# KwangsungKim138/Korean-F5-TTS

Hardware: AMD Instinct MI355X
Metric: RTF (audio_sec/wall_sec) F5-TTS Base NFE=16 batch=1 (higher is better)
Workload: dtype f16; 1 GPU; C2: F5-TTS Base, 1 utterance/rank/step, prompt 256 + generated 768 mel frames, NFE=16 EPSS, cfg 2.0, sway -1, Vocos decode, mel all_gather when n_gpus>1; global_batch=1, frames=1024, parallelism=dp1, weights=synthetic random-init seed 0

## Files before the change

### korean-f5-tts_amd/csrc/attn2.h

```cpp
#pragma once
#include "attn.h"
#include "gemm2.h"

namespace f5 {

__device__ __forceinline__ float group_max(float v) {
    const unsigned u = __builtin_bit_cast(unsigned, v);
    auto a = __builtin_amdgcn_permlane32_swap(u, u, false, false);
    float m = fmaxf(__builtin_bit_cast(float, (unsigned)a[0]), __builtin_bit_cast(float, (unsigned)a[1]));
    const unsigned w = __builtin_bit_cast(unsigned, m);
    auto b = __builtin_amdgcn_permlane16_swap(w, w, false, false);
    return fmaxf(__builtin_bit_cast(float, (unsigned)b[0]), __builtin_bit_cast(float, (unsigned)b[1]));
}

template <typename T, int STAGE_IDX, bool EDGE, int VAR>
__device__ __forceinline__ void attn2_tile(const char* smem_ptr, unsigned lds_base, int k_off, int kc0, int kc1, int v_off, int vc,
                                           const u32x4 (&qf)[2][2], f32x4 (&o)[4][2], float (&mrun)[2], float (&lrun)[2],
                                           int key_base, int kv_len, bool first) {
    constexpr bool LAZY = (VAR & 4) != 0;
    constexpr int TILE = 64 * 128;
    constexpr float L2E = 1.4426950408889634f;
    const unsigned sb = lds_base + STAGE_IDX * (2 * TILE);
    u32x4 kf[2][2], vf[4];
    const char* sbp = smem_ptr + STAGE_IDX * (2 * TILE);
// ... 78 lines not shown
#pragma unroll
            for (int ks = 0; ks < 2; ++ks)
#pragma unroll
                for (int r = 0; r < 4; ++r) {
                    float p = __builtin_amdgcn_exp2f(s[ks][qs][r]);
                    if (EDGE && key_base + ks * 4 + r >= kv_len) p = 0.f;
                    s[ks][qs][r] = p;
                    psum += p;
                }
            lrun[qs] += psum;
        }
    } else {
    float alpha[2];
    bool grew = false;
#pragma unroll
    for (int qs = 0; qs < 2; ++qs) {
        if (EDGE) {
#pragma unroll
            for (int ks = 0; ks < 2; ++ks)
#pragma unroll
                for (int r = 0; r < 4; ++r)
                    if (key_base + ks * 4 + r >= kv_len) s[ks][qs][r] = -1e30f;
        }
#pragma unroll
        for (int ks = 0; ks < 2; ++ks)
#pragma unroll
            for (int r = 0; r < 4; ++r) s[ks][qs][r] *= L2E;
        float mloc = fmaxf(fmaxf(fmaxf(s[0][qs][0], s[0][qs][1]), fmaxf(s[0][qs][2], s[0][qs][3])),
                           fmaxf(fmaxf(s[1][qs][0], s[1][qs][1]), fmaxf(s[1][qs][2], s[1][qs][3])));
        if (VAR & 2) {
            mloc = group_max(mloc);
        } else {
            mloc = fmaxf(mloc, __shfl_xor(mloc, 16, 64));
            mloc = fmaxf(mloc, __shfl_xor(mloc, 32, 64));
        }
        const float mnew = fmaxf(mrun[qs], mloc);
        grew = grew || (mnew > mrun[qs]);
        alpha[qs] = __builtin_amdgcn_exp2f(mrun[qs] - mnew);
        mrun[qs] = mnew;
        float psum = 0.f;
#pragma unroll
        for (int ks = 0; ks < 2; ++ks)
#pragma unroll
            for (int r = 0; r < 4; ++r) {
                float p = __builtin_amdgcn_exp2f(s[ks][qs][r] - mnew);
                if (EDGE && key_base + ks * 4 + r >= kv_len) p = 0.f;
                s[ks][qs][r] = p;
                psum += p;
            }
        lrun[qs] = lrun[qs] * alpha[qs] + psum;
    }
    if (__any(grew)) {
#pragma unroll
        for (int qs = 0; qs < 2; ++qs)
#pragma unroll
            for (int dt = 0; dt < 4; ++dt) {
                o[dt][qs][0] *= alpha[qs]; o[dt][qs][1] *= alpha[qs]; o[dt][qs][2] *= alpha[qs]; o[dt][qs][3] *= alpha[qs];
            }
    }
    }
    u32x4 pf2[2];
#pragma unroll
    for (int qs = 0; qs < 2; ++qs) {
        pf2[qs] = pack8<T>(s[0][qs][0], s[0][qs][1], s[0][qs][2], s[0][qs][3], s[1][qs][0], s[1][qs][1], s[1][qs][2], s[1][qs][3]);
    }
    if (VAR & 1) {
        __builtin_amdgcn_sched_barrier(0);
        wait_lgkm<0>(vf[0], vf[1], vf[2], vf[3]);
    }
#pragma unroll
    for (int dt = 0; dt < 4; ++dt) {
#pragma unroll
        for (int qs = 0; qs < 2; ++qs) o[dt][qs] = Mma<T>::run(vf[dt], pf2[qs], o[dt][qs]);
    }
}

__device__ __forceinline__ int kswz(int r) { return (((r >> 3) & 3) << 1) | ((r >> 1) & 1); }

template <typename T, int VAR>
__global__ __launch_bounds__(512) void attn2_fwd_kernel(const T* __restrict__ Q, const T* __restrict__ K,
                                                               const T* __restrict__ Vt, T* __restrict__ O, int H,
                                                               int N, int Npad, const int* __restrict__ kv_lens,
                                                               int nbatch_lens, const int* __restrict__ q_lens,
                                                               const int* __restrict__ o_row_start, float* __restrict__ Of = nullptr) {
    extern __shared__ __attribute__((aligned(16))) char smem[];
    int bhid, qblk;
    attn_block_map(bhid, qblk);
    if (q_lens && qblk * 128 >= q_lens[(bhid / H) % nbatch_lens]) return;
    constexpr int NS = 3;
    constexpr int TILE = 64 * 128;
    constexpr int STAGE = 2 * TILE;
    constexpr int L = 2;
    constexpr float L2E = 1.4426950408889634f;

    const int tid = threadIdx.x, lane = tid & 63;
    const int wave = __builtin_amdgcn_readfirstlane(tid >> 6);
    const int qg = wave >> 1, kh = wave & 1;
    const int l15 = lane & 15, g = lane >> 4;
    const int b = bhid / H, h = bhid - b * H;
    const size_t bh = (size_t)bhid;
    const int q0 = qblk * 128 + qg * 32;
    int kv_len = N;
    if (kv_lens) kv_len = min(N, kv_lens[b % nbatch_lens]);
    const int nkt = (kv_len + 63) / 64;

    u32x4 qf[2][2];
#pragma unroll
    for (int qs = 0; qs < 2; ++qs) {
        const int q = min(q0 + qs * 16 + l15, N - 1);
#pragma unroll
        for (int f = 0; f < 2; ++f)
            qf[qs][f] = *reinterpret_cast<const u32x4*>(reinterpret_cast<const char*>(Q + (bh * N + q) * 64) + f * 64 + g * 16);
    }

    const int lr = lane >> 3, ls = lane & 7;
    const int krow = wave * 8 + lr;
    const int kchunk = ls ^ kswz(krow);
    const int vrow = wave * 8 + lr;
    const int vchunk = ls ^ (vrow & 7);
    const T* ksrc = K + bh * (size_t)N * 64 + kchunk * 8;
    const T* vsrc = Vt + (bh * 64 + vrow) * (size_t)Npad + vchunk * 8;
    auto issue = [&](int kt, int stage) {
        if (kt >= nkt) return;
        const int t = kt;
        char* base = smem + stage * STAGE;
        const int key = min(t * 64 + krow, N - 1);
        glds16(ksrc + (size_t)key * 64, base + wave * 1024);
        glds16(vsrc + t * 64, base + TILE + wave * 1024);
    };

    f32x4 o[4][2];
#pragma unroll
    for (int dt = 0; dt < 4; ++dt)
#pragma unroll
        for (int qs = 0; qs < 2; ++qs) o[dt][qs] = f32x4{0.f, 0.f, 0.f, 0.f};
    float mrun[2] = {(VAR & 4) ? 0.f : -1e30f, (VAR & 4) ? 0.f : -1e30f}, lrun[2] = {0.f, 0.f};

    const int ka = l15 >> 2, kb = l15 & 3;
    const int krd = kh * 32 + 8 * ka + kb;
    const int ksw = kswz(krd);
    const int k_off = krd * 128;
    const int kc0 = ((0 + g) ^ ksw) * 16, kc1 = ((4 + g) ^ ksw) * 16;
    const int v_off = TILE + l15 * 128;
    const int vc = ((4 * kh + g) ^ (l15 & 7)) * 16;
    const int key_lane = kh * 32 + 8 * g;
    const unsigned lds_base = (unsigned)(size_t)(__attribute__((address_space(3))) char*)smem;

    issue(0, 0);
    issue(1, 1);
    if (VAR & 1) __builtin_amdgcn_s_waitcnt(0xC07F);
    const int nfull = kv_len / 64;
    int kt = 0;
#define F5_ATTN_STEP(SI, EDGE_)                                                                                        \
    {                                                                                                                  \
        if (kt + 1 < nkt) wait_vmcnt<(NS - 2) * L>(); else wait_vmcnt<0>();                                            \
        __builtin_amdgcn_s_barrier();                                                                                  \
        issue(kt + NS - 1, (SI + NS - 1) % NS);                                                                        \
        attn2_tile<T, SI, EDGE_, VAR>(smem, lds_base, k_off, kc0, kc1, v_off, vc, qf, o, mrun, lrun, kt * 64 + key_lane, kv_len, kt == 0);        \
        ++kt;                                                                                                          \
    }
    while (kt + 3 <= nfull) {
        F5_ATTN_STEP(0, false)
        F5_ATTN_STEP(1, false)
        F5_ATTN_STEP(2, false)
    }
    if (kt < nkt) { if (kt < nfull) F5_ATTN_STEP(0, false) else F5_ATTN_STEP(0, true) }
    if (kt < nkt) { if (kt < nfull) F5_ATTN_STEP(1, false) else F5_ATTN_STEP(1, true) }
    if (kt < nkt) { F5_ATTN_STEP(2, true) }
#undef F5_ATTN_STEP
    __builtin_amdgcn_s_barrier();

#pragma unroll
    for (int qs = 0; qs < 2; ++qs) {
        float l = lrun[qs];
        l += __shfl_xor(l, 16, 64);
        l += __shfl_xor(l, 32, 64);
        lrun[qs] = l;
    }
    float* mb = reinterpret_cast<float*>(smem) + (size_t)qg * (36 * 64);
    if (kh == 1) {
#pragma unroll
        for (int dt = 0; dt < 4; ++dt)
#pragma unroll
            for (int qs = 0; qs < 2; ++qs)
#pragma unroll
                for (int r = 0; r < 4; ++r) mb[((dt * 2 + qs) * 4 + r) * 64 + lane] = o[dt][qs][r];
        mb[32 * 64 + lane] = mrun[0];
        mb[33 * 64 + lane] = mrun[1];
        mb[34 * 64 + lane] = lrun[0];
        mb[35 * 64 + lane] = lrun[1];
    }
    __syncthreads();
    if (kh == 0) {
#pragma unroll
        for (int qs = 0; qs < 2; ++qs) {
            const float m1 = mb[(32 + qs) * 64 + lane], l1 = mb[(34 + qs) * 64 + lane];
            const float m = fmaxf(mrun[qs], m1);
            const float a0 = exp2f(mrun[qs] - m), a1 = exp2f(m1 - m);
            const float inv = 1.0f / (lrun[qs] * a0 + l1 * a1);
            const int q = q0 + qs * 16 + l15;
            const size_t orow = o_row_start ? (size_t)o_row_start[b] + q : (size_t)b * N + q;
            if (q < (o_row_start ? min(N, o_row_start[b + 1] - o_row_start[b]) : N)) {
                T* dst = O + orow * (H * 64) + h * 64 + g * 4;
#pragma unroll
                for (int dt = 0; dt < 4; ++dt) {
                    float v[4];
#pragma unroll
                    for (int r = 0; r < 4; ++r)
                        v[r] = (o[dt][qs][r] * a0 + mb[((dt * 2 + qs) * 4 + r) * 64 + lane] * a1) * inv;
                    if (Of) store4_planar(Of + orow * (H * 64), h * 64 + g * 4 + dt * 16, v[0], v[1], v[2], v[3]);
                    else store4(dst + dt * 16, v[0], v[1], v[2], v[3]);
                }
            }
        }
    }
}

inline int& attn2_variant() { static int v = 7; return v; }
template <typename T> inline float attention_q_scale();
template <> inline float attention_q_scale<float>() { return 0.125f; }
template <> inline float attention_q_scale<bf16_t>() { return (attn2_variant() & 4) ? 0.125f * 1.4426950408889634f : 0.125f; }
template <> inline float attention_q_scale<f16_t>() { return attention_q_scale<bf16_t>(); }
template <typename T>
inline hipError_t launch_attention_v2(hipStream_t s, const T* Q, const T* K, const T* Vt, T* O, int Bp, int H,
                                      int N, int Npad, const int* kv_lens, int nbatch_lens, const int* q_lens, const int* o_row_start,
                                      float* o_planar_f32 = nullptr) {
    constexpr int smem = 3 * 2 * 64 * 128;
    dim3 grid(Bp * H, (N + 127) / 128);
    const int var = attn2_variant();
#define F5_ATTN2_LAUNCH(V)                                                                                             \
    {                                                                                                                  \
        static bool attr_set = false;                                                                                  \
        if (!attr_set) {                                                                                               \
            hipError_t e = hipFuncSetAttribute(reinterpret_cast<const void*>(&attn2_fwd_kernel<T, V>),                    \
                                               hipFuncAttributeMaxDynamicSharedMemorySize, smem);                      \
            if (e != hipSuccess) return e;                                                                             \
            attr_set = true;                                                                                           \
        }                                                                                                              \
        hipLaunchKernelGGL((attn2_fwd_kernel<T, V>), grid, dim3(512), smem, s, Q, K, Vt, O, H, N, Npad, kv_lens, nbatch_lens, q_lens, o_row_start, o_planar_f32); \
    }
    if (var == 0) F5_ATTN2_LAUNCH(0)
    else if (var == 3) F5_ATTN2_LAUNCH(3)
    else F5_ATTN2_LAUNCH(7)
#undef F5_ATTN2_LAUNCH
    return hipGetLastError();
}

inline hipError_t launch_attention_any(hipStream_t s, const bf16_t* Q, const bf16_t* K, const bf16_t* Vt, bf16_t* O, int Bp,
                                       int H, int N, int Npad, const int* kv_lens, int nbl, const int* q_lens = nullptr,
                                       const int* o_row_start = nullptr, bool  = false, bool  = false, int  = 0) {
    return launch_attention_v2<bf16_t>(s, Q, K, Vt, O, Bp, H, N, Npad, kv_lens, nbl, q_lens, o_row_start);
}
inline hipError_t launch_attention_any(hipStream_t s, const f16_t* Q, const f16_t* K, const f16_t* Vt, f16_t* O, int Bp,
                                       int H, int N, int Npad, const int* kv_lens, int nbl, const int* q_lens = nullptr,
                                       const int* o_row_start = nullptr, bool  = false, bool  = false, int  = 0) {
    return launch_attention_v2<f16_t>(s, Q, K, Vt, O, Bp, H, N, Npad, kv_lens, nbl, q_lens, o_row_start);
}
inline hipError_t launch_attention_any(hipStream_t s, const float* Q, const float* K, const float* Vt, float* O, int Bp, int H,
                                       int N, int Npad, const int* kv_lens, int nbl, const int* q_lens = nullptr,
                                       const int* o_row_start = nullptr, bool split16 = false, bool o_planar = false, int hi_only = 0) {
    if (split16) return launch_attention_split(s, Q, K, Vt, O, Bp, H, N, Npad, kv_lens, nbl, q_lens, o_row_start, o_planar, hi_only);
    return launch_attention<float>(s, Q, K, Vt, O, Bp, H, N, Npad, kv_lens, nbl, q_lens, o_row_start);
}

}
```

### korean-f5-tts_amd/csrc/elementwise.h

```cpp
#pragma once
#include "f5_common.h"

namespace f5 {


inline int ew_blocks(long total, int per_block = 256, int cap = 4096) {
    long b = (total + per_block - 1) / per_block;
    if (b < 1) b = 1;
    return (int)(b > cap ? cap : b);
}

struct Prefetch { const char* p0 = nullptr; size_t n0 = 0; const char* p1 = nullptr; size_t n1 = 0; };
template <typename TO>
__global__ __launch_bounds__(256) void layernorm_kernel(const float* __restrict__ x, int ldx, TO* __restrict__ out,
                                                        int ldo, int R, int D, float eps, const float* __restrict__ A,
                                                        const float* __restrict__ Bv, int vec_stride,
                                                        int rows_per_batch, int modulate, Prefetch pf,
                                                        const int* __restrict__ m_limit = nullptr, int planar = 0) {
    const int lane = threadIdx.x & 63;
    const int r = blockIdx.x * 4 + (threadIdx.x >> 6);
    if (r >= R || (m_limit && r >= *m_limit)) return;
    const float* xr = x + (size_t)r * ldx;
    float4 v[8], ga[8], gb[8];
    const size_t vb = (size_t)(rows_per_batch > 0 ? r / rows_per_batch : 0) * vec_stride;
    const float a0 = modulate ? 0.f : 1.f;
#pragma unroll
    for (int i = 0; i < 8; ++i) {
        const int c = lane * 4 + i * 256;
        v[i] = c < D ? *reinterpret_cast<const float4*>(xr + c) : make_float4(0, 0, 0, 0);
        ga[i] = (A && c < D) ? *reinterpret_cast<const float4*>(A + vb + c) : make_float4(a0, a0, a0, a0);
        gb[i] = (Bv && c < D) ? *reinterpret_cast<const float4*>(Bv + vb + c) : make_float4(0, 0, 0, 0);
    }
    u32x4 pfv[8] = {};
    if (pf.n0 | pf.n1) {
        const size_t gtid = (size_t)blockIdx.x * 256 + threadIdx.x, gsz = (size_t)gridDim.x * 256;
#pragma unroll
        for (int i = 0; i < 8; ++i) {
            const size_t off = (gtid + (size_t)(i & 3) * gsz) * 16;
            const char* base = i < 4 ? pf.p0 : pf.p1;
            const size_t n = i < 4 ? pf.n0 : pf.n1;
            if (off + 16 <= n) pfv[i] = *reinterpret_cast<const u32x4*>(base + off);
        }
    }
    float s = 0.f;
#pragma unroll
    for (int i = 0; i < 8; ++i) s += (v[i].x + v[i].y) + (v[i].z + v[i].w);
    const float mean = wave_sum(s) / (float)D;
    float q = 0.f;
#pragma unroll
    for (int i = 0; i < 8; ++i) {
        const int c = lane * 4 + i * 256;
        if (c < D) {
            const float a = v[i].x - mean, b = v[i].y - mean, cc = v[i].z - mean, d = v[i].w - mean;
            q += (a * a + b * b) + (cc * cc + d * d);
        }
    }
    const float rstd = rsqrtf(wave_sum(q) / (float)D + eps);
#pragma unroll
    for (int i = 0; i < 8; ++i) {
        const int c = lane * 4 + i * 256;
        if (c < D) {
            float4 a = ga[i];
            const float4 b = gb[i];
            if (modulate) { a.x += 1.f; a.y += 1.f; a.z += 1.f; a.w += 1.f; }
            store4_at(out + (size_t)r * ldo, c, planar, (v[i].x - mean) * rstd * a.x + b.x, (v[i].y - mean) * rstd * a.y + b.y,
                      (v[i].z - mean) * rstd * a.z + b.z, (v[i].w - mean) * rstd * a.w + b.w);
        }
    }
#pragma unroll
    for (int i = 0; i < 8; ++i) asm volatile("" ::"v"(pfv[i]));
}

template <typename TO>
__global__ __launch_bounds__(256) void xrmsnorm_kernel(const float* __restrict__ x, int ldx, TO* __restrict__ out, int ldo,
                                                       int R, int D, const float* __restrict__ gvec, int planar = 0) {
    const int lane = threadIdx.x & 63;
    const int r = blockIdx.x * 4 + (threadIdx.x >> 6);
    if (r >= R) return;
    const float* xr = x + (size_t)r * ldx;
    float4 v[8];
    float q = 0.f;
#pragma unroll
    for (int i = 0; i < 8; ++i) {
        const int c = lane * 4 + i * 256;
        v[i] = c < D ? *reinterpret_cast<const float4*>(xr + c) : make_float4(0, 0, 0, 0);
        q += (v[i].x * v[i].x + v[i].y * v[i].y) + (v[i].z * v[i].z + v[i].w * v[i].w);
    }
    const float nrm = fmaxf(sqrtf(wave_sum(q)), 1e-12f);
    const float sc = sqrtf((float)D) / nrm;
#pragma unroll
    for (int i = 0; i < 8; ++i) {
        const int c = lane * 4 + i * 256;
        if (c < D) {
            const float4 gg = *reinterpret_cast<const float4*>(gvec + c);
            store4_at(out + (size_t)r * ldo, c, planar, v[i].x * sc * gg.x, v[i].y * sc * gg.y, v[i].z * sc * gg.z, v[i].w * sc * gg.w);
        }
    }
}
template <typename TO>
inline void launch_xrmsnorm(hipStream_t s, const float* x, TO* out, int rows, int D, const float* g, int planar) {
    hipLaunchKernelGGL((xrmsnorm_kernel<TO>), dim3((rows + 3) / 4), dim3(256), 0, s, x, D, out, D, rows, D, g, planar);
}

template <typename T>
__global__ void pack_input_kernel(const float* __restrict__ x, const float* __restrict__ cond,
                                  const float* __restrict__ text_c, const float* __restrict__ text_u,
                                  T* __restrict__ out, int ldo, int B, int Bp, int N, int mel, int Dt, int drop_cond_first,
                                  const int2* __restrict__ rowmap = nullptr, const int* __restrict__ row_limit = nullptr,
                                  const int* __restrict__ lens = nullptr) {
    const int K4 = (2 * mel + Dt) / 4;
    const long total = (rowmap ? (long)*row_limit : (long)Bp * N) * K4;
    for (long idx = blockIdx.x * (long)blockDim.x + threadIdx.x; idx < total; idx += (long)gridDim.x * blockDim.x) {
        const int c = (int)(idx % K4) * 4;
        const long row = idx / K4;
        int n = (int)(row % N), bp = (int)(row / N);
        if (rowmap) { const int2 m = rowmap[row]; bp = m.x; n = m.y; }
        const bool un = bp >= B;
        const int b = un ? bp - B : bp;
        float4 v;
        if (rowmap && n >= lens[b]) v = make_float4(0, 0, 0, 0);
        else if (c < mel) v = *reinterpret_cast<const float4*>(x + ((size_t)b * N + n) * mel + c);
        else if (c < 2 * mel)
            v = (un || drop_cond_first) ? make_float4(0, 0, 0, 0)
                                        : *reinterpret_cast<const float4*>(cond + ((size_t)b * N + n) * mel + (c - mel));
        else
            v = *reinterpret_cast<const float4*>((un ? text_u : text_c) + ((size_t)b * N + n) * Dt + (c - 2 * mel));
        store4(out + (size_t)row * ldo + c, v.x, v.y, v.z, v.w);
    }
}
template <typename T>
inline void launch_pack_input(hipStream_t s, const float* x, const float* cond, const float* text_c, const float* text_u, T* out, int ldo, int B,
                              int Bp, int N, int mel, int Dt, int drop_cond_first, const int2* rowmap, const int* row_limit, const int* lens) {
    const int rows = Bp * N, kin = 2 * mel + Dt;
    hipLaunchKernelGGL((pack_input_kernel<T>), dim3(ew_blocks((long)rows * kin / 4)), dim3(256), 0, s, x, cond, text_c, text_u, out, ldo, B, Bp,
                       N, mel, Dt, drop_cond_first, rowmap, row_limit, lens);
}

static __global__ void unett_assemble_kernel(const float* __restrict__ h, const float* __restrict__ temb, int temb_stride,
                                             float* __restrict__ x, int Bp, int N, int D) {
    const int d4 = D / 4;
    const long total = (long)Bp * (N + 1) * d4;
    for (long i = blockIdx.x * (long)blockDim.x + threadIdx.x; i < total; i += (long)gridDim.x * blockDim.x) {
        const int c = (int)(i % d4);
        const long row = i / d4;
        const int n = (int)(row % (N + 1)), b = (int)(row / (N + 1));
        const float4 v = n == 0 ? reinterpret_cast<const float4*>(temb + (size_t)b * temb_stride)[c]
                                : reinterpret_cast<const float4*>(h + ((size_t)b * N + (n - 1)) * D)[c];
        reinterpret_cast<float4*>(x)[i] = v;
    }
}
inline void launch_unett_assemble(hipStream_t s, const float* h, const float* temb, int temb_stride, float* x, int Bp, int N, int D) {
    const int rows = Bp * (N + 1);
    hipLaunchKernelGGL(unett_assemble_kernel, dim3(ew_blocks((long)rows * D / 4)), dim3(256), 0, s, h, temb, temb_stride, x, Bp, N, D);
}
template <typename T>
__global__ void cat2_kernel(const float* __restrict__ x, const float* __restrict__ skip, T* __restrict__ out, long rows, int D, int planar = 0) {
    const int d4 = D / 4;
    const long total = rows * 2 * d4;
    for (long i = blockIdx.x * (long)blockDim.x + threadIdx.x; i < total; i += (long)gridDim.x * blockDim.x) {
        const int c = (int)(i % (2 * d4));
        const long r = i / (2 * d4);
        const float4 v = c < d4 ? reinterpret_cast<const float4*>(x + r * D)[c]
                                : reinterpret_cast<const float4*>(skip + r * D)[c - d4];
        store4_at(out + r * 2 * D, c * 4, planar, v.x, v.y, v.z, v.w);
    }
}
template <typename T> inline void launch_cat2(hipStream_t s, const float* x, const float* skip, T* out, int rows, int D, int planar) {
    hipLaunchKernelGGL((cat2_kernel<T>), dim3(ew_blocks((long)rows * 2 * D / 4)), dim3(256), 0, s, x, skip, out, (long)rows, D, planar);
}
static __global__ void strip_first_token_kernel(const float* __restrict__ in, float* __restrict__ out, int Bp, int N, int C) {
    const int c4 = C / 4;
    const long total = (long)Bp * N * c4;
    for (long i = blockIdx.x * (long)blockDim.x + threadIdx.x; i < total; i += (long)gridDim.x * blockDim.x) {
        const int c = (int)(i % c4);
        const long row = i / c4;
        const int n = (int)(row % N), b = (int)(row / N);
        reinterpret_cast<float4*>(out)[i] = reinterpret_cast<const float4*>(in + ((size_t)b * (N + 1) + n + 1) * C)[c];
    }
}
inline void launch_strip_first_token(hipStream_t s, const float* in, float* out, int Bp, int N, int C) {
    const int rows_in = Bp * N;
    hipLaunchKernelGGL(strip_first_token_kernel, dim3(ew_blocks((long)rows_in * C / 4)), dim3(256), 0, s, in, out, Bp, N, C);
}

// ... 562 lines not shown
```

### korean-f5-tts_amd/csrc/engine.hip

```cpp
#include "engine_types.h"

#define F5_OPS(e, CALL)                                                  \
    ((e)->cfg.precision == F5_PREC_BF16  ? EngineOps<bf16_t>::CALL       \
     : ((e)->cfg.precision == F5_PREC_F16 || (e)->cfg.precision == F5_PREC_F16P) ? EngineOps<f16_t>::CALL        \
                                         : EngineOps<float>::CALL)

static thread_local char g_err[512] = "";
int f5_fail(int code, const char* fmt, ...) {
    va_list ap;
    va_start(ap, fmt);
    vsnprintf(g_err, sizeof(g_err), fmt, ap);
    va_end(ap);
    return code;
}
extern "C" const char* f5_last_error(void) { return g_err; }
extern "C" const char* f5_version(void) { return "f5hip 2 gfx950"; }
static Switches read_switches(const f5_config& c) {
    auto flag = [](const char* name, bool dflt) {
        const char* v = getenv(name);
        return (v && v[0] == (dflt ? '0' : '1')) ? !dflt : dflt;
    };
    Switches sw;
    sw.graphs = flag("F5_HIP_GRAPH", true);
    sw.split_cfg = flag("F5_SPLIT_CFG", false);
    sw.pack_rows = flag("F5_PACK_ROWS", true);
    if (const char* v = getenv("F5_CHUNK_ROWS")) sw.chunk_rows = std::max(1L, atol(v));
    sw.weight_prefetch = flag("F5_WEIGHT_PREFETCH", true);
    if (const char* v = getenv("F5_X3_ABLATE")) sw.x3_ablate = c.precision == F5_PREC_F16X3 ? atoi(v) : 0;
    sw.x3_attn_split = flag("F5_X3_ATTN_SPLIT", false);
    if (const char* v = getenv("F5_LEN_BUCKET")) sw.len_bucket = (int)std::min(std::max(atol(v), -1L), 1L << 20);
    return sw;
}
extern "C" int f5_create(const f5_config* c, f5_engine** out) {
    if (!c || !out) return fail(F5_EINVAL, "f5_create: null argument");
    if (c->dim_head != 64) return fail(F5_EINVAL, "dim_head must be 64 (got %d)", c->dim_head);
    if (c->dim % 256 != 0 || (c->dim / 16 != 16 && c->dim / 16 != 32 && c->dim / 16 != 48 && c->dim / 16 != 64))
        return fail(F5_EINVAL, "dim must be 256, 512, 768 or 1024 (got %d)", c->dim);
    if (c->heads <= 0 || (c->heads * 64) % 64 != 0 || c->depth <= 0) return fail(F5_EINVAL, "bad heads/depth");
    if (c->mel_dim % 4 || c->text_dim % 4 || c->ff_dim % 8) return fail(F5_EINVAL, "mel_dim/text_dim %% 4, ff_dim %% 8 required");
    if ((2 * c->mel_dim + c->text_dim) % 4) return fail(F5_EINVAL, "2*mel_dim + text_dim must be a multiple of 4");
    if (c->precision != F5_PREC_F32 && c->precision != F5_PREC_BF16 && c->precision != F5_PREC_F16 && c->precision != F5_PREC_F16X3 &&
        c->precision != F5_PREC_F16P)
        return fail(F5_EINVAL, "bad precision");
    if (c->precision == F5_PREC_F16X3 && c->ff_dim % 32)
        return fail(F5_EINVAL, "F5_PREC_F16X3 needs ff_dim %% 32 == 0 (whole 32-element blocks of the split operand layout; got %d)", c->ff_dim);
    if (c->backbone != F5_BACKBONE_DIT && c->backbone != F5_BACKBONE_UNETT) return fail(F5_EINVAL, "bad backbone");
    if (c->backbone == F5_BACKBONE_UNETT && (c->depth % 2)) return fail(F5_EINVAL, "UNetT depth must be even");
    if (c->text_dim > 2048 || c->dim > 2048) return fail(F5_EINVAL, "dims > 2048 unsupported");
    if (c->options & ~(F5_OPT_QK_RMSNORM | F5_OPT_LONG_SKIP | F5_OPT_TEXT_AVG_UPSAMPLE | F5_OPT_ADAPTERS)) return fail(F5_EINVAL, "unknown option bits %d", c->options);
    if (c->options && c->backbone != F5_BACKBONE_DIT) return fail(F5_EINVAL, "F5_OPT_* are options of the DiT backbone (dit.py:160-166)");
    if ((c->options & F5_OPT_TEXT_AVG_UPSAMPLE) && !c->text_mask_padding)
        return fail(F5_EINVAL, "text_embedding_average_upsampling requires text_mask_padding to be True (dit.py:41-42)");
    f5_engine* e = new f5_engine();
    e->cfg = *c;
    e->inner = c->heads * 64;
    e->kin = 2 * c->mel_dim + c->text_dim;
    e->kin_pad = round_up(e->kin, 64);
    e->modN = (6 * c->depth + 2) * c->dim;
    e->split16 = c->precision == F5_PREC_F16X3;
    e->io_split = c->precision == F5_PREC_F16P;
    e->sw = read_switches(*c);
    if (!valid_len_bucket(e->sw.len_bucket)) {
        const int g = e->sw.len_bucket;
        delete e;
        return fail(F5_EINVAL, "F5_LEN_BUCKET=%d: the granule is 0 (off) or a multiple of 8 in [8, 1024]", g);
    }
    e->adapters_on = (c->options & F5_OPT_ADAPTERS) != 0;
    if (e->adapters_on && e->sw.x3_ablate) {
        delete e;
        return fail(F5_EINVAL, "F5_OPT_ADAPTERS cannot be combined with the F5_X3_ABLATE diagnostic");
    }
    *out = e;
    return F5_OK;
}
extern "C" int f5_destroy(f5_engine* e) {
    if (e) {
        (void)hipDeviceSynchronize();
        delete e;
    }
    return F5_OK;
}
extern "C" int f5_load_weight(f5_engine* e, const char* name, const void* dev, const int64_t* shape, int32_t ndim,
                              f5_stream stream) {
    if (!e) return fail(F5_EINVAL, "null engine");
    e->finalized = false;
    e->uc_N = -1;
    e->clear_graphs();
    e->active = nullptr;
    e->adapt_gen++;
    return e->ws.put("f5_load_weight", name, dev, shape, ndim, (hipStream_t)stream);
}
extern "C" int f5_finalize(f5_engine* e, f5_stream stream) {
    if (!e) return fail(F5_EINVAL, "null engine");
    hipStream_t s = (hipStream_t)stream;
    e->clear_graphs();
    for (void* p : e->owned) (void)hipFree(p);
    e->owned.clear();
    e->pf = Packed<float>();
    e->pb = Packed<bf16_t>();
    e->ph = Packed<f16_t>();
    e->uc_N = -1;
    e->targets.clear();
    e->target_slot.clear();
    e->base_table = nullptr;
    e->active = nullptr;
    e->adapt_gen++;
    int r = F5_OPS(e, finalize(e, s));
    if (r != F5_OK) return r;
    if (e->adapters_on) {
        std::vector<MergeDesc> tab;
        for (auto& t : e->targets) {
            tab.push_back(t.base);
// ... 232 lines not shown
```

### korean-f5-tts_amd/csrc/engine_impl.h

```cpp
#pragma once
#include "engine_types.h"

static int need(const WeightStore& ws, const std::string& n, std::initializer_list<int64_t> shape, const Tensor** out) {
    const Tensor* t = ws.get(n);
    if (!t) return fail(F5_ESTATE, "missing weight '%s'", n.c_str());
    std::vector<int64_t> want(shape);
    if (t->shape != want) {
        std::string got, exp;
        for (auto s : t->shape) got += std::to_string(s) + ",";
        for (auto s : want) exp += std::to_string(s) + ",";
        return fail(F5_EINVAL, "weight '%s' has shape [%s], expected [%s]", n.c_str(), got.c_str(), exp.c_str());
    }
    *out = t;
    return F5_OK;
}

template <typename T, bool BB> static int maybe_split_weight(f5_engine* e, hipStream_t s, T* w, size_t elems) {
    if constexpr (BB && std::is_same_v<T, float>) {
        if (e->split16 || e->io_split) {
            hipLaunchKernelGGL(split_planar_kernel, dim3(ew_blocks((long)(elems / 32))), dim3(256), 0, s, w, (long)(elems / 32));
            HIPCHK(hipGetLastError());
        }
    }
    return F5_OK;
// ... 321 lines not shown

template <typename T> static int run_time_path(f5_engine* e, Work<T>& w, int S, hipStream_t s) {
    Packed<T>& P = packed<T>(e);
    const int D = e->cfg.dim;
    return e->prof.timed(PC_TIME, s, [&]() -> int {
        launch_time_sinus(s, w.tdev, P.time_freqs, w.feat, S);
        KCHK();
        HIPCHK(launch_gemm<float>(s, w.feat, 256, P.time0.w, P.time0.ldw, S, D, 256,
                                  EpiStore<float>{w.th, D, P.time0.b, F5_ACT_SILU}));
        HIPCHK(launch_gemm<float>(s, w.th, D, P.time2.w, P.time2.ldw, S, D, D, EpiStore<float>{w.temb, D, P.time2.b, F5_ACT_NONE}));
        if (e->cfg.backbone == F5_BACKBONE_DIT) {
            hipLaunchKernelGGL(act_kernel, dim3(ew_blocks((long)S * D)), dim3(256), 0, s, w.temb, w.st, (long)S * D, F5_ACT_SILU);
            KCHK();
            HIPCHK(launch_gemm<float>(s, w.st, D, P.mod.w, P.mod.ldw, S, e->modN, D,
                                      EpiStore<float>{w.mod, e->modN, P.mod.b, F5_ACT_NONE}));
        }
        return F5_OK;
    });
}

template <typename T>
static int run_text_embed(f5_engine* e, Work<T>& w, const int64_t* text, int B, int nt, const int* lens_dev, int N,
                          int drop_text, float* out, hipStream_t s) {
    Packed<T>& P = packed<T>(e);
    const f5_config& c = e->cfg;
    const int Dt = c.text_dim;
    const bool dit = c.backbone == F5_BACKBONE_DIT;
    const long rows = (long)B * N;
    if (c.conv_layers > 0 && dit && N > P.text_pos_rows) return fail(F5_EINVAL, "N=%d exceeds aux.text_pos rows", N);
    return e->prof.timed(PC_TEXT, s, [&]() -> int {
        float* cur = c.conv_layers > 0 ? w.tx_a : out;
        const int pos_rows = P.text_pos_rows > 0 ? P.text_pos_rows : 1;
        hipLaunchKernelGGL(text_embed_kernel, dim3(ew_blocks(rows * Dt / 4)), dim3(256), 0, s, (const long long*)text, nt, P.E,
                           P.text_pos, cur, B, N, Dt, lens_dev, drop_text, c.text_mask_padding && c.conv_layers > 0,
                           c.conv_layers > 0, dit ? 1 << 30 : pos_rows);
        KCHK();
        for (int i = 0; i < c.conv_layers; ++i) {
            TextBlockW& tb = P.tblocks[i];
            float* nxt = (i == c.conv_layers - 1) ? out : cur;
            hipLaunchKernelGGL(dwconv7_ln_kernel, dim3((rows + 3) / 4), dim3(256), 0, s, cur, w.tx_b, tb.dwk, tb.dwb, tb.lnw,
                               tb.lnb, B, N, Dt, lens_dev, 1e-6f);
            KCHK();
            HIPCHK(launch_gemm<float>(s, w.tx_b, Dt, tb.pw1.w, tb.pw1.ldw, (int)rows, 2 * Dt, Dt,
                                      EpiStore<float>{w.tx_h1, 2 * Dt, tb.pw1.b, F5_ACT_GELU_ERF}));
            hipLaunchKernelGGL(grn_partial_kernel, dim3((2 * Dt + 255) / 256, GRN_P, B), dim3(256), 0, s, w.tx_h1, w.grn_part,
                               N, 2 * Dt, lens_dev);
            KCHK();
            const int rpb = 16;
            hipLaunchKernelGGL(grn_apply_kernel, dim3((N + rpb - 1) / rpb, B), dim3(256), (2 * Dt + 8) * sizeof(float), s,
                               w.tx_h1, w.grn_part, tb.gamma, tb.beta, N, 2 * Dt, lens_dev, rpb);
            KCHK();
            HIPCHK(launch_gemm<float>(s, w.tx_h1, 2 * Dt, tb.pw2.w, tb.pw2.ldw, (int)rows, Dt, 2 * Dt,
                                      EpiGateRes{nxt, cur, Dt, tb.pw2.b, nullptr, 0, N, nullptr}));
            if (c.text_mask_padding) {
                hipLaunchKernelGGL(zero_filler_rows_kernel, dim3(ew_blocks(rows * Dt / 4)), dim3(256), 0, s,
                                   (const long long*)text, nt, nxt, B, N, Dt);
                KCHK();
            }
            cur = nxt;
        }
        if (lens_dev && c.conv_layers > 0) {
            hipLaunchKernelGGL(zero_tail_rows_kernel, dim3(ew_blocks(rows * Dt / 4)), dim3(256), 0, s, out, B, N, Dt, lens_dev);
            KCHK();
        }
        if (c.options & F5_OPT_TEXT_AVG_UPSAMPLE) {
            hipLaunchKernelGGL(text_avg_upsample_kernel, dim3(B), dim3(256), (size_t)N * sizeof(int), s, (const long long*)text, nt, out, w.tx_b, N, Dt,
                               lens_dev);
            KCHK();
            HIPCHK(hipMemcpyAsync(out, w.tx_b, (size_t)rows * Dt * sizeof(float), hipMemcpyDeviceToDevice, s));
        }
        return F5_OK;
    });
}

struct FwdCtx {
    f5_engine* e;
    hipStream_t s;
    int B, Bp, N, rows;
    const int* lens_dev;
    RowPack pk;
    const int* ml() const { return pk.rows_dev; }
    int mh() const { return pk ? (int)pk.rows_host : 0; }
    int pl() const { return e->split16 ? 1 : 0; }
    double gflops(double n, double k) const { return 2.0 * (pk ? pk.rows_host : (double)rows) * n * k; }
    template <typename T, typename Epi> int gemm(const T* A, int lda, const LinW<T>& L, int n, int k, const Epi& epi, bool a_split = false) const {
        HIPCHK(e->prof.timed(PC_GEMM, s, gflops(n, k), [&] { return egemm<T>(e, s, A, lda, L.w, L.ldw, rows, n, k, epi, ml(), mh(), a_split); }));
        return F5_OK;
    }
    template <typename T> void ablate(int bit, T* a, int k) const {
        if (e->sw.x3_ablate & bit) zero_lo_planar(s, a, (size_t)rows * k);
    }
};

template <typename T, typename U>
static int embed_input(const FwdCtx& f, Work<T>& w, const float* y, const float* cond, int drop_cond_first, const float* text_first,
                       const float* text_second, float* dst, bool ablate = false) {
    f5_engine* e = f.e;
    hipStream_t s = f.s;
    Packed<T>& P = packed<T>(e);
    Prof& pr = e->prof;
    const f5_config& c = e->cfg;
    const int D = c.dim, rows = f.rows, B = f.B, Bp = f.Bp, N = f.N;
    const RowPack& pk = f.pk;
    U* acat = reinterpret_cast<U*>(w.acat);
    const LinW<U>* ip;
    U* const* cw;
    int kp;
    bool cs;
    if constexpr (std::is_same_v<U, T>) {
        ip = &P.in_proj; cw = P.conv_w; kp = P.conv_kp; cs = conv_split(e);
    } else {
        ip = &P.in_proj_f; cw = P.conv_w_f; kp = P.conv_kp_f; cs = convpos_can_split(D);
    }
    HIPCHK(pr.timed(PC_MISC, s, [&] {
        launch_pack_input<U>(s, y, cond, text_first, text_second, acat, e->kin_pad, B, Bp, N, c.mel_dim, c.text_dim, drop_cond_first, pk.rowmap,
                             f.ml(), f.lens_dev);
        return hipGetLastError();
    }));
    auto ablate_round = [&](int bit, const float* src, float* to, long n) -> const float* {
        if (!ablate || !(e->sw.x3_ablate & bit)) return src;
        hipLaunchKernelGGL(round_f16_kernel, dim3(ew_blocks(n)), dim3(256), 0, s, src, to, n);
        return to;
    };
    if constexpr (std::is_same_v<U, float>) ablate_round(64, acat, acat, (long)rows * e->kin_pad);
    HIPCHK(pr.timed(PC_GEMM, s, f.gflops(D, e->kin), [&] {
        const EpiStore<float> epi{w.h, D, ip->b, F5_ACT_NONE};
        if constexpr (std::is_same_v<U, T>) return egemm<T>(e, s, acat, e->kin_pad, ip->w, ip->ldw, rows, D, e->kin_pad, epi, f.ml(), f.mh());
        else return launch_gemm<float>(s, acat, e->kin_pad, ip->w, ip->ldw, rows, D, e->kin_pad, epi, {GemmOperands::WSplit, -1, f.ml(), f.mh()});
    }));
    const double conv_fl = f.gflops(D, (D / 16) * 31);
    HIPCHK(pr.timed(PC_CONV, s, conv_fl, [&] {
        const float* conv1_in = ablate_round(128, w.h, w.x, (long)rows * D);
        return launch_convpos<U>(s, conv1_in, cw[0], kp, P.conv_b[0], nullptr, w.c1, Bp, N, D, f.lens_dev, B, pk.row_start, cs);
    }));
    ablate_round(128, w.c1, w.c1, (long)rows * D);
    HIPCHK(pr.timed(PC_CONV, s, conv_fl, [&] {
        return launch_convpos<U>(s, w.c1, cw[1], kp, P.conv_b[1], w.h, dst, Bp, N, D, f.lens_dev, B, pk.row_start, cs);
    }));
    return F5_OK;
}

template <typename T>
static int attention_block(const FwdCtx& f, Work<T>& w, const BlockW<T>& bw, bool qk_norm, const EpiGateRes& out_epi) {
    f5_engine* e = f.e;
    hipStream_t s = f.s;
    Packed<T>& P = packed<T>(e);
    Prof& pr = e->prof;
    const f5_config& c = e->cfg;
    const int D = c.dim, inner = e->inner, H = c.heads, B = f.B, Bp = f.Bp, N = f.N, pl = f.pl();
    const RowPack& pk = f.pk;
    const int pe_heads = c.pe_attn_head < 0 ? H : c.pe_attn_head;
    const int* attn_lens = ((c.attn_mask_enabled || pk) && f.lens_dev) ? f.lens_dev : nullptr;
    const double attn_fl = 4.0 * H * 64 * (pk ? pk.sq_host : (double)Bp * N * N);
    f.ablate(1, w.xn, D);
    bool attn16 = false;
    if constexpr (std::is_same_v<T, float>) {
        attn16 = e->split16 && e->sw.x3_attn_hi() == 3 && !qk_norm;
        if (attn16) {
            f16_t *q = reinterpret_cast<f16_t*>(w.q), *k = reinterpret_cast<f16_t*>(w.k), *vt = reinterpret_cast<f16_t*>(w.vt);
            CHK(f.gemm(w.xn, D, bw.qkv, 3 * inner, D,
                       EpiQKV<f16_t>{q, k, vt, bw.qkv.b, P.rope_frag, N, w.Npad, H, pe_heads, attention_q_scale<f16_t>(), pk.rowmap}, pl));
            HIPCHK(pr.timed(PC_ATTN, s, attn_fl, [&] {
                return launch_attention_v2<f16_t>(s, q, k, vt, nullptr, Bp, H, N, w.Npad, attn_lens, B, f.lens_dev, pk.row_start, w.ao);
            }));
        }
    }
    if (!attn16) {
        CHK(f.gemm(w.xn, D, bw.qkv, 3 * inner, D,
                   EpiQKV<T>{w.q, w.k, w.vt, bw.qkv.b, P.rope_frag, N, w.Npad, H, qk_norm ? 0 : pe_heads,
                             qk_norm ? 1.0f : attention_q_scale<T>(), pk.rowmap}, pl));
        if (qk_norm) {
            const long qrows = (long)Bp * H * N;
            HIPCHK(pr.timed(PC_MISC, s, [&] {
                hipLaunchKernelGGL((qknorm_rope_kernel<T>), dim3((unsigned)((qrows * 16 + 255) / 256)), dim3(256), 0, s, w.q, w.k, bw.qn, bw.kn,
                                   P.rope_cos, P.rope_sin, qrows, N, H, pe_heads, attention_q_scale<T>(), 1e-6f);
                return hipGetLastError();
            }));
        }
        HIPCHK(pr.timed(PC_ATTN, s, attn_fl, [&] {
            return launch_attention_any(s, w.q, w.k, w.vt, w.ao, Bp, H, N, w.Npad, attn_lens, B, f.lens_dev, pk.row_start, e->split16, pl,
                                        e->sw.x3_attn_hi());
        }));
    }
    f.ablate(8, w.ao, inner);
    return f.gemm(w.ao, inner, bw.out, D, inner, out_epi, pl);
}

template <typename T> static int ff_block(const FwdCtx& f, Work<T>& w, const BlockW<T>& bw, const EpiGateRes& out_epi) {
    const int D = f.e->cfg.dim, F = f.e->cfg.ff_dim, pl = f.pl();
    f.ablate(16, w.xn, D);
    CHK(f.gemm(w.xn, D, bw.ff1, F, D, EpiStore<T>{w.ffh, F, bw.ff1.b, F5_ACT_GELU_TANH, pl}, pl));
    f.ablate(32, w.ffh, F);
    return f.gemm(w.ffh, F, bw.ff2, D, F, out_epi, pl);
}

template <typename T, typename U> static int project_out(const FwdCtx& f, const U* xn, float* pred) {
    f5_engine* e = f.e;
    Packed<T>& P = packed<T>(e);
    const int D = e->cfg.dim, mel = e->cfg.mel_dim;
    if constexpr (std::is_same_v<U, T>) {
        return f.gemm(xn, D, P.proj_out, mel, D, EpiStore<float>{pred, mel, P.proj_out.b, F5_ACT_NONE}, f.pl());
    } else {
        HIPCHK(e->prof.timed(PC_GEMM, f.s, f.gflops(mel, D), [&] {
            return launch_gemm<float>(f.s, xn, D, P.proj_out_f.w, P.proj_out_f.ldw, f.rows, mel, D,
                                      EpiStore<float>{pred, mel, P.proj_out_f.b, F5_ACT_NONE}, {GemmOperands::AWSplit, -1, f.ml(), f.mh()});
        }));
        return F5_OK;
    }
}

template <typename T>
static int run_dit_forward(f5_engine* e, Work<T>& w, const float* y, const float* cond, int B, int Bp, int N,
                           const float* mod_row, int mod_stride, const int* lens_dev, int drop_cond_first,
                           const float* text_first, const float* text_second, hipStream_t s, const RowPack& pk = RowPack{}) {
    Packed<T>& P = packed<T>(e);
    const f5_config& c = e->cfg;
    const int D = c.dim, rows = Bp * N;
    const FwdCtx f{e, s, B, Bp, N, rows, lens_dev, pk};
    const int* ml = f.ml();
    const int mh = f.mh(), pl = f.pl();
    const int* gate_lens = pk ? nullptr : lens_dev;
    Prof& pr = e->prof;
    if (e->io_split) CHK((embed_input<T, float>(f, w, y, cond, drop_cond_first, text_first, text_second, w.x)));
    else CHK((embed_input<T, T>(f, w, y, cond, drop_cond_first, text_first, text_second, w.x, true)));
    const bool long_skip = (c.options & F5_OPT_LONG_SKIP) != 0;
    if (long_skip)
        HIPCHK(hipMemcpyAsync(w.h, w.x, (size_t)rows * D * sizeof(float), hipMemcpyDeviceToDevice, s));
    const bool qk_norm = (c.options & F5_OPT_QK_RMSNORM) != 0;
    const bool wpf = rows <= 4096 && e->sw.weight_prefetch;
    auto prefetch = [&](const LinW<T>& a, const LinW<T>& b) {
        return wpf ? Prefetch{(const char*)a.w, (size_t)a.N * a.ldw * sizeof(T), (const char*)b.w, (size_t)b.N * b.ldw * sizeof(T)} : Prefetch{};
    };
    auto adaln = [&](auto* out, const float* scale, const float* shift, const Prefetch& pf, int planar) {
        using TO = std::remove_pointer_t<decltype(out)>;
        return pr.timed(PC_LN, s, [&] {
            hipLaunchKernelGGL((layernorm_kernel<TO>), dim3((rows + 3) / 4), dim3(256), 0, s, w.x, D, out, D, rows, D, 1e-6f, scale, shift,
                               mod_stride, N, 1, pf, ml, planar);
            return hipGetLastError();
        });
    };
    for (int l = 0; l < c.depth; ++l) {
        BlockW<T>& bw = P.blocks[l];
        const float* m = mod_row + (size_t)l * 6 * D;
        HIPCHK(adaln(w.xn, m + D, m, prefetch(bw.qkv, bw.out), pl));
        CHK(attention_block<T>(f, w, bw, qk_norm, EpiGateRes{w.x, w.x, D, bw.out.b, m + 2 * D, mod_stride, N, gate_lens}));
        HIPCHK(adaln(w.xn, m + 4 * D, m + 3 * D, prefetch(bw.ff1, bw.ff2), pl));
        CHK(ff_block<T>(f, w, bw, EpiGateRes{w.x, w.x, D, bw.ff2.b, m + 5 * D, mod_stride, N, nullptr}));
    }
    if (long_skip) {
        auto cat_skip = [&](auto* cat) {
            return pr.timed(PC_MISC, s, [&] {
                launch_cat2(s, w.x, w.h, cat, rows, D, 0);
                return hipGetLastError();
            });
        };
        const EpiStore<float> epi{w.x, D, nullptr, F5_ACT_NONE};
        if (e->io_split) {
            float* cat_f = reinterpret_cast<float*>(w.cat2);
            HIPCHK(cat_skip(cat_f));
            HIPCHK(pr.timed(PC_GEMM, s, f.gflops(D, 2 * D), [&] {
                return launch_gemm<float>(s, cat_f, 2 * D, P.long_skip_f.w, P.long_skip_f.ldw, rows, D, 2 * D, epi, {GemmOperands::WSplit, -1, ml, mh});
            }));
        } else {
            HIPCHK(cat_skip(w.cat2));
            CHK(f.gemm(w.cat2, 2 * D, P.long_skip, D, 2 * D, epi));
        }
    }
    const float* mf = mod_row + (size_t)c.depth * 6 * D;
    if (e->io_split) {
        HIPCHK(adaln(w.c1, mf, mf + D, Prefetch{}, 1));
        return project_out<T, float>(f, w.c1, w.pred);
    }
    HIPCHK(adaln(w.xn, mf, mf + D, Prefetch{}, pl));
    f.ablate(256, w.xn, D);
    return project_out<T, T>(f, w.xn, w.pred);
}

template <typename T>
static int run_unett_forward(f5_engine* e, Work<T>& w, const float* y, const float* cond, int B, int Bp, int N,
                             const float* temb, int temb_stride, const int* lens_dev, int drop_cond_first,
                             const float* text_first, const float* text_second, hipStream_t s) {
    Packed<T>& P = packed<T>(e);
    const f5_config& c = e->cfg;
    const int D = c.dim, mel = c.mel_dim;
    const int Nt = N + 1;
    const int rows_in = Bp * N, rows = Bp * Nt;
    Prof& pr = e->prof;
    float* emb = reinterpret_cast<float*>(w.cat2);
    const FwdCtx in{e, s, B, Bp, N, rows_in, nullptr, RowPack{}};
    if (e->io_split) CHK((embed_input<T, float>(in, w, y, cond, drop_cond_first, text_first, text_second, emb)));
    else CHK((embed_input<T, T>(in, w, y, cond, drop_cond_first, text_first, text_second, emb)));
    const int half = c.depth / 2;
    auto slot = [&](int l) { return w.skips + (size_t)l * rows * D; };
    HIPCHK(pr.timed(PC_MISC, s, [&] {
        launch_unett_assemble(s, emb, temb, temb_stride, half > 0 ? slot(0) : w.x, Bp, N, D);
        return hipGetLastError();
    }));
    const FwdCtx f{e, s, B, Bp, Nt, rows, lens_dev, RowPack{}};
    const int pl = f.pl();
    auto rmsnorm = [&](const float* x, auto* out, const float* g, int planar) {
        return pr.timed(PC_LN, s, [&] {
            launch_xrmsnorm(s, x, out, rows, D, g, planar);
            return hipGetLastError();
        });
    };
    for (int l = 0; l < c.depth; ++l) {
        BlockW<T>& bw = P.blocks[l];
        const float* x_in = l < half ? slot(l) : w.x;
        float* x_out = l + 1 < half ? slot(l + 1) : w.x;
        if (l >= half) {
            const float* skip = w.skips + (size_t)(c.depth - 1 - l) * rows * D;
            HIPCHK(pr.timed(PC_MISC, s, [&] {
                launch_cat2(s, w.x, skip, w.cat2, rows, D, pl);
                return hipGetLastError();
            }));
            f.ablate(512, w.cat2, 2 * D);
            CHK(f.gemm(w.cat2, 2 * D, bw.skip, D, 2 * D, EpiStore<float>{w.x, D, nullptr, F5_ACT_NONE}, pl));
        }
        HIPCHK(rmsnorm(x_in, w.xn, bw.norm1_g, pl));
        CHK(attention_block<T>(f, w, bw, false, EpiGateRes{w.x, x_in, D, bw.out.b, nullptr, 0, Nt, lens_dev}));
        HIPCHK(rmsnorm(w.x, w.xn, bw.norm2_g, pl));
        CHK(ff_block<T>(f, w, bw, EpiGateRes{x_out, w.x, D, bw.ff2.b, nullptr, 0, Nt, nullptr}));
    }
    if (e->io_split) {
        HIPCHK(rmsnorm(w.x, w.skips, P.norm_out_g, 1));
        CHK((project_out<T, float>(f, w.skips, w.pred_all)));
    } else {
        HIPCHK(rmsnorm(w.x, w.xn, P.norm_out_g, pl));
        CHK((project_out<T, T>(f, w.xn, w.pred_all)));
    }
    HIPCHK(pr.timed(PC_MISC, s, [&] {
        launch_strip_first_token(s, w.pred_all, w.pred, Bp, N, mel);
        return hipGetLastError();
    }));
    return F5_OK;
}

template <typename T>
static int run_backbone(f5_engine* e, Work<T>& w, const float* y, const float* cond, int B, int Bp, int N, int step_row,
                        int per_row_time, const int* lens_dev, int drop_cond_first, const float* text_first,
                        const float* text_second, hipStream_t s, const RowPack& pk = RowPack{}) {
    if (e->cfg.backbone == F5_BACKBONE_DIT)
        return run_dit_forward<T>(e, w, y, cond, B, Bp, N, w.mod + (size_t)step_row * e->modN, per_row_time ? e->modN : 0,
                                  lens_dev, drop_cond_first, text_first, text_second, s, pk);
    return run_unett_forward<T>(e, w, y, cond, B, Bp, N, w.temb + (size_t)step_row * e->cfg.dim, per_row_time ? e->cfg.dim : 0,
                                lens_dev, drop_cond_first, text_first, text_second, s);
}
template <typename T>
static int upload_small(f5_engine* e, Work<T>& w, const float* t_host, int nT, const int32_t* lens_host, const SamplePlan& p,
                        hipStream_t s) {
    const int B = p.B;
    const size_t bytes = (size_t)nT * 4 + (size_t)3 * B * 4 + ((size_t)3 * B + 16) * 4 + 64;
    char* hb = nullptr;
    int slot = 0;
    CHK(e->stage.acquire(bytes, &hb, &slot));
    float* th = reinterpret_cast<float*>(hb);
    int* lh = reinterpret_cast<int*>(hb + (size_t)nT * 4);
    if (nT > 0) {
        memcpy(th, t_host, (size_t)nT * 4);
        HIPCHK(hipMemcpyAsync(w.tdev, th, (size_t)nT * 4, hipMemcpyHostToDevice, s));
    }
    if (lens_host) {
        const int add = e->cfg.backbone == F5_BACKBONE_UNETT ? 1 : 0;
        int* rs = lh + 3 * B;
        int nrs = 0;
        for (const SamplePlan::Chunk& k : p.chunks) {
            int* l = lh + p.lens_at(k);
            for (int i = 0; i < k.bc; ++i) l[i] = l[k.bc + i] = lens_host[k.u0 + i] + add;
            int* t = rs + p.row_start_at(k);
            t[0] = 0;
            for (int q = 0; q < p.halves * k.bc; ++q) t[q + 1] = t[q] + round_up(lens_host[k.u0 + q % k.bc], 4);
            nrs = p.row_start_at(k) + p.halves * k.bc + 1;
        }
        for (int i = 0; i < B; ++i) lh[2 * B + i] = lens_host[i] + add;
        HIPCHK(hipMemcpyAsync(w.lens, lh, (size_t)2 * B * 4, hipMemcpyHostToDevice, s));
        HIPCHK(hipMemcpyAsync(w.lens_plain, lh + 2 * B, (size_t)B * 4, hipMemcpyHostToDevice, s));
        HIPCHK(hipMemcpyAsync(w.row_start, rs, (size_t)nrs * 4, hipMemcpyHostToDevice, s));
    }
    return e->stage.release(slot, s);
}
template <typename T>
int EngineOps<T>::text_embed(f5_engine* e, const int64_t* text, int B, int nt, const int32_t* lens_host, int N, int drop_text,
                             float* out, hipStream_t s) {
    CHK(ensure_arena(e, B, N, 1));
    Work<T> w;
    carve<T>(e, w, e->res_B, e->res_N, e->res_S);
    CHK(upload_small<T>(e, w, nullptr, 0, lens_host, plan_sample(e, B, N, lens_host, B), s));
    const bool per_sample = lens_host && e->cfg.backbone == F5_BACKBONE_DIT;
    return run_text_embed<T>(e, w, text, B, nt, per_sample ? w.lens_plain : nullptr, N, drop_text, out, s);
}
template <typename T>
int EngineOps<T>::forward(f5_engine* e, const float* x, const float* cond, const int64_t* text, int nt, const float* time_host,
                          const int32_t* lens_host, int B, int N, int cfg_infer, int drop_audio_cond, int drop_text, float* out,
                          hipStream_t s) {
    const int Bp = cfg_infer ? 2 * B : B;
    CHK(ensure_arena(e, B, N, Bp));
    Work<T> w;
    carve<T>(e, w, e->res_B, e->res_N, e->res_S);
    std::vector<float> tt(Bp);
    for (int i = 0; i < Bp; ++i) tt[i] = time_host[i % B];
    CHK(upload_small<T>(e, w, tt.data(), Bp, lens_host, plan_sample(e, B, N, lens_host, B), s));
    const int* lens_dev = lens_host ? w.lens : nullptr;
    CHK(run_time_path<T>(e, w, Bp, s));
    const int* tlens = (e->cfg.backbone == F5_BACKBONE_DIT && lens_host) ? w.lens_plain : nullptr;
    if (cfg_infer) {
// ... 260 lines not shown
```

### korean-f5-tts_amd/csrc/engine_types.h

```cpp
#pragma once
#include <hip/hip_runtime.h>

#include <cmath>
#include <cstdarg>
#include <cstdio>
#include <algorithm>
#include <cstdlib>
#include <chrono>
#include <cstring>
#include <map>
#include <string>
#include <vector>

#include "internal.h"
#include "adapter.h"
#include "attn2.h"
#include "convpos.h"
#include "elementwise.h"
#include "gemm_dispatch.h"

using namespace f5;
#define fail f5_fail
struct Prof {
    enum { MAXEV = 65536 };
// ... 25 lines not shown
            hipEvent_t e;
            if (hipEventCreate(&e) != hipSuccess) return;
            ev.push_back(e);
        }
        (void)hipEventRecord(ev[used], s);
        cls.push_back(c);
        flops.push_back(fl);
    }
    void end(hipStream_t s) {
        if (!on || used + 2 > MAXEV || (int)ev.size() < used + 2 || (int)cls.size() * 2 != used + 2) return;
        (void)hipEventRecord(ev[used + 1], s);
        used += 2;
    }
};
enum { PC_GEMM = 0, PC_ATTN = 1, PC_LN = 2, PC_CONV = 3, PC_MISC = 4, PC_TEXT = 5, PC_TIME = 6 };

template <typename T> struct LinW {
    T* w = nullptr;
    float* b = nullptr;
    int N = 0, K = 0, ldw = 0;
};

template <typename T> struct BlockW {
    LinW<T> qkv, out, ff1, ff2, skip;
    float* norm1_g = nullptr;
    float* norm2_g = nullptr;
    float *qn = nullptr, *kn = nullptr;
};

struct TextBlockW {
    float *dwk = nullptr, *dwb = nullptr, *lnw = nullptr, *lnb = nullptr, *gamma = nullptr, *beta = nullptr;
    LinW<float> pw1, pw2;
};

template <typename T> struct Packed {
    LinW<float> time0, time2, mod;
    float* E = nullptr;
    std::vector<TextBlockW> tblocks;
    LinW<T> in_proj;
    T* conv_w[2] = {nullptr, nullptr};
    float* conv_b[2] = {nullptr, nullptr};
    int conv_kp = 0;
    std::vector<BlockW<T>> blocks;
    LinW<T> proj_out;
    LinW<T> long_skip;
    LinW<float> long_skip_f;
    LinW<float> in_proj_f, proj_out_f;
    float* conv_w_f[2] = {nullptr, nullptr};
    int conv_kp_f = 0;
    float* norm_out_g = nullptr;
    float *rope_cos = nullptr, *rope_sin = nullptr, *time_freqs = nullptr, *text_pos = nullptr;
    float* rope_frag = nullptr;
    int text_pos_rows = 0;
};

struct AdaptTarget {
    std::string name;
    std::vector<int64_t> shape;
    bool lowrank = false;
    MergeDesc base{};
};
struct f5_adapter {
    f5_engine* eng = nullptr;
    unsigned gen = 0;
    MergeDesc* table = nullptr;
    std::map<int, std::vector<void*>> bufs;
    ~f5_adapter() {
        for (auto& kv : bufs)
            for (void* p : kv.second) (void)hipFree(p);
        if (table) (void)hipFree(table);
    }
};

struct Switches {
    bool graphs = true;
    bool split_cfg = false;
    bool pack_rows = true;
    long chunk_rows = 0;
    bool weight_prefetch = true;
    int x3_ablate = 0;
    bool x3_attn_split = false;
    int x3_attn_hi() const { return x3_attn_split ? (x3_ablate >> 1) & 3 : 3; }
    int len_bucket = 0;
};
inline bool valid_len_bucket(long g) { return g == 0 || (g >= 8 && g <= 1024 && g % 8 == 0); }

struct GraphCache {
    enum { DEFAULT_CAPACITY = 16, MAX_CAPACITY = 64 };
    struct Entry { std::string key; hipGraph_t graph; hipGraphExec_t exec; };
    struct Stats { int captures = 0, replays = 0, eager = 0, evictions = 0; };
    Stats stats;
    size_t capacity = DEFAULT_CAPACITY;
    std::vector<Entry> graphs;
    std::vector<std::string> warm;
    hipStream_t cap_stream = nullptr;
    bool disabled = false;
    GraphCache() = default;
    GraphCache(const GraphCache&) = delete;
    void clear() {
        while (!graphs.empty()) evict(0);
        warm.clear();
    }
    hipGraphExec_t find(const std::string& key) const {
        for (auto& g : graphs)
            if (g.key == key) return g.exec;
        return nullptr;
    }
    bool is_warm(const std::string& base_key) const { return std::find(warm.begin(), warm.end(), base_key) != warm.end(); }
    void mark_warm(const std::string& base_key) {
        if (!is_warm(base_key)) warm.push_back(base_key);
    }
    template <typename F> int capture(const std::string& key, F&& body, hipGraphExec_t* exec) {
        if (!cap_stream) HIPCHK(hipStreamCreateWithFlags(&cap_stream, hipStreamNonBlocking));
        hipGraph_t graph = nullptr;
        if (hipStreamBeginCapture(cap_stream, hipStreamCaptureModeRelaxed) != hipSuccess) {
            fprintf(stderr, "libf5hip: hipStreamBeginCapture failed (%s); continuing with eager launches\n",
                    hipGetErrorString(hipGetLastError()));
        } else {
            const int rc = body(cap_stream);
            const hipError_t ce = hipStreamEndCapture(cap_stream, &graph);
            if (rc == F5_OK && ce == hipSuccess && graph && hipGraphInstantiate(exec, graph, nullptr, nullptr, 0) == hipSuccess) {
                while (graphs.size() >= capacity) {
                    evict(0);
                    stats.evictions++;
                }
                graphs.push_back({key, graph, *exec});
                stats.captures++;
                return F5_OK;
            }
            fprintf(stderr, "libf5hip: HIP graph capture of sample() failed (body rc %d, end-capture: %s, last: %s); "
                            "continuing with eager launches\n", rc, hipGetErrorString(ce), hipGetErrorString(hipGetLastError()));
            if (graph) (void)hipGraphDestroy(graph);
        }
        *exec = nullptr;
        disabled = true;
        return F5_OK;
    }
    void evict(size_t i) {
        if (graphs[i].exec) (void)hipGraphExecDestroy(graphs[i].exec);
        if (graphs[i].graph) (void)hipGraphDestroy(graphs[i].graph);
        graphs.erase(graphs.begin() + i);
    }
};

struct f5_engine {
    f5_config cfg{};
    int inner = 0, kin = 0, kin_pad = 0, modN = 0;
    bool io_split = false;
    bool split16 = false;
    Switches sw;
    WeightStore ws;
    std::vector<void*> owned;
    Packed<float> pf;
    Packed<bf16_t> pb;
    Packed<f16_t> ph;
    bool finalized = false;
    Arena arena;
    Staging stage;
    Prof prof;
    int res_B = 0, res_N = 0, res_S = 0;
    int uc_N = -1;
    GraphCache gc;
    hipStream_t side_stream = nullptr;
    hipEvent_t ev_fork = nullptr, ev_join = nullptr;
    int res_nt = 0;
    bool adapters_on = false;
// ... 97 lines not shown
```

### korean-f5-tts_amd/csrc/f5_common.h

```cpp
#pragma once
#include <type_traits>
#include <hip/hip_runtime.h>
#include <stdint.h>

typedef __bf16 bf16_t;
typedef __attribute__((ext_vector_type(8))) __bf16 bf16x8;
typedef __attribute__((ext_vector_type(4))) __bf16 bf16x4;
typedef __attribute__((ext_vector_type(2))) __bf16 bf16x2;
typedef _Float16 f16_t;
typedef __attribute__((ext_vector_type(8))) _Float16 f16x8;
typedef __attribute__((ext_vector_type(4))) _Float16 f16x4;
typedef __attribute__((ext_vector_type(4))) float f32x4;
typedef __attribute__((ext_vector_type(4))) unsigned int u32x4;
typedef __attribute__((ext_vector_type(2))) unsigned int u32x2;

#define F5_WAVE 64

enum { F5_ACT_NONE = 0, F5_ACT_GELU_TANH = 1, F5_ACT_GELU_ERF = 2, F5_ACT_SILU = 3, F5_ACT_MISH = 4, F5_ACT_LOGCLAMP = 5 };

namespace f5 {

__device__ __forceinline__ float gelu_tanh(float x) {
    const float c0 = -2.0f * 1.4426950408889634f * 0.7978845608028654f, c1 = c0 * 0.044715f;
    const float e = __builtin_amdgcn_exp2f(x * __builtin_fmaf(c1, x * x, c0));
    return x * __builtin_amdgcn_rcpf(1.0f + e);
}
__device__ __forceinline__ float gelu_erf(float x) { return 0.5f * x * (1.0f + erff(x * 0.7071067811865476f)); }
__device__ __forceinline__ float silu(float x) { return x / (1.0f + expf(-x)); }
__device__ __forceinline__ float mish(float x) {
    const float n = expf(fminf(x, 20.0f));
    const float t = n * (n + 2.0f);
    return x > 20.0f ? x : x * t * __frcp_rn(t + 2.0f);
}
__device__ __forceinline__ float apply_act(float v, int act) {
    switch (act) {
        case F5_ACT_GELU_TANH: return gelu_tanh(v);
        case F5_ACT_GELU_ERF: return gelu_erf(v);
        case F5_ACT_SILU: return silu(v);
        case F5_ACT_MISH: return mish(v);
        case F5_ACT_LOGCLAMP: return logf(fmaxf(v, 1e-5f));
        default: return v;
    }
}

__device__ __forceinline__ float f16_src(float v) {
    asm("" : "+v"(v));
    return v;
}
typedef __attribute__((ext_vector_type(2))) float f32x2_cv;
typedef __attribute__((ext_vector_type(2))) _Float16 f16x2_cv;
__device__ __forceinline__ unsigned cvt2_f16(float a, float b) {
    return __builtin_bit_cast(unsigned, __builtin_convertvector(f32x2_cv{a, b}, f16x2_cv));
}
__device__ __forceinline__ float to_f32(float v) { return v; }
__device__ __forceinline__ float to_f32(bf16_t v) { return (float)v; }
__device__ __forceinline__ float to_f32(f16_t v) { return (float)v; }
template <typename T> __device__ __forceinline__ T from_f32(float v);
template <> __device__ __forceinline__ float from_f32<float>(float v) { return v; }
template <> __device__ __forceinline__ bf16_t from_f32<bf16_t>(float v) { return (bf16_t)v; }
template <> __device__ __forceinline__ f16_t from_f32<f16_t>(float v) { return (f16_t)f16_src(v); }

__device__ __forceinline__ void store4(float* p, float a, float b, float c, float d) {
    *reinterpret_cast<float4*>(p) = make_float4(a, b, c, d);
}
__device__ __forceinline__ void store4(bf16_t* p, float a, float b, float c, float d) {
    bf16x4 v = {(bf16_t)a, (bf16_t)b, (bf16_t)c, (bf16_t)d};
    *reinterpret_cast<bf16x4*>(p) = v;
}
__device__ __forceinline__ void store4(f16_t* p, float a, float b, float c, float d) {
    *reinterpret_cast<u32x2*>(p) = u32x2{cvt2_f16(a, b), cvt2_f16(c, d)};
}

template <typename TO> __device__ __forceinline__ u32x2 pack4(float a, float b, float c, float d);
template <> __device__ __forceinline__ u32x2 pack4<bf16_t>(float a, float b, float c, float d) {
    bf16x4 v = {(bf16_t)a, (bf16_t)b, (bf16_t)c, (bf16_t)d};
    return __builtin_bit_cast(u32x2, v);
}
template <> __device__ __forceinline__ u32x2 pack4<f16_t>(float a, float b, float c, float d) {
    return u32x2{cvt2_f16(a, b), cvt2_f16(c, d)};
}

__device__ __forceinline__ void split4_f16(const u32x4& c, u32x2& hi, u32x2& lo) {
    typedef __attribute__((ext_vector_type(2))) float v2f;
    typedef __attribute__((ext_vector_type(2))) _Float16 v2h;
    const f32x4 x = __builtin_bit_cast(f32x4, c);
    const v2f a{x[0], x[1]}, b{x[2], x[3]};
    const v2h ah = __builtin_convertvector(a, v2h), bh = __builtin_convertvector(b, v2h);
    const v2h al = __builtin_convertvector(a - __builtin_convertvector(ah, v2f), v2h);
    const v2h bl = __builtin_convertvector(b - __builtin_convertvector(bh, v2f), v2h);
    hi = u32x2{__builtin_bit_cast(unsigned, ah), __builtin_bit_cast(unsigned, bh)};
    lo = u32x2{__builtin_bit_cast(unsigned, al), __builtin_bit_cast(unsigned, bl)};
}
__device__ __forceinline__ void store4_planar(float* row, int col, float a, float b, float c, float d) {
    u32x2 hi, lo;
    split4_f16(__builtin_bit_cast(u32x4, f32x4{a, b, c, d}), hi, lo);
    const int kk = col & 31;
    char* p = reinterpret_cast<char*>(row + (col & ~31)) + ((kk & 15) >> 2) * 16 + (kk >> 4) * 8;
    *reinterpret_cast<u32x2*>(p) = hi;
    *reinterpret_cast<u32x2*>(p + 64) = lo;
}
template <typename TO> __device__ __forceinline__ void store4_at(TO* row, int col, int planar, float a, float b, float c, float d) {
    if constexpr (std::is_same_v<TO, float>) {
        if (planar) { store4_planar(row, col, a, b, c, d); return; }
    }
    store4(row + col, a, b, c, d);
}

template <typename T> __device__ __forceinline__ u32x4 pack8(float a0, float a1, float a2, float a3, float a4, float a5, float a6, float a7);
template <> __device__ __forceinline__ u32x4 pack8<bf16_t>(float a0, float a1, float a2, float a3, float a4, float a5, float a6, float a7) {
    bf16x8 v = {(bf16_t)a0, (bf16_t)a1, (bf16_t)a2, (bf16_t)a3, (bf16_t)a4, (bf16_t)a5, (bf16_t)a6, (bf16_t)a7};
    return __builtin_bit_cast(u32x4, v);
}
template <> __device__ __forceinline__ u32x4 pack8<f16_t>(float a0, float a1, float a2, float a3, float a4, float a5, float a6, float a7) {
    return u32x4{cvt2_f16(a0, a1), cvt2_f16(a2, a3), cvt2_f16(a4, a5), cvt2_f16(a6, a7)};
}

__device__ __forceinline__ float wave_sum(float v) {
#pragma unroll
    for (int o = 32; o > 0; o >>= 1) v += __shfl_xor(v, o, 64);
    return v;
}
__device__ __forceinline__ float wave_max(float v) {
#pragma unroll
    for (int o = 32; o > 0; o >>= 1) v = fmaxf(v, __shfl_xor(v, o, 64));
    return v;
}

}
```

### korean-f5-tts_amd/csrc/gemm.h

```cpp
#pragma once
#include <type_traits>
#include "f5_common.h"

namespace f5 {

constexpr int GEMM_ROW_BYTES = 128;
constexpr int GEMM_ROW_STRIDE = 144;

template <typename T> struct Mma;
template <> struct Mma<bf16_t> {
    static __device__ __forceinline__ f32x4 run(const u32x4& a, const u32x4& b, f32x4 c) {
        return __builtin_amdgcn_mfma_f32_16x16x32_bf16(__builtin_bit_cast(bf16x8, a), __builtin_bit_cast(bf16x8, b), c,
                                                       0, 0, 0);
    }
};
template <> struct Mma<f16_t> {
    static __device__ __forceinline__ f32x4 run(const u32x4& a, const u32x4& b, f32x4 c) {
        return __builtin_amdgcn_mfma_f32_16x16x32_f16(__builtin_bit_cast(f16x8, a), __builtin_bit_cast(f16x8, b), c, 0, 0, 0);
    }
};
template <> struct Mma<float> {
    static __device__ __forceinline__ f32x4 run(const u32x4& a, const u32x4& b, f32x4 c) {
        const f32x4 fa = __builtin_bit_cast(f32x4, a), fb = __builtin_bit_cast(f32x4, b);
#pragma unroll
        for (int j = 0; j < 4; ++j) c = __builtin_amdgcn_mfma_f32_16x16x4f32(fa[j], fb[j], c, 0, 0, 0);
        return c;
    }
};

struct NoCtx {};

template <typename TO, int ACT = -1> struct EpiStore {
    TO* out; int ldo; const float* bias; int act;
    int planar = 0;
    struct RowCtx { TO* p; };
    struct ColCtx { float4 b; int n; };
    typedef NoCtx TRowCtx;
    typedef NoCtx TColCtx;
    static constexpr bool kTransposes = false;
    __device__ __forceinline__ bool tile_transposed(int) const { return false; }
    __device__ __forceinline__ RowCtx row(int m) const { return {out + (size_t)m * ldo}; }
    __device__ __forceinline__ ColCtx col(int n) const {
        return {bias ? *reinterpret_cast<const float4*>(bias + n) : make_float4(0, 0, 0, 0), n};
    }
    typedef NoCtx Pre;
    __device__ __forceinline__ NoCtx preload(const RowCtx&, const ColCtx&) const { return {}; }
    __device__ __forceinline__ void store(const RowCtx& r, const ColCtx& c, f32x4 v, const NoCtx&) const {
        const int a = ACT >= 0 ? ACT : act;
        store4_at(r.p, c.n, planar, apply_act(v[0] + c.b.x, a), apply_act(v[1] + c.b.y, a), apply_act(v[2] + c.b.z, a),
                  apply_act(v[3] + c.b.w, a));
    }
    static constexpr bool kStaged = sizeof(TO) == 2;
    __device__ __forceinline__ bool staged_ok(bool transposed) const { return !transposed; }
    template <int MI, int NJ>
    __device__ __forceinline__ void staged(char* slice, int lane, int mw, int nw, const f32x4 (&acc)[MI][NJ], bool) const {
        if constexpr (sizeof(TO) == 2) {
            static_assert(MI == 8 && NJ == 4, "128 x 64 wave tile");
            const int l15 = lane & 15, g = lane >> 4, a = ACT >= 0 ? ACT : act;
            float4 bj[NJ];
#pragma unroll
            for (int j = 0; j < NJ; ++j) bj[j] = bias ? *reinterpret_cast<const float4*>(bias + nw + j * 16 + g * 4) : make_float4(0, 0, 0, 0);
#pragma unroll
            for (int j = 0; j < NJ; ++j)
#pragma unroll
                for (int i = 0; i < MI; ++i) {
                    const f32x4 v = acc[i][j];
                    const int r = i * 16 + l15;
                    *reinterpret_cast<u32x2*>(slice + r * 128 + (((j * 2 + (g >> 1)) ^ (r & 7)) << 4) + ((g & 1) << 3)) =
                        pack4<TO>(apply_act(v[0] + bj[j].x, a), apply_act(v[1] + bj[j].y, a), apply_act(v[2] + bj[j].z, a), apply_act(v[3] + bj[j].w, a));
                }
            const int rr = lane >> 3, ch = lane & 7;
            TO* dst = out + (size_t)(mw + rr) * ldo + nw + ch * 8;
#pragma unroll
            for (int p = 0; p < 16; ++p) {
                const int r = p * 8 + rr;
                *reinterpret_cast<u32x4*>(dst + (size_t)p * 8 * ldo) = *reinterpret_cast<const u32x4*>(slice + r * 128 + ((ch ^ (r & 7)) << 4));
            }
        }
    }
    __device__ __forceinline__ NoCtx trow(int, int) const { return {}; }
    __device__ __forceinline__ NoCtx tcol(int) const { return {}; }
    __device__ __forceinline__ void tstore(const NoCtx&, const NoCtx&, f32x4) const {}
};

template <typename Epi, typename F> inline hipError_t with_static_act(const Epi& e, F&& f) { return f(e); }
template <typename TO, typename F> inline hipError_t with_static_act(const EpiStore<TO, -1>& e, F&& f) {
    switch (e.act) {
        case F5_ACT_NONE: return f(EpiStore<TO, F5_ACT_NONE>{e.out, e.ldo, e.bias, e.act, e.planar});
        case F5_ACT_GELU_TANH: return f(EpiStore<TO, F5_ACT_GELU_TANH>{e.out, e.ldo, e.bias, e.act, e.planar});
        case F5_ACT_GELU_ERF: return f(EpiStore<TO, F5_ACT_GELU_ERF>{e.out, e.ldo, e.bias, e.act, e.planar});
        case F5_ACT_SILU: return f(EpiStore<TO, F5_ACT_SILU>{e.out, e.ldo, e.bias, e.act, e.planar});
        case F5_ACT_MISH: return f(EpiStore<TO, F5_ACT_MISH>{e.out, e.ldo, e.bias, e.act, e.planar});
        case F5_ACT_LOGCLAMP: return f(EpiStore<TO, F5_ACT_LOGCLAMP>{e.out, e.ldo, e.bias, e.act, e.planar});
        default: return hipErrorInvalidValue;
    }
}

struct EpiGateRes {
    float* x; const float* res; int ld; const float* bias; const float* gate; int gate_stride; int rows_per_batch;
    const int* lens;
    struct RowCtx { size_t off; const float* g; bool masked; };
    struct ColCtx { float4 b; int n; };
    typedef NoCtx TRowCtx;
    typedef NoCtx TColCtx;
    static constexpr bool kTransposes = false;
    __device__ __forceinline__ bool tile_transposed(int) const { return false; }
    __device__ __forceinline__ RowCtx row(int m) const {
        const int b = m / rows_per_batch;
        return {(size_t)m * ld, gate ? gate + (size_t)b * gate_stride : nullptr,
                lens ? (m - b * rows_per_batch) >= lens[b] : false};
    }
    __device__ __forceinline__ ColCtx col(int n) const {
        return {bias ? *reinterpret_cast<const float4*>(bias + n) : make_float4(0, 0, 0, 0), n};
    }
    struct Pre { float4 r, g; };
    __device__ __forceinline__ Pre preload(const RowCtx& rc, const ColCtx& c) const {
        return {*reinterpret_cast<const float4*>(res + rc.off + c.n),
                rc.g ? *reinterpret_cast<const float4*>(rc.g + c.n) : make_float4(1, 1, 1, 1)};
    }
    __device__ __forceinline__ void store(const RowCtx& rc, const ColCtx& c, f32x4 v, const Pre& p) const {
        float4 r = p.r;
        if (!rc.masked) {
            const float4 g = p.g;
            r.x += g.x * (v[0] + c.b.x); r.y += g.y * (v[1] + c.b.y);
            r.z += g.z * (v[2] + c.b.z); r.w += g.w * (v[3] + c.b.w);
        }
        *reinterpret_cast<float4*>(x + rc.off + c.n) = r;
    }
    __device__ __forceinline__ NoCtx trow(int, int) const { return {}; }
    __device__ __forceinline__ NoCtx tcol(int) const { return {}; }
    __device__ __forceinline__ void tstore(const NoCtx&, const NoCtx&, f32x4) const {}
    static constexpr bool kStaged = true;
    __device__ __forceinline__ bool staged_ok(bool transposed) const { return !transposed && rows_per_batch >= 64; }
    template <int MI, int NJ>
    __device__ __forceinline__ void staged(char* slice, int lane, int mw, int nw, const f32x4 (&acc)[MI][NJ], bool) const {
        static_assert(MI == 8 && NJ == 4, "128 x 64 wave tile");
        const int l15 = lane & 15, g = lane >> 4, rr = lane >> 4, ch = lane & 15;
        const int n = nw + ch * 4;
        const float4 bv = bias ? *reinterpret_cast<const float4*>(bias + n) : make_float4(0, 0, 0, 0);
#pragma unroll
        for (int half = 0; half < 2; ++half) {
            const int mb = mw + half * 64;
            const int b0 = mb / rows_per_batch, b1 = (mb + 63) / rows_per_batch;
            const int m0 = b0 * rows_per_batch, m1 = b1 * rows_per_batch;
            float4 g0 = make_float4(1, 1, 1, 1), g1 = g0;
            if (gate) {
                g0 = *reinterpret_cast<const float4*>(gate + (size_t)b0 * gate_stride + n);
                g1 = *reinterpret_cast<const float4*>(gate + (size_t)b1 * gate_stride + n);
            }
            int len0 = 0x7fffffff, len1 = 0x7fffffff;
            if (lens) { len0 = lens[b0]; len1 = lens[b1]; }
            float4 rv[16];
            const float* rp = res + (size_t)(mb + rr) * ld + n;
#pragma unroll
            for (int p = 0; p < 16; ++p) rv[p] = *reinterpret_cast<const float4*>(rp + (size_t)p * 4 * ld);
#pragma unroll
            for (int j = 0; j < NJ; ++j)
#pragma unroll
                for (int i = 0; i < 4; ++i) {
                    const int r = i * 16 + l15;
                    *reinterpret_cast<f32x4*>(slice + r * 256 + (((j * 4 + g) ^ (r & 15)) << 4)) = acc[half * 4 + i][j];
                }
            float* xp = x + (size_t)(mb + rr) * ld + n;
#pragma unroll
            for (int p = 0; p < 16; ++p) {
                const int r = p * 4 + rr, m = mb + r;
                const f32x4 v = *reinterpret_cast<const f32x4*>(slice + r * 256 + ((ch ^ (r & 15)) << 4));
                const bool second = m >= m1 && b1 != b0;
                const float4 gg = second ? g1 : g0;
                const bool masked = (m - (second ? m1 : m0)) >= (second ? len1 : len0);
                float4 o = rv[p];
                const float tx = gg.x * (v[0] + bv.x), ty = gg.y * (v[1] + bv.y), tz = gg.z * (v[2] + bv.z), tw = gg.w * (v[3] + bv.w);
                o.x = masked ? o.x : o.x + tx; o.y = masked ? o.y : o.y + ty; o.z = masked ? o.z : o.z + tz; o.w = masked ? o.w : o.w + tw;
                *reinterpret_cast<float4*>(xp + (size_t)p * 4 * ld) = o;
            }
        }
    }
};

template <typename TO> struct EpiQKV {
    TO* q; TO* k; TO* vt; const float* bias; const float* rope;
    int Nseq, Npad, H, pe_heads; float q_scale;
    const int2* rowmap = nullptr;
    struct RowCtx { size_t base; const float* cs; };
    struct ColCtx { float4 b; TO* dst; size_t hoff; int d; bool rot; float scale; };
    struct TRowCtx { size_t base; int pos; int b; bool fast; int m; int M; };
    struct TColCtx { float b; size_t hoff; };
    static constexpr bool kTransposes = true;
    __device__ __forceinline__ bool tile_transposed(int n0) const { return n0 >= 2 * H * 64; }
    __device__ __forceinline__ RowCtx row(int m) const {
        int b = m / Nseq, pos = m - b * Nseq;
        if (rowmap) { const int2 bp = rowmap[m]; b = bp.x; pos = bp.y; }
        if (pos >= Nseq) return {0, nullptr};
        return {((size_t)b * H * Nseq + pos) * 64, rope + pos * 64};
    }
    __device__ __forceinline__ ColCtx col(int n) const {
        const int inner = H * 64;
        const int which = n >= inner ? 1 : 0, c = n - which * inner, h = c >> 6, d = c & 63;
        return {*reinterpret_cast<const float4*>(bias + n), which ? k : q, (size_t)h * Nseq * 64 + d, d, h < pe_heads,
                which ? 1.0f : q_scale};
    }
    struct Pre { float2 cs, sn; };
    __device__ __forceinline__ Pre preload(const RowCtx& r, const ColCtx& c) const {
        if (!c.rot || !r.cs) return {make_float2(1, 1), make_float2(0, 0)};
        const float4 t = *reinterpret_cast<const float4*>(r.cs + ((c.d >> 2) & 3) * 16 + (c.d >> 4) * 4);
        return {make_float2(t.x, t.y), make_float2(t.z, t.w)};
    }
    __device__ __forceinline__ void store(const RowCtx& r, const ColCtx& c, f32x4 v, const Pre& p) const {
        float a0 = v[0] + c.b.x, a1 = v[1] + c.b.y, a2 = v[2] + c.b.z, a3 = v[3] + c.b.w;
        if (c.rot) {
            const float2 cs = p.cs;
            const float2 sn = p.sn;
            const float r0 = a0 * cs.x - a1 * sn.x, r1 = a1 * cs.x + a0 * sn.x;
            const float r2 = a2 * cs.y - a3 * sn.y, r3 = a3 * cs.y + a2 * sn.y;
            a0 = r0; a1 = r1; a2 = r2; a3 = r3;
        }
        if (r.cs) store4(c.dst + r.base + c.hoff, a0 * c.scale, a1 * c.scale, a2 * c.scale, a3 * c.scale);
    }
    static constexpr bool kStaged = sizeof(TO) == 2;
    __device__ __forceinline__ bool staged_ok(bool transposed) const {
        return Nseq >= 8 && (!transposed || (rowmap == nullptr && (Nseq & 7) == 0));
    }
    template <int MI, int NJ>
    __device__ __forceinline__ void staged(char* slice, int lane, int mw, int nw, const f32x4 (&acc)[MI][NJ], bool transposed) const {
        if constexpr (sizeof(TO) == 2) {
            static_assert(MI == 8 && NJ == 4, "128 x 64 wave tile");
            const int l15 = lane & 15, g = lane >> 4;
            if (transposed) {
                float bn[NJ];
#pragma unroll
                for (int j = 0; j < NJ; ++j) bn[j] = bias[nw + j * 16 + l15];
#pragma unroll
                for (int j = 0; j < NJ; ++j) {
                    const int r = j * 16 + l15;
#pragma unroll
                    for (int i = 0; i < MI; ++i) {
                        const f32x4 v = acc[i][j];
                        *reinterpret_cast<u32x2*>(slice + r * 256 + (((i * 2 + (g >> 1)) ^ (r & 15)) << 4) + ((g & 1) << 3)) =
                            pack4<TO>(v[0] + bn[j], v[1] + bn[j], v[2] + bn[j], v[3] + bn[j]);
                    }
                }
                const int rr = lane >> 4, ch = lane & 15;
                const int m = mw + ch * 8, b = m / Nseq, pos = m - b * Nseq;
                TO* dst = vt + (size_t)b * H * 64 * Npad + (size_t)(nw - 2 * H * 64 + rr) * Npad + pos;
#pragma unroll
                for (int p = 0; p < 16; ++p) {
                    const int r = p * 4 + rr;
                    *reinterpret_cast<u32x4*>(dst + (size_t)p * 4 * Npad) = *reinterpret_cast<const u32x4*>(slice + r * 256 + ((ch ^ (r & 15)) << 4));
                }
                return;
            }
            const int inner = H * 64;
            const int which = nw >= inner ? 1 : 0, h = (nw - which * inner) >> 6;
            const bool rot = h < pe_heads;
            const float scale = which ? 1.0f : q_scale;
            float4 bj[NJ];
#pragma unroll
            for (int j = 0; j < NJ; ++j) bj[j] = *reinterpret_cast<const float4*>(bias + nw + j * 16 + g * 4);
            auto put = [&](int i, int j, float a0, float a1, float a2, float a3) {
                const int r = i * 16 + l15;
                *reinterpret_cast<u32x2*>(slice + r * 128 + (((j * 2 + (g >> 1)) ^ (r & 7)) << 4) + ((g & 1) << 3)) =
                    pack4<TO>(a0 * scale, a1 * scale, a2 * scale, a3 * scale);
            };
            if (rot) {
#pragma unroll
                for (int ih = 0; ih < 4; ++ih) {
// ... 216 lines not shown
```

### korean-f5-tts_amd/csrc/gemm2.h

```cpp
#pragma once
#include "gemm.h"


namespace f5 {

template <int N> __device__ __forceinline__ void wait_vmcnt() { asm volatile("s_waitcnt vmcnt(%0)" ::"n"(N) : "memory"); }

__device__ __forceinline__ void glds16(const void* gsrc, char* lds_dst) {
    __builtin_amdgcn_global_load_lds((const __attribute__((address_space(1))) void*)gsrc,
                                     (__attribute__((address_space(3))) void*)lds_dst, 16, 0, 0);
}

__device__ __forceinline__ void lds_read_b128_asm(u32x4& dst, unsigned addr) {
    asm volatile("ds_read_b128 %0, %1" : "=v"(dst) : "v"(addr));
}
template <int N> __device__ __forceinline__ void wait_lgkm(u32x4& a) { asm volatile("s_waitcnt lgkmcnt(%1)" : "+v"(a) : "n"(N > 15 ? 15 : N)); }
template <int N> __device__ __forceinline__ void wait_lgkm(u32x4& a, u32x4& b) {
    asm volatile("s_waitcnt lgkmcnt(%2)" : "+v"(a), "+v"(b) : "n"(N > 15 ? 15 : N));
}
template <int N> __device__ __forceinline__ void wait_lgkm(u32x4& a, u32x4& b, u32x4& c) {
    asm volatile("s_waitcnt lgkmcnt(%3)" : "+v"(a), "+v"(b), "+v"(c) : "n"(N > 15 ? 15 : N));
}
template <int N> __device__ __forceinline__ void wait_lgkm(u32x4& a, u32x4& b, u32x4& c, u32x4& d) {
    asm volatile("s_waitcnt lgkmcnt(%4)" : "+v"(a), "+v"(b), "+v"(c), "+v"(d) : "n"(N > 15 ? 15 : N));
// ... 194 lines not shown
                for (int j = 0; j < NJ; ++j) lds_read_b128_asm(wf[kk][j], sbu + w_row_off + j * 16 * GEMM_ROW_BYTES + co);
#pragma unroll
                for (int i = 1; i < MI; ++i) lds_read_b128_asm(af[kk][i], sbu + a_row_off + i * 16 * GEMM_ROW_BYTES + co);
            }
            if constexpr (OPS != GemmOperands::Plain) {
#pragma unroll
                for (int i = 0; i < MI; ++i) {
                    __builtin_amdgcn_sched_barrier(0);
                    wait_row<R, MI, NJ>(1, i, af, wf);
                    tie(af[0][i]);
                    if (i == 0) {
#pragma unroll
                        for (int j = 0; j < NJ; ++j) tie(wf[0][j]);
                    }
                    f16x8 ah, al;
                    if constexpr (OPS == GemmOperands::AWSplit) { ah = __builtin_bit_cast(f16x8, af[0][i]); al = __builtin_bit_cast(f16x8, af[1][i]); }
                    else split8_f16(af[0][i], af[1][i], ah, al);
#pragma unroll
                    for (int term = (DIAG == GemmDiag::TwoOfThree ? 1 : DIAG == GemmDiag::OneOfThree ? 2 : 0); term < 3; ++term) {
#pragma unroll
                        for (int j = 0; j < NJ; ++j) {
                            const f16x8 w = __builtin_bit_cast(f16x8, wf[term == 0 ? 1 : 0][j]);
                            const f16x8 a = term == 1 ? al : ah;
                            if (j < NJ - NT) acc[i][j] = __builtin_amdgcn_mfma_f32_16x16x32_f16(w, a, acc[i][j], 0, 0, 0);
                            else acc[i][j] = __builtin_amdgcn_mfma_f32_16x16x32_f16(a, w, acc[i][j], 0, 0, 0);
                        }
                    }
                }
                return;
            }
#pragma unroll
            for (int kk = 0; kk < 2; ++kk) {
#pragma unroll
                for (int i = 0; i < MI; ++i) {
                    __builtin_amdgcn_sched_barrier(0);
                    wait_row<R, MI, NJ>(kk, i, af, wf);
#pragma unroll
                    for (int j = 0; j < NJ; ++j) {
                        if (j < NJ - NT) acc[i][j] = Mma<T>::run(wf[kk][j], af[kk][i], acc[i][j]);
                        else acc[i][j] = Mma<T>::run(af[kk][i], wf[kk][j], acc[i][j]);
                    }
                }
            }
        };
        int stage = 0;
        {
            for (int kt = 0; kt < nkt; ++kt) {
                if (DIAG != GemmDiag::ComputeOnly) wait_tiles(nkt - 1 - kt);
                __builtin_amdgcn_s_barrier();
                int pf = stage + NS - 1;
                if (pf >= NS) pf -= NS;
                if (DIAG != GemmDiag::ComputeOnly) issue(kt + NS - 1, pf);
                if (DIAG != GemmDiag::DmaOnly) tile(stage);
                stage = stage + 1 == NS ? 0 : stage + 1;
            }
        }
    };
    if constexpr (Epi::kTransposes) {
        constexpr bool MIXED = (BN % 64) != 0 || BN == 192;
        if (nt == 0) kloop(std::integral_constant<int, 0>{});
        else if (nt == NJ) kloop(std::integral_constant<int, NJ>{});
        else if constexpr (MIXED && NJ >= 2) {
            if (nt == 1) kloop(std::integral_constant<int, 1>{});
            else if constexpr (NJ >= 3) {
                if (nt == 2) kloop(std::integral_constant<int, 2>{});
                else if constexpr (NJ >= 4) kloop(std::integral_constant<int, 3>{});
            }
        }
    } else {
        kloop(std::integral_constant<int, 0>{});
    }

    if (DIAG == GemmDiag::NoEpilogue && K > 0) {
        float sink = 0.f;
#pragma unroll
        for (int i = 0; i < MI; ++i)
#pragma unroll
            for (int j = 0; j < NJ; ++j) sink += acc[i][j][0] + acc[i][j][1] + acc[i][j][2] + acc[i][j][3];
        if (sink == 1234.5678f && lda < 0) *reinterpret_cast<volatile float*>(smem) = sink;
        return;
    }
    if (!EARLY) epilogue_setup();
    __builtin_amdgcn_s_waitcnt(0x0F70);
#pragma unroll
    for (int j = 0; j < NJ; ++j) {
        const int n = nw + j * 16 + g * 4;
        if (trj[j] || n >= N) continue;
#pragma unroll
        for (int i = 0; i < MI; ++i)
            if (mw + i * 16 + l15 < M) epi.store(rc[i], cc[j], acc[i][j], pre[i][j]);
    }
    if (any_tr) {
#pragma unroll
        for (int j = 0; j < NJ; ++j) {
            const int n = nw + j * 16 + l15;
            if (!trj[j] || n >= N) continue;
#pragma unroll
            for (int i = 0; i < MI; ++i)
                if (mw + i * 16 + g * 4 < M) epi.tstore(trc[i], tcc[j], acc[i][j]);
        }
    }
}

template <typename T, int BM, int BN, int WM, int WN, int NS, typename Epi, GemmOperands OPS = GemmOperands::Plain, GemmDiag DIAG = GemmDiag::None>
__global__ __launch_bounds__(WM* WN * 64) void gemm_tn_glds_kernel(const T* __restrict__ A, int lda,
                                                                   const T* __restrict__ W, int ldw, int M, int N, int K,
                                                                   Epi epi, int xa, int xb, const int* __restrict__ m_limit,
                                                                   const GemmConv cv) {
    extern __shared__ __attribute__((aligned(16))) char smem[];
    gemm_tn_glds_body<T, BM, BN, WM, WN, NS, Epi, OPS, DIAG>(smem, A, lda, W, ldw, M, N, K, epi, xa, xb, m_limit, cv);
}

inline int& xcd_mode() { static int m = 1; return m; }
inline void pick_xcd_rect(int tiles_m, int tiles_n, int* xa, int* xb) {
    *xa = *xb = 0;
    if (!xcd_mode()) return;
    long best = -1;
    for (int a = 1; a <= tiles_m && a <= 16; ++a) {
        if (tiles_m % a) continue;
        for (int b = 1; b <= tiles_n && b <= 32; ++b) {
            if (tiles_n % b) continue;
            const long rects = (long)(tiles_m / a) * (tiles_n / b);
            if (rects % 8) continue;
            const int area = a * b;
            if (area > 64) continue;
            const long score = 1000L * (64 - (area > 32 ? area - 32 : 32 - area)) - 10L * (a + b);
            if (score > best) { best = score; *xa = a; *xb = b; }
        }
    }
    if (*xa * *xb <= 1) *xa = *xb = 0;
}

template <typename T, int BM, int BN, int WM, int WN, int NS, typename Epi, GemmOperands OPS = GemmOperands::Plain, GemmDiag DIAG = GemmDiag::None>
inline hipError_t launch_gemm2(hipStream_t s, const T* A, int lda, const T* W, int ldw, int M, int N, int K,
                               const Epi& epi, const int* m_limit = nullptr, const GemmConv& cv = GemmConv{}) {
    constexpr int smem = NS * (BM + BN) * GEMM_ROW_BYTES;
    static bool attr_set = false;
    if (!attr_set) {
        hipError_t e = hipFuncSetAttribute(reinterpret_cast<const void*>(&gemm_tn_glds_kernel<T, BM, BN, WM, WN, NS, Epi, OPS, DIAG>),
                                           hipFuncAttributeMaxDynamicSharedMemorySize, smem);
        if (e != hipSuccess) return e;
        attr_set = true;
    }
    dim3 grid((N + BN - 1) / BN, (M + BM - 1) / BM);
    if (m_limit) grid.y = (grid.y + 7) / 8 * 8;
    int xa = 0, xb = 0;
    if (!m_limit) pick_xcd_rect((int)grid.y, (int)grid.x, &xa, &xb);
    hipLaunchKernelGGL((gemm_tn_glds_kernel<T, BM, BN, WM, WN, NS, Epi, OPS, DIAG>), grid, dim3(WM * WN * 64), smem, s, A, lda, W,
                       ldw, M, N, K, epi, xa, xb, m_limit, cv);
    return hipGetLastError();
}

}
```

### korean-f5-tts_amd/csrc/kapi.hip

```cpp
#include "kapi_common.h"

static int forced_cfg(int tm, int tn) { return tm > 0 ? tm * 1000 + tn : tm < 0 ? -tm : -1; }
static bool v1_tile(int cfg) { return gemm_tile(cfg) && gemm_tile(cfg)->family == GEMM_V1; }

template <typename T>
static int gemm_impl(const float* A, const float* W, const float* bias, int act, float* out, int M, int N, int K, int cfg, GemmOperands ops,
                     hipStream_t s) {
    const int Kp = round_up(K, v1_tile(cfg) ? 8 : GEMM_ROW_BYTES / (int)sizeof(T));
    if (cfg == G3_256x256_PP && !gemm_has_pingpong(sizeof(T), ops)) return fail(F5_EINVAL, "f5k_gemm: no ping-pong kernel (cfg 20) for these operands");
    GemmStage<T> g;
    CHK(g.stage(s, A, K, W, K, M, N, K, Kp, ops));
    HIPCHK(launch_gemm<T>(s, g.a.p, Kp, g.w.p, Kp, M, N, Kp, EpiStore<float>{out, N, bias, act}, {ops, cfg}));
    HIPCHK(hipStreamSynchronize(s));
    return F5_OK;
}

extern "C" int f5k_gemm(int32_t prec, const float* A, const float* W, const float* bias, int32_t act, float* out, int32_t M,
                        int32_t N, int32_t K, int32_t tm, int32_t tn, f5_stream stream) {
    if (!A || !W || !out || M <= 0 || N <= 0 || K <= 0 || (N % 4)) return fail(F5_EINVAL, "f5k_gemm: bad arguments (N %% 4 == 0)");
    const int cfg = forced_cfg(tm, tn);
    if (tm != 0 && (!gemm_tile(cfg) || v1_tile(cfg) != (tm > 0))) return fail(F5_EINVAL, "f5k_gemm: bad tile (tile_m > 0) or tile id (tile_m < 0)");
    const GemmOperands ops = prec != F5_PREC_F16X3 ? GemmOperands::Plain : (tm <= 0 && tn == 5) ? GemmOperands::AWSplit : GemmOperands::WSplit;
    if (ops != GemmOperands::Plain && tm > 0) return fail(F5_EINVAL, "f5k_gemm: the split-operand mode has no v1 kernel");
    return F5K_BY_PREC(prec, gemm_impl, A, W, bias, act, out, M, N, K, cfg, ops, (hipStream_t)stream);
// ... 38 lines not shown
    HIPCHK(hipEventSynchronize(e1));
    float ms = 0.f;
    HIPCHK(hipEventElapsedTime(&ms, e0, e1));
    *avg_us = ms * 1000.0f / iters;
    (void)hipEventDestroy(e0);
    (void)hipEventDestroy(e1);
    return F5_OK;
}

extern "C" int f5k_gemm_time(int32_t prec, int32_t M, int32_t N, int32_t K, int32_t tm, int32_t tn, int32_t iters,
                             float* avg_us, f5_stream stream) {
    if (!avg_us || M <= 0 || N <= 0 || K <= 0 || iters <= 0 || (N % 4)) return fail(F5_EINVAL, "f5k_gemm_time: bad arguments");
    const GemmOperands ops = prec == F5_PREC_F16X3 && tm <= 0 ? GemmOperands::WSplit : GemmOperands::Plain;
    return F5K_BY_PREC(prec, gemm_time_impl, M, N, K, forced_cfg(tm, tn), ops, iters, avg_us, (hipStream_t)stream);
}

template <typename T>
__global__ void pack_qkv_test_kernel(const float* q, const float* k, const float* v, T* qo, T* ko, T* vto, long nrows, int N,
                                     int Npad, float qscale) {
    const long total = nrows * 64;
    for (long i = blockIdx.x * (long)blockDim.x + threadIdx.x; i < total; i += (long)gridDim.x * blockDim.x) {
        const int d = (int)(i % 64);
        const long row = i / 64;
        const long bh = row / N;
        const int n = (int)(row % N);
        qo[i] = from_f32<T>(q[i] * qscale);
        ko[i] = from_f32<T>(k[i]);
        vto[(bh * 64 + d) * Npad + n] = from_f32<T>(v[i]);
    }
}
template <typename T> __global__ void to_f32_kernel(const T* in, float* out, long n) {
    for (long i = blockIdx.x * (long)blockDim.x + threadIdx.x; i < n; i += (long)gridDim.x * blockDim.x) out[i] = (float)in[i];
}

template <typename T> __global__ void fill_test_kernel(T* p, long n, float v) {
    for (long i = blockIdx.x * (long)blockDim.x + threadIdx.x; i < n; i += (long)gridDim.x * blockDim.x) p[i] = from_f32<T>(v);
}
template <typename TO> static int copy_f32(hipStream_t s, const void* src, float* dst, int64_t n) {
    if constexpr (!std::is_same_v<TO, float>) {
        if (dst && n > 0) {
            hipLaunchKernelGGL((to_f32_kernel<TO>), dim3(ew_blocks((long)n)), dim3(256), 0, s, static_cast<const TO*>(src), dst, (long)n);
            KCHK();
        }
    }
    return F5_OK;
}
static int upload_ints(Scratch<int>& d, const int32_t* host, int n) {
    if (!host) return F5_OK;
    HIPCHK(d.alloc((size_t)n));
    HIPCHK(hipMemcpy(d.p, host, (size_t)n * 4, hipMemcpyHostToDevice));
    return F5_OK;
}
template <typename F> static bool row_start_ok(const int32_t* rs, int Bp, int N, F min_span) {
    if (rs[0] != 0) return false;
    for (int b = 0; b < Bp; ++b) {
        const int cnt = rs[b + 1] - rs[b];
        if (rs[b] % 4 || cnt < min_span(b) || cnt > round_up(N, 4)) return false;
    }
    return rs[Bp] % 4 == 0;
}

template <typename T>
static int attn_body(const float* q, const float* k, const float* v, int Bp, int H, int N, const f5k_attn& p, bool split16, hipStream_t s) {
    const int Npad = round_up(N, 64);
    const long rows = (long)Bp * H * N;
    const size_t vt_elems = (size_t)Bp * H * 64 * Npad;
    Scratch<T> qd, kd, vd;
    Scratch<int> kl, ql, rs;
    HIPCHK(qd.alloc(rows * 64));
    HIPCHK(kd.alloc(rows * 64));
    HIPCHK(vd.alloc(vt_elems));
    CHK(upload_ints(kl, p.kv_lens_host, p.nlens));
    CHK(upload_ints(ql, p.q_lens_host, p.nlens));
    CHK(upload_ints(rs, p.row_start_host, Bp + 1));
    hipLaunchKernelGGL((fill_test_kernel<T>), dim3(ew_blocks((long)vt_elems)), dim3(256), 0, s, vd.p, (long)vt_elems, p.vt_pad_fill);
    hipLaunchKernelGGL((pack_qkv_test_kernel<T>), dim3(ew_blocks(rows * 64)), dim3(256), 0, s, q, k, v, qd.p, kd.p, vd.p, rows,
                       N, Npad, attention_q_scale<T>());
    KCHK();
    if (p.mode == 1) {
        if constexpr (std::is_same_v<T, f16_t>)
            HIPCHK(launch_attention_v2<f16_t>(s, qd.p, kd.p, vd.p, nullptr, Bp, H, N, Npad, kl.p, p.nlens, ql.p, rs.p, static_cast<float*>(p.out)));
    } else {
        HIPCHK(launch_attention_any(s, qd.p, kd.p, vd.p, static_cast<T*>(p.out), Bp, H, N, Npad, kl.p, p.nlens, ql.p, rs.p, split16,
                                    p.o_planar != 0, p.hi_only));
        CHK(copy_f32<T>(s, p.out, p.out_f32, p.n_out));
    }
    HIPCHK(hipStreamSynchronize(s));
    return F5_OK;
}

static int attention_run(const char* who, int32_t prec, const float* q, const float* k, const float* v, int Bp, int H, int N,
                         const f5k_attn* p, hipStream_t s) {
    auto bad = [&](const char* what) { return fail(F5_EINVAL, "%s: %s", who, what); };
    if (!q || !k || !v || !p || !p->out || Bp <= 0 || H <= 0 || N <= 0) return bad("bad arguments");
    if (prec != F5_PREC_F32 && prec != F5_PREC_F16X3 && prec != F5_PREC_BF16 && prec != F5_PREC_F16)
        return bad("precision must be f32, f16x3, bf16 or f16");
    const bool x3 = prec == F5_PREC_F16X3;
    if (p->mode != 0 && p->mode != 1) return bad("mode must be 0 (the precision's own kernel) or 1 (attn16)");
    if (p->mode == 1 && !x3) return bad("mode 1 (the f16 kernel writing pre-split f32 rows) exists under F5_PREC_F16X3 only");
    if (p->hi_only < 0 || p->hi_only > 3 || ((p->hi_only || p->o_planar) && (!x3 || p->mode != 0)))
        return bad("hi_only (0..3) and o_planar belong to the split kernel (F5_PREC_F16X3, mode 0)");
    if (!(p->vt_pad_fill == p->vt_pad_fill) || p->vt_pad_fill - p->vt_pad_fill != 0.f) return bad("vt_pad_fill must be finite");
    if ((p->kv_lens_host || p->q_lens_host) && (p->nlens < 1 || p->nlens > Bp)) return bad("nlens must be 1 .. Bp");
    if (p->row_start_host && !row_start_ok(p->row_start_host, Bp, N, [](int) { return 0; }))
        return bad("row_start must start at 0, in multiples of 4, at most round_up(N, 4) apart");
    const int64_t out_rows = p->row_start_host ? p->row_start_host[Bp] : (int64_t)Bp * N;
    if (p->n_out < out_rows * H * 64) return bad("out is smaller than the rows the launch may write");
    if (p->mode == 1) return attn_body<f16_t>(q, k, v, Bp, H, N, *p, false, s);
    return F5K_BY_PREC(prec, attn_body, q, k, v, Bp, H, N, *p, x3, s);
}

extern "C" int f5k_attention_ex(int32_t prec, const float* q, const float* k, const float* v, int32_t Bp, int32_t H, int32_t N,
                                const f5k_attn* p, f5_stream stream) {
    return attention_run("f5k_attention_ex", prec, q, k, v, Bp, H, N, p, (hipStream_t)stream);
}

extern "C" int f5k_attention(int32_t prec, const float* q, const float* k, const float* v, const int32_t* kv_lens_host,
                             float* out, int32_t Bp, int32_t H, int32_t N, f5_stream stream) {
    if (!out || Bp <= 0 || H <= 0 || N <= 0) return fail(F5_EINVAL, "f5k_attention: bad arguments");
    f5k_attn p{};
    p.kv_lens_host = kv_lens_host;
    p.nlens = Bp;
    p.n_out = (int64_t)Bp * N * H * 64;
    Scratch<uint16_t> o16;
    if (prec == F5_PREC_BF16 || prec == F5_PREC_F16) {
        HIPCHK(o16.alloc((size_t)p.n_out));
        p.out = o16.p;
        p.out_f32 = out;
    } else {
        p.out = out;
    }
    return attention_run("f5k_attention", prec, q, k, v, Bp, H, N, &p, (hipStream_t)stream);
}

template <typename T>
static int convpos_body(const float* x, const float* w, const float* bias, const float* res, float* y, int Bp, int N, int D,
                        const f5k_conv& p, bool split16, hipStream_t s) {
    const int cpg = D / 16, Kp = round_up(31 * cpg, GEMM_ROW_BYTES / (int)sizeof(T));
    Scratch<T> wp;
    Scratch<int> ld, rs;
    HIPCHK(wp.alloc((size_t)D * Kp));
    CHK(upload_ints(ld, p.lens_host, p.nlens));
    CHK(upload_ints(rs, p.row_start_host, Bp + 1));
    hipLaunchKernelGGL((conv_pack_kernel<T>), dim3(ew_blocks((long)D * Kp)), dim3(256), 0, s, w, wp.p, (long)D, cpg, 31, Kp);
    KCHK();
    const bool split = split16 && std::is_same_v<T, float> && convpos_can_split(D);
    if (split) HIPCHK(split_planes(s, wp.p, (size_t)D * Kp));
    HIPCHK(launch_convpos<T>(s, x, wp.p, Kp, bias, res, y, Bp, N, D, ld.p, p.nlens, rs.p, split));
    HIPCHK(hipStreamSynchronize(s));
    return F5_OK;
}

static int convpos_run(const char* who, int32_t prec, const float* x, const float* w, const float* bias, const float* res, float* y,
                       int Bp, int N, int D, const f5k_conv* p, hipStream_t s) {
    auto bad = [&](const char* what) { return fail(F5_EINVAL, "%s: %s", who, what); };
    if (!x || !w || !bias || !y || !p || Bp <= 0 || N <= 0) return bad("bad arguments");
    if (D != 256 && D != 512 && D != 768 && D != 1024) return bad("D must be 256, 512, 768 or 1024");
    if (p->lens_host && (p->nlens < 1 || p->nlens > Bp)) return bad("nlens must be 1 .. Bp");
    auto len = [&](int b) { return p->lens_host ? std::min(N, std::max(0, (int)p->lens_host[b % p->nlens])) : N; };
    if (p->lens_host)
        for (int i = 0; i < p->nlens; ++i)
            if (p->lens_host[i] < 0) return bad("lens must not be negative");
    if (p->row_start_host && !row_start_ok(p->row_start_host, Bp, N, len))
        return bad("row_start must start at 0, in multiples of 4, each span from the row's length to round_up(N, 4)");
    if (p->rows < (p->row_start_host ? p->row_start_host[Bp] : (int64_t)Bp * N)) return bad("x / res / y have fewer rows than the launch touches");
    return F5K_BY_PREC(prec, convpos_body, x, w, bias, res, y, Bp, N, D, *p, prec == F5_PREC_F16X3, s);
}

extern "C" int f5k_convpos_ex(int32_t prec, const float* x, const float* w, const float* bias, const float* res, float* y, int32_t Bp,
                              int32_t N, int32_t D, const f5k_conv* p, f5_stream stream) {
    return convpos_run("f5k_convpos_ex", prec, x, w, bias, res, y, Bp, N, D, p, (hipStream_t)stream);
}

extern "C" int f5k_convpos(int32_t prec, const float* x, const float* w, const float* bias, const float* res,
                           const int32_t* lens_host, float* y, int32_t Bp, int32_t N, int32_t D, f5_stream stream) {
    f5k_conv p{};
    p.lens_host = lens_host;
    p.nlens = Bp;
    p.rows = (int64_t)Bp * N;
    return convpos_run("f5k_convpos", prec, x, w, bias, res, y, Bp, N, D, &p, (hipStream_t)stream);
}

extern "C" int f5k_layernorm_mod(const float* x, const float* scale, const float* shift, float* out, int32_t R, int32_t D,
                                 int32_t rows_per_batch, float eps, f5_stream stream) {
    if (!x || !out || R <= 0 || D <= 0 || D % 4 || D > 2048 || rows_per_batch <= 0) return fail(F5_EINVAL, "f5k_layernorm_mod: bad arguments");
    hipStream_t s = (hipStream_t)stream;
    hipLaunchKernelGGL((layernorm_kernel<float>), dim3((R + 3) / 4), dim3(256), 0, s, x, D, out, D, R, D, eps, scale, shift, D,
                       rows_per_batch, 1, Prefetch{});
    KCHK();
    HIPCHK(hipStreamSynchronize(s));
    return F5_OK;
}

template <typename TO>
static int layernorm_ex_impl(const float* x, const float* scale, const float* shift, void* out, float* out_f32, int R, int D,
                             int rows_per_batch, float eps, int m_limit, int planar, hipStream_t s) {
    Scratch<int> ml;
    if (m_limit >= 0) {
        HIPCHK(ml.alloc(1));
        HIPCHK(hipMemcpy(ml.p, &m_limit, 4, hipMemcpyHostToDevice));
    }
    TO* o = static_cast<TO*>(out);
    hipLaunchKernelGGL((layernorm_kernel<TO>), dim3((R + 3) / 4), dim3(256), 0, s, x, D, o, D, R, D, eps, scale, shift, D, rows_per_batch,
                       1, Prefetch{}, m_limit >= 0 ? ml.p : nullptr, planar == 1);
    KCHK();
    if constexpr (std::is_same_v<TO, float>) {
        if (planar == 2) {
            hipLaunchKernelGGL(split_planar_kernel, dim3(ew_blocks((long)R * D / 32)), dim3(256), 0, s, o, (long)R * D / 32);
            KCHK();
        }
    }
    if (!std::is_same_v<TO, float> && out_f32) {
        hipLaunchKernelGGL((to_f32_kernel<TO>), dim3(ew_blocks((long)R * D)), dim3(256), 0, s, o, out_f32, (long)R * D);
        KCHK();
    }
    HIPCHK(hipStreamSynchronize(s));
    return F5_OK;
}

extern "C" int f5k_layernorm_mod_ex(int32_t prec, const float* x, const float* scale, const float* shift, void* out, float* out_f32,
                                    int32_t R, int32_t D, int32_t rows_per_batch, float eps, int32_t m_limit, int32_t planar,
                                    f5_stream stream) {
    if (!x || !out || R <= 0 || D <= 0 || D % 4 || D > 2048 || rows_per_batch <= 0 || m_limit < -1)
        return fail(F5_EINVAL, "f5k_layernorm_mod_ex: bad arguments");
    if (prec != F5_PREC_F32 && prec != F5_PREC_F16X3 && prec != F5_PREC_BF16 && prec != F5_PREC_F16)
        return fail(F5_EINVAL, "f5k_layernorm_mod_ex: precision must be f32, f16x3, bf16 or f16");
    if (planar < 0 || planar > 2 || (planar && (prec == F5_PREC_BF16 || prec == F5_PREC_F16 || D % 32)) || (planar == 2 && m_limit >= 0))
        return fail(F5_EINVAL, "f5k_layernorm_mod_ex: planar needs an f32 output and D %% 32 == 0 (planar 2: every row)");
    return F5K_BY_PREC(prec, layernorm_ex_impl, x, scale, shift, out, out_f32, R, D, rows_per_batch, eps, m_limit, planar,
                       (hipStream_t)stream);
}

template <typename T, typename Epi>
static int epi_gemm(hipStream_t s, const T* a, const T* w, int ld, int M, int N, int K, const Epi& epi, int cfg, const int* ml,
                    GemmOperands ops) {
    if (cfg == G3_256x256_PP && !(gemm_has_pingpong(sizeof(T), ops) && gemm3_epilogue_ok(epi)))
        return fail(F5_EINVAL, "f5k_gemm_epi: the ping-pong kernel (cfg 20) takes 16-bit or pre-split operands and a QKV split at 256 columns");
    HIPCHK(launch_gemm<T>(s, a, ld, w, ld, M, N, K, epi, {ops, cfg, ml}));
    return F5_OK;
}

template <typename T, typename TO>
static int epi_qkv(hipStream_t s, const T* a, const T* w, int ld, int M, int N, int K, const float* bias, const f5k_epi& p, const int* ml,
                   GemmOperands ops) {
    Scratch<float> frag;
    HIPCHK(frag.alloc((size_t)p.maxpos * 64));
    hipLaunchKernelGGL(rope_frag_kernel, dim3(ew_blocks((long)p.maxpos * 16)), dim3(256), 0, s, p.rope_cos, p.rope_sin, frag.p, (long)p.maxpos);
    KCHK();
    Scratch<int> rs;
    Scratch<int2> rowmap;
    if (p.row_start_host) {
        HIPCHK(rs.alloc((size_t)p.Bp + 1));
        HIPCHK(hipMemcpy(rs.p, p.row_start_host, ((size_t)p.Bp + 1) * 4, hipMemcpyHostToDevice));
        HIPCHK(rowmap.alloc((size_t)M));
        HIPCHK(hipMemsetAsync(rowmap.p, 0, (size_t)M * sizeof(int2), s));
        launch_fill_rowmap(s, rs.p, rowmap.p, p.Bp);
        KCHK();
        ml = rs.p + p.Bp;
    }
    const bool norm = p.kind == F5K_EPI_QKNORM;
    TO* q = static_cast<TO*>(p.out0);
    TO* k = static_cast<TO*>(p.out1);
    CHK(epi_gemm<T>(s, a, w, ld, M, N, K,
                    EpiQKV<TO>{q, k, static_cast<TO*>(p.out2), bias, frag.p, p.Nseq, p.Npad, p.H, norm ? 0 : p.pe_heads,
                               norm ? 1.0f : p.q_scale, rowmap.p},
                    p.cfg, ml, ops));
    if (norm) {
        const long qrows = (long)p.Bp * p.H * p.Nseq;
        hipLaunchKernelGGL((qknorm_rope_kernel<TO>), dim3((unsigned)((qrows * 16 + 255) / 256)), dim3(256), 0, s, q, k, p.gq, p.gk,
                           p.rope_cos, p.rope_sin, qrows, p.Nseq, p.H, p.pe_heads, p.q_scale, 1e-6f);
        KCHK();
    }
    CHK(copy_f32<TO>(s, p.out0, p.out0_f32, p.n0));
    CHK(copy_f32<TO>(s, p.out1, p.out1_f32, p.n1));
    CHK(copy_f32<TO>(s, p.out2, p.out2_f32, p.n2));
    HIPCHK(hipStreamSynchronize(s));
    return F5_OK;
}

template <typename T>
static int gemm_epi_impl(const float* A, const float* W, const float* bias, int M, int N, int K, const f5k_epi& p, GemmOperands ops,
                         hipStream_t s) {
    const int Kp = round_up(K, GEMM_ROW_BYTES / (int)sizeof(T));
    GemmStage<T> g;
    CHK(g.stage(s, A, K, W, K, M, N, K, Kp, ops));
    Scratch<int> ml;
    if (p.m_limit >= 0) {
        HIPCHK(ml.alloc(1));
        HIPCHK(hipMemcpy(ml.p, &p.m_limit, 4, hipMemcpyHostToDevice));
    }
    Scratch<int> lens;
    switch (p.kind) {
        case F5K_EPI_STORE:
            if (p.out16) {
                if constexpr (sizeof(T) == 2) {
                    CHK(epi_gemm<T>(s, g.a.p, g.w.p, Kp, M, N, Kp, EpiStore<T>{static_cast<T*>(p.out0), N, bias, p.act}, p.cfg, ml.p, ops));
                    CHK(copy_f32<T>(s, p.out0, p.out0_f32, p.n0));
                }
            } else {
                CHK(epi_gemm<T>(s, g.a.p, g.w.p, Kp, M, N, Kp, EpiStore<float>{static_cast<float*>(p.out0), N, bias, p.act, p.planar == 1}, p.cfg,
                                ml.p, ops));
                if (p.planar == 2) {
                    hipLaunchKernelGGL(split_planar_kernel, dim3(ew_blocks((long)M * N / 32)), dim3(256), 0, s, static_cast<float*>(p.out0),
                                       (long)M * N / 32);
                    KCHK();
                }
            }
            break;
        case F5K_EPI_GATE_RES:
            if (p.lens_host) {
                HIPCHK(lens.alloc((size_t)p.nlens));
                HIPCHK(hipMemcpy(lens.p, p.lens_host, (size_t)p.nlens * 4, hipMemcpyHostToDevice));
            }
            CHK(epi_gemm<T>(s, g.a.p, g.w.p, Kp, M, N, Kp,
                            EpiGateRes{static_cast<float*>(p.out0), p.res, N, bias, p.gate, p.gate_stride, p.rows_per_batch, lens.p}, p.cfg,
                            ml.p, ops));
            break;
        default:
            if (p.out16) {
                if constexpr (std::is_same_v<T, float>) CHK((epi_qkv<T, f16_t>(s, g.a.p, g.w.p, Kp, M, N, Kp, bias, p, ml.p, ops)));
            } else {
                CHK((epi_qkv<T, T>(s, g.a.p, g.w.p, Kp, M, N, Kp, bias, p, ml.p, ops)));
            }
            break;
    }
    HIPCHK(hipStreamSynchronize(s));
    return F5_OK;
}

extern "C" int f5k_gemm_epi(int32_t prec, const float* A, const float* W, const float* bias, int32_t M, int32_t N, int32_t K,
                            const f5k_epi* p, f5_stream stream) {
    if (!A || !W || !p || !p->out0 || M <= 0 || N <= 0 || K <= 0 || (N % 4)) return fail(F5_EINVAL, "f5k_gemm_epi: bad arguments (N %% 4 == 0)");
    if (prec != F5_PREC_F32 && prec != F5_PREC_F16X3 && prec != F5_PREC_BF16 && prec != F5_PREC_F16)
        return fail(F5_EINVAL, "f5k_gemm_epi: precision must be f32, f16x3, bf16 or f16");
    if (p->cfg != -1 && (!gemm_tile(p->cfg) || v1_tile(p->cfg)))
        return fail(F5_EINVAL, "f5k_gemm_epi: cfg must be -1, 2, 8, 9, 10, 13 or 20");
    if (p->m_limit < -1 || p->m_limit > M) return fail(F5_EINVAL, "f5k_gemm_epi: m_limit must be -1 or 0..M");
    if (p->a_presplit && prec != F5_PREC_F16X3) return fail(F5_EINVAL, "f5k_gemm_epi: a_presplit needs F5_PREC_F16X3");
    const bool op16 = prec == F5_PREC_BF16 || prec == F5_PREC_F16;
    switch (p->kind) {
        case F5K_EPI_STORE:
            if (p->out16 && !op16) return fail(F5_EINVAL, "f5k_gemm_epi: a 16-bit STORE needs a 16-bit operand precision");
            if (p->planar < 0 || p->planar > 2 || (p->planar && (p->out16 || prec != F5_PREC_F16X3 || N % 32)) || (p->planar == 2 && p->m_limit >= 0))
                return fail(F5_EINVAL, "f5k_gemm_epi: planar needs an f32 output under f16x3 and N %% 32 == 0 (planar 2: every row)");
            if (p->act != F5_ACT_NONE && p->act != F5_ACT_GELU_TANH) return fail(F5_EINVAL, "f5k_gemm_epi: act must be none or GELU-tanh");
            break;
        case F5K_EPI_GATE_RES:
            if (p->out16 || p->rows_per_batch <= 0 || !p->res) return fail(F5_EINVAL, "f5k_gemm_epi: GATE_RES needs res and rows_per_batch > 0");
            if (p->lens_host && p->nlens < (M - 1) / p->rows_per_batch + 1) return fail(F5_EINVAL, "f5k_gemm_epi: lens shorter than the batch rows");
            break;
        case F5K_EPI_QKV:
        case F5K_EPI_QKNORM: {
            const bool norm = p->kind == F5K_EPI_QKNORM;
            if (!p->out1 || !p->out2 || !bias || !p->rope_cos || !p->rope_sin || p->H <= 0 || N != 3 * p->H * 64 || p->Nseq <= 0 ||
                p->Npad < p->Nseq || p->Npad % 8 || p->pe_heads < 0 || p->pe_heads > p->H || p->maxpos < p->Nseq || p->Bp <= 0)
                return fail(F5_EINVAL, "f5k_gemm_epi: bad QKV arguments");
            if (p->out16 && op16) return fail(F5_EINVAL, "f5k_gemm_epi: out16 QKV is the f16 output of f32 / f16x3 operands");
            if (norm && (p->out16 || !p->gq || !p->gk || p->row_start_host)) return fail(F5_EINVAL, "f5k_gemm_epi: bad QKNORM arguments");
            if (p->row_start_host) {
                if (p->m_limit != -1 || p->row_start_host[0] != 0 || p->row_start_host[p->Bp] > M)
                    return fail(F5_EINVAL, "f5k_gemm_epi: row_start must start at 0, end <= M and replaces m_limit");
                for (int b = 0; b < p->Bp; ++b) {
                    const int cnt = p->row_start_host[b + 1] - p->row_start_host[b];
                    if (p->row_start_host[b] % 4 || cnt < 0 || cnt > round_up(p->Nseq, 4))
                        return fail(F5_EINVAL, "f5k_gemm_epi: row_start entries must be multiples of 4, at most round_up(Nseq, 4) apart");
                }
            } else if (M != p->Bp * p->Nseq) {
                return fail(F5_EINVAL, "f5k_gemm_epi: M must be Bp * Nseq without row_start");
            }
            break;
        }
        default: return fail(F5_EINVAL, "f5k_gemm_epi: unknown epilogue kind");
    }
    const GemmOperands ops = prec != F5_PREC_F16X3 ? GemmOperands::Plain : p->a_presplit ? GemmOperands::AWSplit : GemmOperands::WSplit;
    return F5K_BY_PREC(prec, gemm_epi_impl, A, W, bias, M, N, K, *p, ops, (hipStream_t)stream);
}

static int glue_done(hipStream_t s) {
    KCHK();
    HIPCHK(hipStreamSynchronize(s));
    return F5_OK;
}
static bool glue_prec_ok(int32_t prec) { return prec == F5_PREC_F32 || prec == F5_PREC_F16X3 || prec == F5_PREC_BF16 || prec == F5_PREC_F16; }

template <typename T>
static int pack_input_impl(const float* x, const float* cond, const float* tc, const float* tu, void* out, int ldo, int B, int Bp, int N, int mel,
                           int Dt, int drop, const int2* rowmap, const int* row_limit, const int* lens, hipStream_t s) {
    launch_pack_input<T>(s, x, cond, tc, tu, static_cast<T*>(out), ldo, B, Bp, N, mel, Dt, drop, rowmap, row_limit, lens);
    return glue_done(s);
}
extern "C" int f5k_pack_input(int32_t prec, const float* x, const float* cond, const float* text_c, const float* text_u, void* out, int32_t ldo,
                              int32_t B, int32_t Bp, int32_t N, int32_t mel, int32_t Dt, int32_t drop_cond_first, const void* rowmap,
                              const int32_t* row_limit, const int32_t* lens, f5_stream stream) {
    if (!x || !cond || !text_c || !text_u || !out || B <= 0 || (Bp != B && Bp != 2 * B) || N <= 0 || mel <= 0 || Dt <= 0 || mel % 4 || Dt % 4 ||
        ldo < 2 * mel + Dt || ldo % 4)
        return fail(F5_EINVAL, "f5k_pack_input: bad arguments (Bp = B or 2 B; mel, Dt, ldo %% 4 == 0; ldo >= 2 mel + Dt)");
    if (!glue_prec_ok(prec)) return fail(F5_EINVAL, "f5k_pack_input: precision must be f32, f16x3, bf16 or f16");
    if ((rowmap != nullptr) != (row_limit != nullptr) || (rowmap != nullptr) != (lens != nullptr))
        return fail(F5_EINVAL, "f5k_pack_input: rowmap, row_limit and lens come together (RowPack) or not at all");
    return F5K_BY_PREC(prec, pack_input_impl, x, cond, text_c, text_u, out, ldo, B, Bp, N, mel, Dt, drop_cond_first,
                       static_cast<const int2*>(rowmap), row_limit, lens, (hipStream_t)stream);
}
extern "C" int f5k_fill_rowmap(const int32_t* row_start, void* rowmap, int32_t Bp, f5_stream stream) {
    if (!row_start || !rowmap || Bp <= 0) return fail(F5_EINVAL, "f5k_fill_rowmap: bad arguments");
    launch_fill_rowmap((hipStream_t)stream, row_start, static_cast<int2*>(rowmap), Bp);
    return glue_done((hipStream_t)stream);
}
static int ode_args(const char* who, const void* y, const void* pred, int B, int N, int mel, const void* row_start, const void* lens,
                    const void* tgrid, int step, const void* out, bool need_out) {
    if (!y || !pred || !tgrid || (need_out && !out) || B <= 0 || N <= 0 || mel <= 0 || mel % 4 || step < 0 || (row_start != nullptr) != (lens != nullptr))
        return fail(F5_EINVAL, "%s: bad arguments (mel %% 4 == 0; row_start and lens come together)", who);
    return F5_OK;
}
extern "C" int f5k_euler_cfg(float* y, const float* pred, int32_t B, int32_t N, int32_t mel, const int32_t* row_start, const int32_t* lens,
                             const float* tgrid, int32_t step, float cfg, int32_t use_cfg, float* traj_slot, f5_stream stream) {
    CHK(ode_args("f5k_euler_cfg", y, pred, B, N, mel, row_start, lens, tgrid, step, traj_slot, false));
    launch_euler_cfg((hipStream_t)stream, y, pred, B, N, mel, row_start, lens, tgrid, step, cfg, use_cfg ? 1 : 0, traj_slot);
    return glue_done((hipStream_t)stream);
}
extern "C" int f5k_midpoint_half_cfg(const float* y, const float* pred, int32_t B, int32_t N, int32_t mel, const int32_t* row_start,
                                     const int32_t* lens, const float* tgrid, int32_t step, float cfg, int32_t use_cfg, float* y_mid,
                                     f5_stream stream) {
    CHK(ode_args("f5k_midpoint_half_cfg", y, pred, B, N, mel, row_start, lens, tgrid, step, y_mid, true));
    launch_midpoint_half_cfg((hipStream_t)stream, y, pred, B, N, mel, row_start, lens, tgrid, step, cfg, use_cfg ? 1 : 0, y_mid);
    return glue_done((hipStream_t)stream);
}
extern "C" int f5k_select_rows(const float* a, const float* b, const uint8_t* rowmask, float* out, int64_t rows, int32_t C, f5_stream stream) {
    if (!a || !rowmask || !out || rows <= 0 || C <= 0 || C % 4) return fail(F5_EINVAL, "f5k_select_rows: bad arguments (C %% 4 == 0)");
    launch_select_rows((hipStream_t)stream, a, b, rowmask, out, (long)rows, C);
    return glue_done((hipStream_t)stream);
}
extern "C" int f5k_time_sinus(const float* t, const float* freq, float* feat, int32_t S, f5_stream stream) {
    if (!t || !freq || !feat || S <= 0) return fail(F5_EINVAL, "f5k_time_sinus: bad arguments");
    launch_time_sinus((hipStream_t)stream, t, freq, feat, S);
    return glue_done((hipStream_t)stream);
}
template <typename TO> static int xrmsnorm_impl(const float* x, void* out, int R, int D, const float* g, int planar, hipStream_t s) {
    launch_xrmsnorm<TO>(s, x, static_cast<TO*>(out), R, D, g, planar);
    return glue_done(s);
}
static bool planar_ok(int32_t prec, int planar, int D) {
    return planar == 0 || (planar == 1 && (prec == F5_PREC_F32 || prec == F5_PREC_F16X3) && D % 32 == 0);
}
extern "C" int f5k_xrmsnorm(int32_t prec, const float* x, void* out, int32_t R, int32_t D, const float* g, int32_t planar, f5_stream stream) {
    if (!x || !out || !g || R <= 0 || D <= 0 || D % 4 || D > 2048 || !glue_prec_ok(prec) || !planar_ok(prec, planar, D))
        return fail(F5_EINVAL, "f5k_xrmsnorm: bad arguments (D %% 4 == 0, D <= 2048; planar: an f32 output and D %% 32 == 0)");
    return F5K_BY_PREC(prec, xrmsnorm_impl, x, out, R, D, g, planar, (hipStream_t)stream);
}
extern "C" int f5k_unett_assemble(const float* h, const float* temb, int32_t temb_stride, float* x, int32_t Bp, int32_t N, int32_t D,
                                  f5_stream stream) {
    if (!h || !temb || !x || Bp <= 0 || N <= 0 || D <= 0 || D % 4 || (temb_stride != 0 && temb_stride != D))
        return fail(F5_EINVAL, "f5k_unett_assemble: bad arguments (D %% 4 == 0, temb_stride 0 or D)");
    launch_unett_assemble((hipStream_t)stream, h, temb, temb_stride, x, Bp, N, D);
    return glue_done((hipStream_t)stream);
}
template <typename T> static int cat2_impl(const float* x, const float* skip, void* out, int rows, int D, int planar, hipStream_t s) {
    launch_cat2<T>(s, x, skip, static_cast<T*>(out), rows, D, planar);
    return glue_done(s);
}
extern "C" int f5k_cat2(int32_t prec, const float* x, const float* skip, void* out, int32_t rows, int32_t D, int32_t planar, f5_stream stream) {
    if (!x || !skip || !out || rows <= 0 || D <= 0 || D % 4 || !glue_prec_ok(prec) || !planar_ok(prec, planar, D))
        return fail(F5_EINVAL, "f5k_cat2: bad arguments (D %% 4 == 0; planar: an f32 output and D %% 32 == 0)");
    return F5K_BY_PREC(prec, cat2_impl, x, skip, out, rows, D, planar, (hipStream_t)stream);
}
extern "C" int f5k_strip_first_token(const float* in, float* out, int32_t Bp, int32_t N, int32_t C, f5_stream stream) {
    if (!in || !out || Bp <= 0 || N <= 0 || C <= 0 || C % 4) return fail(F5_EINVAL, "f5k_strip_first_token: bad arguments (C %% 4 == 0)");
    launch_strip_first_token((hipStream_t)stream, in, out, Bp, N, C);
    return glue_done((hipStream_t)stream);
}
```

### korean-f5-tts_amd/csrc/kapi_diag.hip

```cpp
#include "kapi_common.h"

static int g_cold_weights = 0;
static int g_out_bf16 = 0;

template <typename T, typename Epi>
static hipError_t gemm2_dispatch(int cfg, hipStream_t s, const T* A, int lda, const T* W, int ldw, int M, int N, int K,
                                 const Epi& dyn_epi) {
    constexpr GemmOperands P = GemmOperands::Plain;
    return with_static_act(dyn_epi, [&](const auto& epi) {
        using E = std::decay_t<decltype(epi)>;
        switch (cfg) {
            case 0: return launch_gemm2<T, 128, 128, 2, 2, 3, E>(s, A, lda, W, ldw, M, N, K, epi);
            case 1: return launch_gemm2<T, 128, 128, 2, 2, 4, E>(s, A, lda, W, ldw, M, N, K, epi);
            case 20: return launch_gemm3<T, E>(s, A, lda, W, ldw, M, N, K, epi);
            case 420: return launch_gemm3<T, E, P, GemmDiag::NoEpilogue>(s, A, lda, W, ldw, M, N, K, epi);
            case 3: return launch_gemm2<T, 128, 64, 2, 2, 4, E>(s, A, lda, W, ldw, M, N, K, epi);
            case 5: return launch_gemm2<T, 64, 64, 2, 2, 4, E>(s, A, lda, W, ldw, M, N, K, epi);
            case 7: return launch_gemm2<T, 128, 128, 4, 2, 3, E>(s, A, lda, W, ldw, M, N, K, epi);
            case 11: return launch_gemm2<T, 128, 192, 2, 4, 4, E>(s, A, lda, W, ldw, M, N, K, epi);
            case 102: return launch_gemm2<T, 128, 128, 2, 4, 4, E, P, GemmDiag::DmaOnly>(s, A, lda, W, ldw, M, N, K, epi);
            case 202: return launch_gemm2<T, 128, 128, 2, 4, 4, E, P, GemmDiag::ComputeOnly>(s, A, lda, W, ldw, M, N, K, epi);
            case 16: return launch_gemm2<T, 128, 128, 2, 4, 2, E>(s, A, lda, W, ldw, M, N, K, epi);
            case 17: return launch_gemm2<T, 256, 128, 4, 2, 2, E>(s, A, lda, W, ldw, M, N, K, epi);
            case 18: return launch_gemm2<T, 128, 128, 2, 2, 2, E>(s, A, lda, W, ldw, M, N, K, epi);
            case 113: return launch_gemm2<T, 256, 128, 4, 2, 3, E, P, GemmDiag::DmaOnly>(s, A, lda, W, ldw, M, N, K, epi);
            case 213: return launch_gemm2<T, 256, 128, 4, 2, 3, E, P, GemmDiag::ComputeOnly>(s, A, lda, W, ldw, M, N, K, epi);
            case 413: return launch_gemm2<T, 256, 128, 4, 2, 3, E, P, GemmDiag::NoEpilogue>(s, A, lda, W, ldw, M, N, K, epi);
            case 402: return launch_gemm2<T, 128, 128, 2, 4, 4, E, P, GemmDiag::NoEpilogue>(s, A, lda, W, ldw, M, N, K, epi);
            case 409: return launch_gemm2<T, 128, 64, 4, 2, 4, E, P, GemmDiag::NoEpilogue>(s, A, lda, W, ldw, M, N, K, epi);
        }
        return launch_gemm_tile<T, P, E, true>(s, A, lda, W, ldw, M, N, K, epi, cfg, nullptr, GemmConv{});
    });
}

template <typename T>
static int gemm2_impl(const float* A, const float* W, const float* bias, int act, float* out, int M, int N, int K, int cfg,
                      int iters, float* avg_us, hipStream_t s) {
    const int Kp = round_up(K, 128 / (int)sizeof(T));
    GemmStage<T> g;
    CHK(g.stage(s, A, K, W, K, M, N, K, Kp));
    HIPCHK(gemm2_dispatch<T>(cfg, s, g.a.p, Kp, g.w.p, Kp, M, N, Kp, EpiStore<float>{out, N, bias, act}));
    if (iters > 0 && avg_us) {
        const bool cold = g_cold_weights != 0;
        const size_t wbytes = (size_t)N * Kp * sizeof(T);
        const int ncopy = cold ? (int)std::min<size_t>(64, (320u << 20) / wbytes + 1) : 1;
        Scratch<T> wc;
        if (cold) {
            HIPCHK(wc.alloc((size_t)ncopy * N * Kp));
            for (int c = 0; c < ncopy; ++c)
                HIPCHK(hipMemcpyAsync(wc.p + (size_t)c * N * Kp, g.w.p, wbytes, hipMemcpyDeviceToDevice, s));
        }
        hipEvent_t e0, e1;
        HIPCHK(hipEventCreate(&e0));
        HIPCHK(hipEventCreate(&e1));
        for (int i = 0; cold && i < ncopy; ++i)
            HIPCHK(gemm2_dispatch<T>(cfg, s, g.a.p, Kp, wc.p + (size_t)(i % ncopy) * N * Kp, Kp, M, N, Kp, EpiStore<float>{out, N, bias, act}));
        HIPCHK(hipEventRecord(e0, s));
        for (int i = 0; i < iters; ++i) {
            const T* wp = cold ? wc.p + (size_t)(i % ncopy) * N * Kp : g.w.p;
            if (g_out_bf16)
                HIPCHK(gemm2_dispatch<T>(cfg, s, g.a.p, Kp, wp, Kp, M, N, Kp, EpiStore<bf16_t>{reinterpret_cast<bf16_t*>(out), N, bias, act}));
            else
                HIPCHK(gemm2_dispatch<T>(cfg, s, g.a.p, Kp, wp, Kp, M, N, Kp, EpiStore<float>{out, N, bias, act}));
        }
        HIPCHK(hipEventRecord(e1, s));
        HIPCHK(hipEventSynchronize(e1));
        float ms = 0.f;
        HIPCHK(hipEventElapsedTime(&ms, e0, e1));
        *avg_us = ms * 1000.f / iters;
        (void)hipEventDestroy(e0);
        (void)hipEventDestroy(e1);
    }
    HIPCHK(hipStreamSynchronize(s));
    return F5_OK;
}

extern "C" int f5x_set_xcd_mode(int32_t on) { xcd_mode() = on; return 0; }
extern "C" int f5x_set_attn_variant(int32_t v) { attn2_variant() = v; return 0; }
extern "C" int f5x_set_cold_weights(int32_t on) { g_cold_weights = on; return 0; }
extern "C" int f5x_set_out_bf16(int32_t on) { g_out_bf16 = on; return 0; }
extern "C" int f5x_gemm2(int32_t prec, const float* A, const float* W, const float* bias, int32_t act, float* out, int32_t M,
                         int32_t N, int32_t K, int32_t cfg, int32_t iters, float* avg_us, f5_stream stream) {
    if (!A || !W || !out || M <= 0 || N <= 0 || K <= 0 || (N % 4)) return fail(F5_EINVAL, "f5x_gemm2: bad arguments");
    hipStream_t s = (hipStream_t)stream;
    return F5K_BY_PREC(prec, gemm2_impl, A, W, bias, act, out, M, N, K, cfg, iters, avg_us, s);
}


extern "C" int f5x_block_gemm_time(int32_t M, int32_t cfg, int32_t iters, float* us4, f5_stream stream) {
    if (M <= 0 || M % 1024 || iters <= 0 || !us4) return fail(F5_EINVAL, "f5x_block_gemm_time: M must be a multiple of 1024");
    hipStream_t s = (hipStream_t)stream;
    typedef bf16_t T;
    const int D = 1024, F = 2048, N = 1024, ncopy = 8;
    const int H = getenv("F5X_QKV_H") ? atoi(getenv("F5X_QKV_H")) : 16;
    const int PE = getenv("F5X_QKV_PE") ? atoi(getenv("F5X_QKV_PE")) : 1;
    Scratch<T> xn, ao, ffh, q, k, vt, wqkv, wout, wff1, wff2;
    Scratch<float> x, bias, gate, rope, rnd;
    HIPCHK(xn.alloc((size_t)M * D)); HIPCHK(ao.alloc((size_t)M * D)); HIPCHK(ffh.alloc((size_t)M * F));
    HIPCHK(q.alloc((size_t)M * D * 3 / 2)); HIPCHK(k.alloc((size_t)M * D * 3 / 2)); HIPCHK(vt.alloc((size_t)M * D));
    HIPCHK(wqkv.alloc((size_t)ncopy * 3 * D * D)); HIPCHK(wout.alloc((size_t)ncopy * D * D));
    HIPCHK(wff1.alloc((size_t)ncopy * F * D)); HIPCHK(wff2.alloc((size_t)ncopy * D * F));
    HIPCHK(x.alloc((size_t)M * D)); HIPCHK(bias.alloc(3 * D)); HIPCHK(gate.alloc((size_t)(M / N) * D)); HIPCHK(rope.alloc((size_t)2 * N * 32));
    const size_t nr = (size_t)4 << 20;
    HIPCHK(rnd.alloc(nr));
    std::vector<float> h(nr);
    unsigned r = 777u;
    for (size_t i = 0; i < nr; ++i) { r = r * 1664525u + 1013904223u; h[i] = (((r >> 8) & 0xFFFF) / 32768.0f - 1.0f) * 0.05f; }
    HIPCHK(hipMemcpy(rnd.p, h.data(), nr * 4, hipMemcpyHostToDevice));
    auto fill_t = [&](T* dst, size_t n) {
        for (size_t o = 0; o < n; o += nr) {
            const size_t c = std::min(nr, n - o);
            hipLaunchKernelGGL((cast_pad_kernel<T>), dim3(ew_blocks((long)c)), dim3(256), 0, s, rnd.p, (int)c, 1, (int)c, dst + o, (int)c, 1);
        }
    };
    fill_t(xn.p, (size_t)M * D); fill_t(ao.p, (size_t)M * D); fill_t(ffh.p, (size_t)M * F);
    fill_t(wqkv.p, (size_t)ncopy * 3 * D * D); fill_t(wout.p, (size_t)ncopy * D * D); fill_t(wff1.p, (size_t)ncopy * F * D); fill_t(wff2.p, (size_t)ncopy * D * F);
    HIPCHK(hipMemcpyAsync(bias.p, rnd.p, 3 * D * 4, hipMemcpyDeviceToDevice, s));
    HIPCHK(hipMemcpyAsync(gate.p, rnd.p + 4096, (size_t)(M / N) * D * 4, hipMemcpyDeviceToDevice, s));
    HIPCHK(hipMemcpyAsync(rope.p, rnd.p + 65536, (size_t)2 * N * 32 * 4, hipMemcpyDeviceToDevice, s));
    HIPCHK(hipMemsetAsync(x.p, 0, (size_t)M * D * 4, s));
    KCHK();
    hipEvent_t ev[5];
    for (auto& e : ev) HIPCHK(hipEventCreate(&e));
    double acc[4] = {0, 0, 0, 0};
    for (int it = -2; it < iters; ++it) {
        const int c = (it + 2) % ncopy;
        HIPCHK(hipEventRecord(ev[0], s));
        HIPCHK(launch_gemm<T>(s, xn.p, D, wqkv.p + (size_t)c * 3 * D * D, D, M, 3 * D, D,
                              EpiQKV<T>{q.p, k.p, vt.p, bias.p, rope.p, N, N, H, PE, 0.18f, nullptr}, {GemmOperands::Plain, cfg}));
        HIPCHK(hipEventRecord(ev[1], s));
        HIPCHK(launch_gemm<T>(s, ao.p, D, wout.p + (size_t)c * D * D, D, M, D, D, EpiGateRes{x.p, x.p, D, bias.p, gate.p, D, N, nullptr}, {GemmOperands::Plain, cfg}));
        HIPCHK(hipEventRecord(ev[2], s));
        HIPCHK(launch_gemm<T>(s, xn.p, D, wff1.p + (size_t)c * F * D, D, M, F, D, EpiStore<T>{ffh.p, F, bias.p, F5_ACT_GELU_TANH}, {GemmOperands::Plain, cfg}));
        HIPCHK(hipEventRecord(ev[3], s));
        HIPCHK(launch_gemm<T>(s, ffh.p, F, wff2.p + (size_t)c * D * F, F, M, D, F, EpiGateRes{x.p, x.p, D, bias.p, gate.p, D, N, nullptr}, {GemmOperands::Plain, cfg}));
        HIPCHK(hipEventRecord(ev[4], s));
        HIPCHK(hipEventSynchronize(ev[4]));
        if (it >= 0)
            for (int g = 0; g < 4; ++g) {
                float ms = 0.f;
                HIPCHK(hipEventElapsedTime(&ms, ev[g], ev[g + 1]));
                acc[g] += ms * 1000.0;
            }
    }
    for (int g = 0; g < 4; ++g) us4[g] = (float)(acc[g] / iters);
    for (auto& e : ev) (void)hipEventDestroy(e);
    return F5_OK;
}

extern "C" int f5x_pair_time(int32_t M, int32_t N, int32_t K, int32_t cfg, int32_t iters, float* res6, f5_stream stream) {
    hipStream_t s = (hipStream_t)stream;
    typedef bf16_t T;
    Scratch<float> x, sc;
    Scratch<T> xn, xn2, w, o;
    const int ncopy = 48;
    HIPCHK(x.alloc((size_t)M * K));
    HIPCHK(sc.alloc((size_t)2 * K));
    HIPCHK(xn.alloc((size_t)M * K));
    HIPCHK(xn2.alloc((size_t)M * K));
    HIPCHK(w.alloc((size_t)ncopy * N * K));
    HIPCHK(o.alloc((size_t)M * N));
    HIPCHK(hipMemsetAsync(x.p, 0x3c, (size_t)M * K * 4, s));
// ... 90 lines not shown
extern "C" int f5x_grid_barrier_probe(int32_t blocks, int32_t iters, int32_t payload_floats, float* us_per_barrier, int32_t* bad_out,
                                      f5_stream stream) {
    hipStream_t s = (hipStream_t)stream;
    Scratch<unsigned> ctr, data, bad;
    Scratch<float> payload;
    HIPCHK(ctr.alloc(1));
    HIPCHK(bad.alloc(1));
    HIPCHK(data.alloc(blocks));
    HIPCHK(payload.alloc((size_t)blocks * std::max(payload_floats, 1) * 512));
    hipEvent_t e0, e1;
    HIPCHK(hipEventCreate(&e0));
    HIPCHK(hipEventCreate(&e1));
    float ms = 0.f;
    for (int rep = 0; rep < 2; ++rep) {
        HIPCHK(hipMemsetAsync(ctr.p, 0, 4, s));
        HIPCHK(hipMemsetAsync(bad.p, 0, 4, s));
        HIPCHK(hipMemsetAsync(data.p, 0, (size_t)blocks * 4, s));
        HIPCHK(hipEventRecord(e0, s));
        hipLaunchKernelGGL(grid_barrier_probe_kernel, dim3(blocks), dim3(512), 0, s, ctr.p, data.p, iters, payload_floats, payload.p, bad.p);
        HIPCHK(hipEventRecord(e1, s));
        HIPCHK(hipEventSynchronize(e1));
        HIPCHK(hipEventElapsedTime(&ms, e0, e1));
    }
    unsigned b = 0;
    HIPCHK(hipMemcpy(&b, bad.p, 4, hipMemcpyDeviceToHost));
    *us_per_barrier = ms * 1000.f / iters;
    *bad_out = (int32_t)b;
    (void)hipEventDestroy(e0);
    (void)hipEventDestroy(e1);
    return F5_OK;
}


__global__ __launch_bounds__(512) void mfma_rate_probe_kernel(int iters, unsigned long long* out) {
    bf16x8 a, b;
    for (int i = 0; i < 8; ++i) { a[i] = (bf16_t)(float)(threadIdx.x & 7); b[i] = (bf16_t)1.0f; }
    f32x4 acc[8];
    for (int i = 0; i < 8; ++i) acc[i] = f32x4{0.f, 0.f, 0.f, 0.f};
    const unsigned long long c0 = __builtin_readcyclecounter(), r0 = wall_clock64();
    for (int it = 0; it < iters; ++it) {
#pragma unroll
        for (int i = 0; i < 8; ++i) acc[i] = __builtin_amdgcn_mfma_f32_16x16x32_bf16(a, b, acc[i], 0, 0, 0);
    }
    const unsigned long long c1 = __builtin_readcyclecounter(), r1 = wall_clock64();
    float sink = 0.f;
    for (int i = 0; i < 8; ++i) sink += acc[i][0] + acc[i][3];
    if (threadIdx.x == 0) {
        out[blockIdx.x * 3 + 0] = c1 - c0;
        out[blockIdx.x * 3 + 1] = r1 - r0;
        out[blockIdx.x * 3 + 2] = (unsigned long long)(sink != 12345.678f);
    }
}

extern "C" int f5x_mfma_rate_probe(int32_t blocks, int32_t threads, int32_t iters, double* cyc_per_mfma_per_simd, double* mhz,
                                   double* tflops, f5_stream stream) {
    hipStream_t s = (hipStream_t)stream;
    Scratch<unsigned long long> out;
    HIPCHK(out.alloc((size_t)blocks * 3));
    hipEvent_t e0, e1;
    HIPCHK(hipEventCreate(&e0));
    HIPCHK(hipEventCreate(&e1));
    float ms = 0.f;
    for (int rep = 0; rep < 3; ++rep) {
        HIPCHK(hipEventRecord(e0, s));
        hipLaunchKernelGGL(mfma_rate_probe_kernel, dim3(blocks), dim3(threads), 0, s, iters, out.p);
        HIPCHK(hipEventRecord(e1, s));
        HIPCHK(hipEventSynchronize(e1));
        HIPCHK(hipEventElapsedTime(&ms, e0, e1));
    }
    std::vector<unsigned long long> h((size_t)blocks * 3);
    HIPCHK(hipMemcpy(h.data(), out.p, h.size() * 8, hipMemcpyDeviceToHost));
    double cyc = 0, real = 0;
    for (int b = 0; b < blocks; ++b) { cyc += (double)h[b * 3]; real += (double)h[b * 3 + 1]; }
    cyc /= blocks; real /= blocks;
    const int waves_per_simd = (threads / 64 + 3) / 4;
    *cyc_per_mfma_per_simd = cyc / ((double)iters * 8 * waves_per_simd);
    *mhz = cyc / (real / 100.0);
    *tflops = (double)blocks * (threads / 64) * iters * 8 * 16384.0 / (ms * 1e-3) / 1e12;
    (void)hipEventDestroy(e0);
    (void)hipEventDestroy(e1);
    return F5_OK;
}

__global__ __launch_bounds__(512) void store_pattern_kernel(void* out, int ld, int mode, int rd) {
    const int lane = threadIdx.x & 63, wave = threadIdx.x >> 6, wr = wave >> 2, wc = wave & 3;
    const int l15 = lane & 15, g = lane >> 4;
    const size_t m0 = (size_t)blockIdx.y * 256 + wr * 128, n0 = (size_t)blockIdx.x * 256 + wc * 64;
    if (mode == 0) {
        unsigned short* o = reinterpret_cast<unsigned short*>(out);
#pragma unroll
        for (int j = 0; j < 4; ++j)
#pragma unroll
            for (int i = 0; i < 8; ++i)
                *reinterpret_cast<uint2*>(o + (m0 + i * 16 + l15) * ld + n0 + j * 16 + g * 4) = make_uint2(0x3c003c00u + i, 0x3c003c00u + j);
    } else if (mode == 1) {
        unsigned short* o = reinterpret_cast<unsigned short*>(out);
#pragma unroll
        for (int p = 0; p < 16; ++p)
            *reinterpret_cast<uint4*>(o + (m0 + p * 8 + (lane >> 3)) * ld + n0 + (lane & 7) * 8) = make_uint4(0x3c003c00u + p, 1u, 2u, 3u);
    } else if (mode == 2) {
        float* o = reinterpret_cast<float*>(out);
#pragma unroll
        for (int j = 0; j < 4; ++j)
#pragma unroll
            for (int i = 0; i < 8; ++i) {
                float4* p = reinterpret_cast<float4*>(o + (m0 + i * 16 + l15) * ld + n0 + j * 16 + g * 4);
                float4 v = rd ? *p : make_float4(1.f, 2.f, 3.f, 4.f);
                v.x += 1.f; v.y += (float)i; v.z += (float)j; v.w += 1.f;
                *p = v;
            }
    } else {
        float* o = reinterpret_cast<float*>(out);
#pragma unroll
        for (int p = 0; p < 32; ++p) {
            float4* q = reinterpret_cast<float4*>(o + (m0 + p * 4 + (lane >> 4)) * ld + n0 + (lane & 15) * 4);
            float4 v = rd ? *q : make_float4(1.f, 2.f, 3.f, 4.f);
            v.x += 1.f; v.y += (float)p; v.z += 2.f; v.w += 1.f;
            *q = v;
        }
    }
}
extern "C" int f5x_store_pattern_probe(int32_t M, int32_t N, int32_t mode, int32_t rd, int32_t iters, float* avg_us, f5_stream stream) {
    if (M % 256 || N % 256 || mode < 0 || mode > 3 || iters <= 0 || !avg_us) return fail(F5_EINVAL, "f5x_store_pattern_probe: bad arguments");
    hipStream_t s = (hipStream_t)stream;
    Scratch<float> buf;
    HIPCHK(buf.alloc((size_t)M * N));
    HIPCHK(hipMemsetAsync(buf.p, 0, (size_t)M * N * 4, s));
    hipEvent_t e0, e1;
    HIPCHK(hipEventCreate(&e0));
    HIPCHK(hipEventCreate(&e1));
    for (int i = 0; i < 2; ++i) hipLaunchKernelGGL(store_pattern_kernel, dim3(N / 256, M / 256), dim3(512), 0, s, buf.p, N, mode, rd);
    HIPCHK(hipEventRecord(e0, s));
    for (int i = 0; i < iters; ++i) hipLaunchKernelGGL(store_pattern_kernel, dim3(N / 256, M / 256), dim3(512), 0, s, buf.p, N, mode, rd);
    HIPCHK(hipEventRecord(e1, s));
    HIPCHK(hipEventSynchronize(e1));
    KCHK();
    float ms = 0.f;
    HIPCHK(hipEventElapsedTime(&ms, e0, e1));
    *avg_us = ms * 1000.f / iters;
    (void)hipEventDestroy(e0);
    (void)hipEventDestroy(e1);
    return F5_OK;
}
```

Baseline: 237.8 audio_sec/wall_sec.

## Add write-through store policy for attention, layernorm, GEMM epilogue outputs

Adds a configurable store policy (F5_STORE_WT mask, default F5_WT_DEFAULT) that switches output writes of attention, layernorm/rmsnorm, the FF1 GEMM store and gate-residual epilogues to write-through stores. Where possible it packs them into 16-byte stores through lane shuffles or regrouping. It applies only when rows <= 4096 and the tensor is under a byte limit. The goal is to cut cache writeback cost for small intermediates that the next kernel reads right away. It adds branches and shuffles, and the real effect depends on cache behaviour and on which bits the default mask enables.

After: 247.4 audio_sec/wall_sec (median of 6 runs). 1.04x the previous value.

```diff
diff --git a/korean-f5-tts_amd/csrc/attn2.h b/korean-f5-tts_amd/csrc/attn2.h
--- a/korean-f5-tts_amd/csrc/attn2.h
+++ b/korean-f5-tts_amd/csrc/attn2.h
@@ -184,7 +184,8 @@
                                                                const T* __restrict__ Vt, T* __restrict__ O, int H,
                                                                int N, int Npad, const int* __restrict__ kv_lens,
                                                                int nbatch_lens, const int* __restrict__ q_lens,
-                                                               const int* __restrict__ o_row_start, float* __restrict__ Of = nullptr) {
+                                                               const int* __restrict__ o_row_start, float* __restrict__ Of = nullptr,
+                                                               int wt = 0) {
     extern __shared__ __attribute__((aligned(16))) char smem[];
     int bhid, qblk;
     attn_block_map(bhid, qblk);
@@ -302,6 +303,24 @@
             const float inv = 1.0f / (lrun[qs] * a0 + l1 * a1);
             const int q = q0 + qs * 16 + l15;
             const size_t orow = o_row_start ? (size_t)o_row_start[b] + q : (size_t)b * N + q;
+            if (wt && !Of) {
+                const bool in = q < (o_row_start ? min(N, o_row_start[b + 1] - o_row_start[b]) : N);
+#pragma unroll
+                for (int dt = 0; dt < 4; dt += 2) {
+                    u32x2 pk[2];
+#pragma unroll
+                    for (int d2 = 0; d2 < 2; ++d2) {
+                        float v[4];
+#pragma unroll
+                        for (int r = 0; r < 4; ++r)
+                            v[r] = (o[dt + d2][qs][r] * a0 + mb[(((dt + d2) * 2 + qs) * 4 + r) * 64 + lane] * a1) * inv;
+                        pk[d2] = pack4<T>(v[0], v[1], v[2], v[3]);
+                    }
+                    const u32x4 d = regroup_pair16(pk[0], pk[1]);
+                    if (in) store16_wt(O, (orow * (H * 64) + h * 64 + dt * 16 + g * 8) * 2, d);
+                }
+                continue;
+            }
             if (q < (o_row_start ? min(N, o_row_start[b + 1] - o_row_start[b]) : N)) {
                 T* dst = O + orow * (H * 64) + h * 64 + g * 4;
 #pragma unroll
@@ -326,7 +345,8 @@
 template <typename T>
 inline hipError_t launch_attention_v2(hipStream_t s, const T* Q, const T* K, const T* Vt, T* O, int Bp, int H,
                                       int N, int Npad, const int* kv_lens, int nbatch_lens, const int* q_lens, const int* o_row_start,
-                                      float* o_planar_f32 = nullptr) {
+                                      float* o_planar_f32 = nullptr, int wt = 0) {
+    wt = wt && (size_t)Bp * N * H * 64 * sizeof(T) < F5_WT_MAX_BYTES ? 1 : 0;
     constexpr int smem = 3 * 2 * 64 * 128;
     dim3 grid(Bp * H, (N + 127) / 128);
     const int var = attn2_variant();
@@ -339,7 +359,7 @@
             if (e != hipSuccess) return e;                                                                             \
             attr_set = true;                                                                                           \
         }                                                                                                              \
-        hipLaunchKernelGGL((attn2_fwd_kernel<T, V>), grid, dim3(512), smem, s, Q, K, Vt, O, H, N, Npad, kv_lens, nbatch_lens, q_lens, o_row_start, o_planar_f32); \
+        hipLaunchKernelGGL((attn2_fwd_kernel<T, V>), grid, dim3(512), smem, s, Q, K, Vt, O, H, N, Npad, kv_lens, nbatch_lens, q_lens, o_row_start, o_planar_f32, wt); \
     }
     if (var == 0) F5_ATTN2_LAUNCH(0)
     else if (var == 3) F5_ATTN2_LAUNCH(3)
@@ -350,17 +370,17 @@
 
 inline hipError_t launch_attention_any(hipStream_t s, const bf16_t* Q, const bf16_t* K, const bf16_t* Vt, bf16_t* O, int Bp,
                                        int H, int N, int Npad, const int* kv_lens, int nbl, const int* q_lens = nullptr,
-                                       const int* o_row_start = nullptr, bool  = false, bool  = false, int  = 0) {
-    return launch_attention_v2<bf16_t>(s, Q, K, Vt, O, Bp, H, N, Npad, kv_lens, nbl, q_lens, o_row_start);
+                                       const int* o_row_start = nullptr, bool  = false, bool  = false, int  = 0, int wt = 0) {
+    return launch_attention_v2<bf16_t>(s, Q, K, Vt, O, Bp, H, N, Npad, kv_lens, nbl, q_lens, o_row_start, nullptr, wt);
 }
 inline hipError_t launch_attention_any(hipStream_t s, const f16_t* Q, const f16_t* K, const f16_t* Vt, f16_t* O, int Bp,
                                        int H, int N, int Npad, const int* kv_lens, int nbl, const int* q_lens = nullptr,
-                                       const int* o_row_start = nullptr, bool  = false, bool  = false, int  = 0) {
-    return launch_attention_v2<f16_t>(s, Q, K, Vt, O, Bp, H, N, Npad, kv_lens, nbl, q_lens, o_row_start);
+                                       const int* o_row_start = nullptr, bool  = false, bool  = false, int  = 0, int wt = 0) {
+    return launch_attention_v2<f16_t>(s, Q, K, Vt, O, Bp, H, N, Npad, kv_lens, nbl, q_lens, o_row_start, nullptr, wt);
 }
 inline hipError_t launch_attention_any(hipStream_t s, const float* Q, const float* K, const float* Vt, float* O, int Bp, int H,
                                        int N, int Npad, const int* kv_lens, int nbl, const int* q_lens = nullptr,
-                                       const int* o_row_start = nullptr, bool split16 = false, bool o_planar = false, int hi_only = 0) {
+                                       const int* o_row_start = nullptr, bool split16 = false, bool o_planar = false, int hi_only = 0, int  = 0) {
     if (split16) return launch_attention_split(s, Q, K, Vt, O, Bp, H, N, Npad, kv_lens, nbl, q_lens, o_row_start, o_planar, hi_only);
     return launch_attention<float>(s, Q, K, Vt, O, Bp, H, N, Npad, kv_lens, nbl, q_lens, o_row_start);
 }
diff --git a/korean-f5-tts_amd/csrc/elementwise.h b/korean-f5-tts_amd/csrc/elementwise.h
--- a/korean-f5-tts_amd/csrc/elementwise.h
+++ b/korean-f5-tts_amd/csrc/elementwise.h
@@ -11,12 +11,35 @@
 }
 
 struct Prefetch { const char* p0 = nullptr; size_t n0 = 0; const char* p1 = nullptr; size_t n1 = 0; };
+template <typename TO>
+__device__ __forceinline__ void store_row_wt(TO* out, size_t row_off, const float4 (&y)[8], int D, int lane, int planar) {
+    if constexpr (sizeof(TO) == 2) {
+#pragma unroll
+        for (int i = 0; i < 8; i += 2) {
+            const u32x2 a = pack4<TO>(y[i].x, y[i].y, y[i].z, y[i].w), b = pack4<TO>(y[i + 1].x, y[i + 1].y, y[i + 1].z, y[i + 1].w);
+            if ((i + 2) * 256 <= D) {
+                const bool odd = lane & 1;
+                const u32x2 send = odd ? a : b;
+                const u32x2 recv = {(unsigned)__shfl_xor((int)send[0], 1, 64), (unsigned)__shfl_xor((int)send[1], 1, 64)};
+                const u32x4 d = odd ? u32x4{recv[0], recv[1], b[0], b[1]} : u32x4{a[0], a[1], recv[0], recv[1]};
+                store16_wt(out, (row_off + (i + (odd ? 1 : 0)) * 256 + (lane >> 1) * 8) * 2, d);
+            } else {
+                if (lane * 4 + i * 256 < D) store8_wt(out + row_off + lane * 4 + i * 256, a);
+                if (lane * 4 + (i + 1) * 256 < D) store8_wt(out + row_off + lane * 4 + (i + 1) * 256, b);
+            }
+        }
+    } else {
+#pragma unroll
+        for (int i = 0; i < 8; ++i)
+            if (lane * 4 + i * 256 < D) store4_at_wt(out, row_off, lane * 4 + i * 256, planar, y[i].x, y[i].y, y[i].z, y[i].w);
+    }
+}
 template <typename TO>
 __global__ __launch_bounds__(256) void layernorm_kernel(const float* __restrict__ x, int ldx, TO* __restrict__ out,
                                                         int ldo, int R, int D, float eps, const float* __restrict__ A,
                                                         const float* __restrict__ Bv, int vec_stride,
                                                         int rows_per_batch, int modulate, Prefetch pf,
-                                                        const int* __restrict__ m_limit = nullptr, int planar = 0) {
+                                                        const int* __restrict__ m_limit = nullptr, int planar = 0, int wt = 0) {
     const int lane = threadIdx.x & 63;
     const int r = blockIdx.x * 4 + (threadIdx.x >> 6);
     if (r >= R || (m_limit && r >= *m_limit)) return;
@@ -56,15 +79,28 @@
         }
     }
     const float rstd = rsqrtf(wave_sum(q) / (float)D + eps);
-#pragma unroll
-    for (int i = 0; i < 8; ++i) {
-        const int c = lane * 4 + i * 256;
-        if (c < D) {
+    if (wt) {
+        float4 y[8];
+#pragma unroll
+        for (int i = 0; i < 8; ++i) {
             float4 a = ga[i];
             const float4 b = gb[i];
             if (modulate) { a.x += 1.f; a.y += 1.f; a.z += 1.f; a.w += 1.f; }
-            store4_at(out + (size_t)r * ldo, c, planar, (v[i].x - mean) * rstd * a.x + b.x, (v[i].y - mean) * rstd * a.y + b.y,
-                      (v[i].z - mean) * rstd * a.z + b.z, (v[i].w - mean) * rstd * a.w + b.w);
+            y[i] = make_float4((v[i].x - mean) * rstd * a.x + b.x, (v[i].y - mean) * rstd * a.y + b.y, (v[i].z - mean) * rstd * a.z + b.z,
+                               (v[i].w - mean) * rstd * a.w + b.w);
+        }
+        store_row_wt(out, (size_t)r * ldo, y, D, lane, planar);
+    } else {
+#pragma unroll
+        for (int i = 0; i < 8; ++i) {
+            const int c = lane * 4 + i * 256;
+            if (c < D) {
+                float4 a = ga[i];
+                const float4 b = gb[i];
+                if (modulate) { a.x += 1.f; a.y += 1.f; a.z += 1.f; a.w += 1.f; }
+                store4_at(out + (size_t)r * ldo, c, planar, (v[i].x - mean) * rstd * a.x + b.x, (v[i].y - mean) * rstd * a.y + b.y,
+                          (v[i].z - mean) * rstd * a.z + b.z, (v[i].w - mean) * rstd * a.w + b.w);
+            }
         }
     }
 #pragma unroll
@@ -73,7 +109,7 @@
 
 template <typename TO>
 __global__ __launch_bounds__(256) void xrmsnorm_kernel(const float* __restrict__ x, int ldx, TO* __restrict__ out, int ldo,
-                                                       int R, int D, const float* __restrict__ gvec, int planar = 0) {
+                                                       int R, int D, const float* __restrict__ gvec, int planar = 0, int wt = 0) {
     const int lane = threadIdx.x & 63;
     const int r = blockIdx.x * 4 + (threadIdx.x >> 6);
     if (r >= R) return;
@@ -88,6 +124,17 @@
     }
     const float nrm = fmaxf(sqrtf(wave_sum(q)), 1e-12f);
     const float sc = sqrtf((float)D) / nrm;
+    if (wt) {
+        float4 y[8];
+#pragma unroll
+        for (int i = 0; i < 8; ++i) {
+            const int c = lane * 4 + i * 256;
+            const float4 gg = c < D ? *reinterpret_cast<const float4*>(gvec + c) : make_float4(0, 0, 0, 0);
+            y[i] = make_float4(v[i].x * sc * gg.x, v[i].y * sc * gg.y, v[i].z * sc * gg.z, v[i].w * sc * gg.w);
+        }
+        store_row_wt(out, (size_t)r * ldo, y, D, lane, planar);
+        return;
+    }
 #pragma unroll
     for (int i = 0; i < 8; ++i) {
         const int c = lane * 4 + i * 256;
@@ -97,9 +144,11 @@
         }
     }
 }
+inline int wt_fits(int wt, size_t bytes) { return wt && bytes < F5_WT_MAX_BYTES ? 1 : 0; }
 template <typename TO>
-inline void launch_xrmsnorm(hipStream_t s, const float* x, TO* out, int rows, int D, const float* g, int planar) {
-    hipLaunchKernelGGL((xrmsnorm_kernel<TO>), dim3((rows + 3) / 4), dim3(256), 0, s, x, D, out, D, rows, D, g, planar);
+inline void launch_xrmsnorm(hipStream_t s, const float* x, TO* out, int rows, int D, const float* g, int planar, int wt = 0) {
+    hipLaunchKernelGGL((xrmsnorm_kernel<TO>), dim3((rows + 3) / 4), dim3(256), 0, s, x, D, out, D, rows, D, g, planar,
+                       wt_fits(wt, (size_t)rows * D * sizeof(TO)));
 }
 
 template <typename T>
diff --git a/korean-f5-tts_amd/csrc/engine.hip b/korean-f5-tts_amd/csrc/engine.hip
--- a/korean-f5-tts_amd/csrc/engine.hip
+++ b/korean-f5-tts_amd/csrc/engine.hip
@@ -28,6 +28,7 @@
     sw.weight_prefetch = flag("F5_WEIGHT_PREFETCH", true);
     if (const char* v = getenv("F5_X3_ABLATE")) sw.x3_ablate = c.precision == F5_PREC_F16X3 ? atoi(v) : 0;
     sw.x3_attn_split = flag("F5_X3_ATTN_SPLIT", false);
+    if (const char* v = getenv("F5_STORE_WT")) sw.store_wt = atoi(v) & F5_WT_ALL;
     if (const char* v = getenv("F5_LEN_BUCKET")) sw.len_bucket = (int)std::min(std::max(atol(v), -1L), 1L << 20);
     return sw;
 }
diff --git a/korean-f5-tts_amd/csrc/engine_impl.h b/korean-f5-tts_amd/csrc/engine_impl.h
--- a/korean-f5-tts_amd/csrc/engine_impl.h
+++ b/korean-f5-tts_amd/csrc/engine_impl.h
@@ -427,6 +427,7 @@
     const int* ml() const { return pk.rows_dev; }
     int mh() const { return pk ? (int)pk.rows_host : 0; }
     int pl() const { return e->split16 ? 1 : 0; }
+    int wt(int bit) const { return rows <= 4096 && (e->sw.store_wt & bit) ? 1 : 0; }
     double gflops(double n, double k) const { return 2.0 * (pk ? pk.rows_host : (double)rows) * n * k; }
     template <typename T, typename Epi> int gemm(const T* A, int lda, const LinW<T>& L, int n, int k, const Epi& epi, bool a_split = false) const {
         HIPCHK(e->prof.timed(PC_GEMM, s, gflops(n, k), [&] { return egemm<T>(e, s, A, lda, L.w, L.ldw, rows, n, k, epi, ml(), mh(), a_split); }));
@@ -524,7 +525,7 @@
         }
         HIPCHK(pr.timed(PC_ATTN, s, attn_fl, [&] {
             return launch_attention_any(s, w.q, w.k, w.vt, w.ao, Bp, H, N, w.Npad, attn_lens, B, f.lens_dev, pk.row_start, e->split16, pl,
-                                        e->sw.x3_attn_hi());
+                                        e->sw.x3_attn_hi(), f.wt(F5_WT_ATTN));
         }));
     }
     f.ablate(8, w.ao, inner);
@@ -534,7 +535,7 @@
 template <typename T> static int ff_block(const FwdCtx& f, Work<T>& w, const BlockW<T>& bw, const EpiGateRes& out_epi) {
     const int D = f.e->cfg.dim, F = f.e->cfg.ff_dim, pl = f.pl();
     f.ablate(16, w.xn, D);
-    CHK(f.gemm(w.xn, D, bw.ff1, F, D, EpiStore<T>{w.ffh, F, bw.ff1.b, F5_ACT_GELU_TANH, pl}, pl));
+    CHK(f.gemm(w.xn, D, bw.ff1, F, D, EpiStore<T>{w.ffh, F, bw.ff1.b, F5_ACT_GELU_TANH, pl, f.wt(F5_WT_STORE16)}, pl));
     f.ablate(32, w.ffh, F);
     return f.gemm(w.ffh, F, bw.ff2, D, F, out_epi, pl);
 }
@@ -580,7 +581,7 @@
         using TO = std::remove_pointer_t<decltype(out)>;
         return pr.timed(PC_LN, s, [&] {
             hipLaunchKernelGGL((layernorm_kernel<TO>), dim3((rows + 3) / 4), dim3(256), 0, s, w.x, D, out, D, rows, D, 1e-6f, scale, shift,
-                               mod_stride, N, 1, pf, ml, planar);
+                               mod_stride, N, 1, pf, ml, planar, f.wt(F5_WT_LN));
             return hipGetLastError();
         });
     };
@@ -588,9 +589,9 @@
         BlockW<T>& bw = P.blocks[l];
         const float* m = mod_row + (size_t)l * 6 * D;
         HIPCHK(adaln(w.xn, m + D, m, prefetch(bw.qkv, bw.out), pl));
-        CHK(attention_block<T>(f, w, bw, qk_norm, EpiGateRes{w.x, w.x, D, bw.out.b, m + 2 * D, mod_stride, N, gate_lens}));
+        CHK(attention_block<T>(f, w, bw, qk_norm, EpiGateRes{w.x, w.x, D, bw.out.b, m + 2 * D, mod_stride, N, gate_lens, f.wt(F5_WT_GATE_RES)}));
         HIPCHK(adaln(w.xn, m + 4 * D, m + 3 * D, prefetch(bw.ff1, bw.ff2), pl));
-        CHK(ff_block<T>(f, w, bw, EpiGateRes{w.x, w.x, D, bw.ff2.b, m + 5 * D, mod_stride, N, nullptr}));
+        CHK(ff_block<T>(f, w, bw, EpiGateRes{w.x, w.x, D, bw.ff2.b, m + 5 * D, mod_stride, N, nullptr, f.wt(F5_WT_GATE_RES)}));
     }
     if (long_skip) {
         auto cat_skip = [&](auto* cat) {
@@ -645,7 +646,7 @@
     const int pl = f.pl();
     auto rmsnorm = [&](const float* x, auto* out, const float* g, int planar) {
         return pr.timed(PC_LN, s, [&] {
-            launch_xrmsnorm(s, x, out, rows, D, g, planar);
+            launch_xrmsnorm(s, x, out, rows, D, g, planar, f.wt(F5_WT_LN));
             return hipGetLastError();
         });
     };
@@ -663,9 +664,9 @@
             CHK(f.gemm(w.cat2, 2 * D, bw.skip, D, 2 * D, EpiStore<float>{w.x, D, nullptr, F5_ACT_NONE}, pl));
         }
         HIPCHK(rmsnorm(x_in, w.xn, bw.norm1_g, pl));
-        CHK(attention_block<T>(f, w, bw, false, EpiGateRes{w.x, x_in, D, bw.out.b, nullptr, 0, Nt, lens_dev}));
+        CHK(attention_block<T>(f, w, bw, false, EpiGateRes{w.x, x_in, D, bw.out.b, nullptr, 0, Nt, lens_dev, f.wt(F5_WT_GATE_RES)}));
         HIPCHK(rmsnorm(w.x, w.xn, bw.norm2_g, pl));
-        CHK(ff_block<T>(f, w, bw, EpiGateRes{x_out, w.x, D, bw.ff2.b, nullptr, 0, Nt, nullptr}));
+        CHK(ff_block<T>(f, w, bw, EpiGateRes{x_out, w.x, D, bw.ff2.b, nullptr, 0, Nt, nullptr, f.wt(F5_WT_GATE_RES)}));
     }
     if (e->io_split) {
         HIPCHK(rmsnorm(w.x, w.skips, P.norm_out_g, 1));
diff --git a/korean-f5-tts_amd/csrc/engine_types.h b/korean-f5-tts_amd/csrc/engine_types.h
--- a/korean-f5-tts_amd/csrc/engine_types.h
+++ b/korean-f5-tts_amd/csrc/engine_types.h
@@ -131,6 +131,7 @@
     bool x3_attn_split = false;
     int x3_attn_hi() const { return x3_attn_split ? (x3_ablate >> 1) & 3 : 3; }
     int len_bucket = 0;
+    int store_wt = F5_WT_DEFAULT;
 };
 inline bool valid_len_bucket(long g) { return g == 0 || (g >= 8 && g <= 1024 && g % 8 == 0); }
 
diff --git a/korean-f5-tts_amd/csrc/f5_common.h b/korean-f5-tts_amd/csrc/f5_common.h
--- a/korean-f5-tts_amd/csrc/f5_common.h
+++ b/korean-f5-tts_amd/csrc/f5_common.h
@@ -106,6 +106,57 @@
     store4(row + col, a, b, c, d);
 }
 
+enum { F5_WT_LN = 1, F5_WT_ATTN = 4, F5_WT_GATE_RES = 8, F5_WT_STORE16 = 16, F5_WT_ALL = 29, F5_WT_DEFAULT = F5_WT_ALL };
+inline int& store_policy() { static int m = 0; return m; }
+constexpr size_t F5_WT_MAX_BYTES = (size_t)1 << 31;
+template <typename T> __device__ __forceinline__ T* uniform_ptr(T* p) {
+    const size_t a = (size_t)p;
+    const unsigned lo = (unsigned)__builtin_amdgcn_readfirstlane((int)(unsigned)a), hi = (unsigned)__builtin_amdgcn_readfirstlane((int)(unsigned)(a >> 32));
+    return reinterpret_cast<T*>(((size_t)hi << 32) | (size_t)lo);
+}
+__device__ __forceinline__ void store16_wt(void* base, size_t byte_off, u32x4 v) {
+    __builtin_amdgcn_raw_buffer_store_b128(v, __builtin_amdgcn_make_buffer_rsrc(base, 0, 0x7fffffff, 0x00020000), (unsigned)byte_off, 0, 16);
+}
+__device__ __forceinline__ void store8_wt(void* p, u32x2 v) {
+    __hip_atomic_store(reinterpret_cast<unsigned long long*>(p), __builtin_bit_cast(unsigned long long, v), __ATOMIC_RELAXED,
+                       __HIP_MEMORY_SCOPE_AGENT);
+}
+__device__ __forceinline__ void store4_wt(float* base, size_t off, float a, float b, float c, float d) {
+    store16_wt(base, off * 4, __builtin_bit_cast(u32x4, f32x4{a, b, c, d}));
+}
+__device__ __forceinline__ void store4_wt(bf16_t* base, size_t off, float a, float b, float c, float d) { store8_wt(base + off, pack4<bf16_t>(a, b, c, d)); }
+__device__ __forceinline__ void store4_wt(f16_t* base, size_t off, float a, float b, float c, float d) { store8_wt(base + off, pack4<f16_t>(a, b, c, d)); }
+__device__ __forceinline__ void store4_planar_wt(float* base, size_t row_off, int col, float a, float b, float c, float d) {
+    u32x2 hi, lo;
+    split4_f16(__builtin_bit_cast(u32x4, f32x4{a, b, c, d}), hi, lo);
+    const int kk = col & 31;
+    char* p = reinterpret_cast<char*>(base + row_off + (col & ~31)) + ((kk & 15) >> 2) * 16 + (kk >> 4) * 8;
+    store8_wt(p, hi);
+    store8_wt(p + 64, lo);
+}
+template <typename TO> __device__ __forceinline__ void store4_at_wt(TO* base, size_t row_off, int col, int planar, float a, float b, float c, float d) {
+    if constexpr (std::is_same_v<TO, float>) {
+        if (planar) { store4_planar_wt(base, row_off, col, a, b, c, d); return; }
+    }
+    store4_wt(base, row_off + col, a, b, c, d);
+}
+template <bool WT, typename TO> __device__ __forceinline__ void store4_sel(TO* base, size_t off, float a, float b, float c, float d) {
+    if constexpr (WT) store4_wt(base, off, a, b, c, d);
+    else store4(base + off, a, b, c, d);
+}
+
+__device__ __forceinline__ u32x4 regroup_pair16(u32x2 a, u32x2 b) {
+    u32x4 r;
+#pragma unroll
+    for (int w = 0; w < 2; ++w) {
+        auto h = __builtin_amdgcn_permlane32_swap(a[w], b[w], false, false);
+        auto q = __builtin_amdgcn_permlane16_swap((unsigned)h[0], (unsigned)h[1], false, false);
+        r[w] = (unsigned)q[0];
+        r[2 + w] = (unsigned)q[1];
+    }
+    return r;
+}
+
 template <typename T> __device__ __forceinline__ u32x4 pack8(float a0, float a1, float a2, float a3, float a4, float a5, float a6, float a7);
 template <> __device__ __forceinline__ u32x4 pack8<bf16_t>(float a0, float a1, float a2, float a3, float a4, float a5, float a6, float a7) {
     bf16x8 v = {(bf16_t)a0, (bf16_t)a1, (bf16_t)a2, (bf16_t)a3, (bf16_t)a4, (bf16_t)a5, (bf16_t)a6, (bf16_t)a7};
diff --git a/korean-f5-tts_amd/csrc/gemm.h b/korean-f5-tts_amd/csrc/gemm.h
--- a/korean-f5-tts_amd/csrc/gemm.h
+++ b/korean-f5-tts_amd/csrc/gemm.h
@@ -33,6 +33,8 @@
 template <typename TO, int ACT = -1> struct EpiStore {
     TO* out; int ldo; const float* bias; int act;
     int planar = 0;
+    int wt = 0;
+    static constexpr bool kWT = sizeof(TO) == 2, kRegroup16 = kWT;
     struct RowCtx { TO* p; };
     struct ColCtx { float4 b; int n; };
     typedef NoCtx TRowCtx;
@@ -45,11 +47,27 @@
     }
     typedef NoCtx Pre;
     __device__ __forceinline__ NoCtx preload(const RowCtx&, const ColCtx&) const { return {}; }
+    template <bool WT = false>
     __device__ __forceinline__ void store(const RowCtx& r, const ColCtx& c, f32x4 v, const NoCtx&) const {
         const int a = ACT >= 0 ? ACT : act;
-        store4_at(r.p, c.n, planar, apply_act(v[0] + c.b.x, a), apply_act(v[1] + c.b.y, a), apply_act(v[2] + c.b.z, a),
-                  apply_act(v[3] + c.b.w, a));
-    }
+        if constexpr (WT)
+            store4_at_wt(out, (size_t)(r.p - out), c.n, planar, apply_act(v[0] + c.b.x, a), apply_act(v[1] + c.b.y, a),
+                         apply_act(v[2] + c.b.z, a), apply_act(v[3] + c.b.w, a));
+        else
+            store4_at(r.p, c.n, planar, apply_act(v[0] + c.b.x, a), apply_act(v[1] + c.b.y, a), apply_act(v[2] + c.b.z, a),
+                      apply_act(v[3] + c.b.w, a));
+    }
+    __device__ __forceinline__ u32x2 pack(const RowCtx&, const ColCtx& c, f32x4 v, const NoCtx&) const {
+        const int a = ACT >= 0 ? ACT : act;
+        if constexpr (sizeof(TO) == 2)
+            return pack4<TO>(apply_act(v[0] + c.b.x, a), apply_act(v[1] + c.b.y, a), apply_act(v[2] + c.b.z, a), apply_act(v[3] + c.b.w, a));
+        else return u32x2{0u, 0u};
+    }
+    __device__ __forceinline__ bool pair_ok(int, int) const { return (ldo & 7) == 0; }
+    __device__ __forceinline__ bool keep(const RowCtx&) const { return true; }
+    __device__ __forceinline__ TO* dst_base(const ColCtx&) const { return out; }
+    __device__ __forceinline__ size_t dst_off(const RowCtx& r, const ColCtx& c) const { return (size_t)(r.p - out) + c.n; }
+    template <bool WT = false> __device__ __forceinline__ void tstore(const NoCtx&, const NoCtx&, f32x4) const {}
     static constexpr bool kStaged = sizeof(TO) == 2;
     __device__ __forceinline__ bool staged_ok(bool transposed) const { return !transposed; }
     template <int MI, int NJ>
@@ -80,18 +98,17 @@
     }
     __device__ __forceinline__ NoCtx trow(int, int) const { return {}; }
     __device__ __forceinline__ NoCtx tcol(int) const { return {}; }
-    __device__ __forceinline__ void tstore(const NoCtx&, const NoCtx&, f32x4) const {}
 };
 
 template <typename Epi, typename F> inline hipError_t with_static_act(const Epi& e, F&& f) { return f(e); }
 template <typename TO, typename F> inline hipError_t with_static_act(const EpiStore<TO, -1>& e, F&& f) {
     switch (e.act) {
-        case F5_ACT_NONE: return f(EpiStore<TO, F5_ACT_NONE>{e.out, e.ldo, e.bias, e.act, e.planar});
-        case F5_ACT_GELU_TANH: return f(EpiStore<TO, F5_ACT_GELU_TANH>{e.out, e.ldo, e.bias, e.act, e.planar});
-        case F5_ACT_GELU_ERF: return f(EpiStore<TO, F5_ACT_GELU_ERF>{e.out, e.ldo, e.bias, e.act, e.planar});
-        case F5_ACT_SILU: return f(EpiStore<TO, F5_ACT_SILU>{e.out, e.ldo, e.bias, e.act, e.planar});
-        case F5_ACT_MISH: return f(EpiStore<TO, F5_ACT_MISH>{e.out, e.ldo, e.bias, e.act, e.planar});
-        case F5_ACT_LOGCLAMP: return f(EpiStore<TO, F5_ACT_LOGCLAMP>{e.out, e.ldo, e.bias, e.act, e.planar});
+        case F5_ACT_NONE: return f(EpiStore<TO, F5_ACT_NONE>{e.out, e.ldo, e.bias, e.act, e.planar, e.wt});
+        case F5_ACT_GELU_TANH: return f(EpiStore<TO, F5_ACT_GELU_TANH>{e.out, e.ldo, e.bias, e.act, e.planar, e.wt});
+        case F5_ACT_GELU_ERF: return f(EpiStore<TO, F5_ACT_GELU_ERF>{e.out, e.ldo, e.bias, e.act, e.planar, e.wt});
+        case F5_ACT_SILU: return f(EpiStore<TO, F5_ACT_SILU>{e.out, e.ldo, e.bias, e.act, e.planar, e.wt});
+        case F5_ACT_MISH: return f(EpiStore<TO, F5_ACT_MISH>{e.out, e.ldo, e.bias, e.act, e.planar, e.wt});
+        case F5_ACT_LOGCLAMP: return f(EpiStore<TO, F5_ACT_LOGCLAMP>{e.out, e.ldo, e.bias, e.act, e.planar, e.wt});
         default: return hipErrorInvalidValue;
     }
 }
@@ -99,6 +116,8 @@
 struct EpiGateRes {
     float* x; const float* res; int ld; const float* bias; const float* gate; int gate_stride; int rows_per_batch;
     const int* lens;
+    int wt = 0;
+    static constexpr bool kWT = true, kRegroup16 = false;
     struct RowCtx { size_t off; const float* g; bool masked; };
     struct ColCtx { float4 b; int n; };
     typedef NoCtx TRowCtx;
@@ -118,6 +137,7 @@
         return {*reinterpret_cast<const float4*>(res + rc.off + c.n),
                 rc.g ? *reinterpret_cast<const float4*>(rc.g + c.n) : make_float4(1, 1, 1, 1)};
     }
+    template <bool WT = false>
     __device__ __forceinline__ void store(const RowCtx& rc, const ColCtx& c, f32x4 v, const Pre& p) const {
         float4 r = p.r;
         if (!rc.masked) {
@@ -125,11 +145,12 @@
             r.x += g.x * (v[0] + c.b.x); r.y += g.y * (v[1] + c.b.y);
             r.z += g.z * (v[2] + c.b.z); r.w += g.w * (v[3] + c.b.w);
         }
-        *reinterpret_cast<float4*>(x + rc.off + c.n) = r;
+        if constexpr (WT) store4_wt(x, rc.off + c.n, r.x, r.y, r.z, r.w);
+        else *reinterpret_cast<float4*>(x + rc.off + c.n) = r;
     }
     __device__ __forceinline__ NoCtx trow(int, int) const { return {}; }
     __device__ __forceinline__ NoCtx tcol(int) const { return {}; }
-    __device__ __forceinline__ void tstore(const NoCtx&, const NoCtx&, f32x4) const {}
+    template <bool WT = false> __device__ __forceinline__ void tstore(const NoCtx&, const NoCtx&, f32x4) const {}
     static constexpr bool kStaged = true;
     __device__ __forceinline__ bool staged_ok(bool transposed) const { return !transposed && rows_per_batch >= 64; }
     template <int MI, int NJ>
@@ -182,6 +203,7 @@
     TO* q; TO* k; TO* vt; const float* bias; const float* rope;
     int Nseq, Npad, H, pe_heads; float q_scale;
     const int2* rowmap = nullptr;
+    static constexpr bool kWT = false, kRegroup16 = false;
     struct RowCtx { size_t base; const float* cs; };
     struct ColCtx { float4 b; TO* dst; size_t hoff; int d; bool rot; float scale; };
     struct TRowCtx { size_t base; int pos; int b; bool fast; int m; int M; };
diff --git a/korean-f5-tts_amd/csrc/gemm2.h b/korean-f5-tts_amd/csrc/gemm2.h
--- a/korean-f5-tts_amd/csrc/gemm2.h
+++ b/korean-f5-tts_amd/csrc/gemm2.h
@@ -300,6 +300,46 @@
     }
     if (!EARLY) epilogue_setup();
     __builtin_amdgcn_s_waitcnt(0x0F70);
+    if constexpr (Epi::kWT && BM * BN <= 128 * 192) {
+        if (epi.wt) {
+#pragma unroll
+            for (int j = 0; j < NJ; ++j) {
+                if (trj[j]) continue;
+                bool paired = false;
+                if constexpr (Epi::kRegroup16) {
+                    const int j0 = j & ~1;
+                    if (j0 + 1 < NJ && !trj[j0] && !trj[j0 + 1] && nw + (j0 + 2) * 16 <= N && epi.pair_ok(nw + j0 * 16, nw + j0 * 16 + 16)) {
+                        paired = true;
+                        if (j == j0) {
+                            auto* base = uniform_ptr(epi.dst_base(cc[j0]));
+#pragma unroll
+                            for (int i = 0; i < MI; ++i) {
+                                const u32x4 d = regroup_pair16(epi.pack(rc[i], cc[j0], acc[i][j0], pre[i][j0]),
+                                                               epi.pack(rc[i], cc[j0 + 1], acc[i][j0 + 1], pre[i][j0 + 1]));
+                                const size_t off = (g >> 1 ? epi.dst_off(rc[i], cc[j0 + 1]) : epi.dst_off(rc[i], cc[j0])) + (g & 1) * 8 - g * 4;
+                                if (mw + i * 16 + l15 < M && epi.keep(rc[i])) store16_wt(base, off * 2, d);
+                            }
+                        }
+                    }
+                }
+                if (paired || nw + j * 16 + g * 4 >= N) continue;
+#pragma unroll
+                for (int i = 0; i < MI; ++i)
+                    if (mw + i * 16 + l15 < M) epi.template store<true>(rc[i], cc[j], acc[i][j], pre[i][j]);
+            }
+            if (any_tr) {
+#pragma unroll
+                for (int j = 0; j < NJ; ++j) {
+                    const int n = nw + j * 16 + l15;
+                    if (!trj[j] || n >= N) continue;
+#pragma unroll
+                    for (int i = 0; i < MI; ++i)
+                        if (mw + i * 16 + g * 4 < M) epi.template tstore<true>(trc[i], tcc[j], acc[i][j]);
+                }
+            }
+            return;
+        }
+    }
 #pragma unroll
     for (int j = 0; j < NJ; ++j) {
         const int n = nw + j * 16 + g * 4;
diff --git a/korean-f5-tts_amd/csrc/kapi.hip b/korean-f5-tts_amd/csrc/kapi.hip
--- a/korean-f5-tts_amd/csrc/kapi.hip
+++ b/korean-f5-tts_amd/csrc/kapi.hip
@@ -144,7 +144,7 @@
             HIPCHK(launch_attention_v2<f16_t>(s, qd.p, kd.p, vd.p, nullptr, Bp, H, N, Npad, kl.p, p.nlens, ql.p, rs.p, static_cast<float*>(p.out)));
     } else {
         HIPCHK(launch_attention_any(s, qd.p, kd.p, vd.p, static_cast<T*>(p.out), Bp, H, N, Npad, kl.p, p.nlens, ql.p, rs.p, split16,
-                                    p.o_planar != 0, p.hi_only));
+                                    p.o_planar != 0, p.hi_only, store_policy() & F5_WT_ATTN));
         CHK(copy_f32<T>(s, p.out, p.out_f32, p.n_out));
     }
     HIPCHK(hipStreamSynchronize(s));
@@ -264,7 +264,7 @@
     }
     TO* o = static_cast<TO*>(out);
     hipLaunchKernelGGL((layernorm_kernel<TO>), dim3((R + 3) / 4), dim3(256), 0, s, x, D, o, D, R, D, eps, scale, shift, D, rows_per_batch,
-                       1, Prefetch{}, m_limit >= 0 ? ml.p : nullptr, planar == 1);
+                       1, Prefetch{}, m_limit >= 0 ? ml.p : nullptr, planar == 1, wt_fits(store_policy() & F5_WT_LN, (size_t)R * D * sizeof(TO)));
     KCHK();
     if constexpr (std::is_same_v<TO, float>) {
         if (planar == 2) {
@@ -356,7 +356,8 @@
         case F5K_EPI_STORE:
             if (p.out16) {
                 if constexpr (sizeof(T) == 2) {
-                    CHK(epi_gemm<T>(s, g.a.p, g.w.p, Kp, M, N, Kp, EpiStore<T>{static_cast<T*>(p.out0), N, bias, p.act}, p.cfg, ml.p, ops));
+                    CHK(epi_gemm<T>(s, g.a.p, g.w.p, Kp, M, N, Kp, EpiStore<T>{static_cast<T*>(p.out0), N, bias, p.act, 0, wt_fits(store_policy() & F5_WT_STORE16, (size_t)M * N * sizeof(T))},
+                                    p.cfg, ml.p, ops));
                     CHK(copy_f32<T>(s, p.out0, p.out0_f32, p.n0));
                 }
             } else {
@@ -375,8 +376,9 @@
                 HIPCHK(hipMemcpy(lens.p, p.lens_host, (size_t)p.nlens * 4, hipMemcpyHostToDevice));
             }
             CHK(epi_gemm<T>(s, g.a.p, g.w.p, Kp, M, N, Kp,
-                            EpiGateRes{static_cast<float*>(p.out0), p.res, N, bias, p.gate, p.gate_stride, p.rows_per_batch, lens.p}, p.cfg,
-                            ml.p, ops));
+                            EpiGateRes{static_cast<float*>(p.out0), p.res, N, bias, p.gate, p.gate_stride, p.rows_per_batch, lens.p,
+                                       wt_fits(store_policy() & F5_WT_GATE_RES, (size_t)M * N * 4)},
+                            p.cfg, ml.p, ops));
             break;
         default:
             if (p.out16) {
@@ -498,7 +500,7 @@
     return glue_done((hipStream_t)stream);
 }
 template <typename TO> static int xrmsnorm_impl(const float* x, void* out, int R, int D, const float* g, int planar, hipStream_t s) {
-    launch_xrmsnorm<TO>(s, x, static_cast<TO*>(out), R, D, g, planar);
+    launch_xrmsnorm<TO>(s, x, static_cast<TO*>(out), R, D, g, planar, store_policy() & F5_WT_LN);
     return glue_done(s);
 }
 static bool planar_ok(int32_t prec, int planar, int D) {
diff --git a/korean-f5-tts_amd/csrc/kapi_diag.hip b/korean-f5-tts_amd/csrc/kapi_diag.hip
--- a/korean-f5-tts_amd/csrc/kapi_diag.hip
+++ b/korean-f5-tts_amd/csrc/kapi_diag.hip
@@ -78,6 +78,7 @@
 extern "C" int f5x_set_xcd_mode(int32_t on) { xcd_mode() = on; return 0; }
 extern "C" int f5x_set_attn_variant(int32_t v) { attn2_variant() = v; return 0; }
 extern "C" int f5x_set_cold_weights(int32_t on) { g_cold_weights = on; return 0; }
+extern "C" int f5x_set_store_policy(int32_t mask) { store_policy() = mask & F5_WT_ALL; return 0; }
 extern "C" int f5x_set_out_bf16(int32_t on) { g_out_bf16 = on; return 0; }
 extern "C" int f5x_gemm2(int32_t prec, const float* A, const float* W, const float* bias, int32_t act, float* out, int32_t M,
                          int32_t N, int32_t K, int32_t cfg, int32_t iters, float* avg_us, f5_stream stream) {
@@ -334,6 +335,51 @@
     return F5_OK;
 }
 
+template <int POL> __device__ __forceinline__ void probe_st8(void* base, size_t off, u32x2 v) {
+    char* p = reinterpret_cast<char*>(base) + off;
+    if constexpr (POL == 1) store8_wt(p, v);
+    else if constexpr (POL == 2) __builtin_nontemporal_store(v, reinterpret_cast<u32x2*>(p));
+    else *reinterpret_cast<u32x2*>(p) = v;
+}
+template <int POL> __device__ __forceinline__ void probe_st16(void* base, size_t off, u32x4 v) {
+    char* p = reinterpret_cast<char*>(base) + off;
+    if constexpr (POL == 1) store16_wt(base, off, v);
+    else if constexpr (POL == 2) __builtin_nontemporal_store(v, reinterpret_cast<u32x4*>(p));
+    else *reinterpret_cast<u32x4*>(p) = v;
+}
+template <int POL>
+__global__ __launch_bounds__(512) void store_policy_kernel(void* out, int ld, int mode, int mi, int M) {
+    const int lane = threadIdx.x & 63, wave = threadIdx.x >> 6, wr = wave >> 2, wc = wave & 3;
+    const int l15 = lane & 15, g = lane >> 4;
+    if (mode >= 5) {
+        const size_t r = (size_t)blockIdx.x * 8 + wave;
+        if (r >= (size_t)M) return;
+        if (mode == 5) {
+            for (int i = 0; i * 256 < ld; ++i) probe_st8<POL>(out, (r * ld + lane * 4 + i * 256) * 2, u32x2{0x3c003c00u + i, 0x3c003c00u});
+        } else {
+            for (int i = 0; i * 256 < ld; i += 2)
+                probe_st16<POL>(out, (r * ld + (i + (lane & 1)) * 256 + (lane >> 1) * 8) * 2, u32x4{0x3c003c00u + i, 0x3c003c00u, 1u, 2u});
+        }
+        return;
+    }
+    const size_t m0 = (size_t)blockIdx.y * 32 * mi + wr * 16 * mi, n0 = (size_t)blockIdx.x * 256 + wc * 64;
+    if (mode == 0) {
+#pragma unroll
+        for (int j = 0; j < 4; ++j)
+            for (int i = 0; i < mi; ++i)
+                probe_st8<POL>(out, ((m0 + i * 16 + l15) * ld + n0 + j * 16 + g * 4) * 2, u32x2{0x3c003c00u + i, 0x3c003c00u + j});
+    } else if (mode == 4) {
+#pragma unroll
+        for (int j = 0; j < 4; j += 2)
+            for (int i = 0; i < mi; ++i)
+                probe_st16<POL>(out, ((m0 + i * 16 + l15) * ld + n0 + j * 16 + g * 8) * 2, u32x4{0x3c003c00u + i, 0x3c003c00u + j, 1u, 2u});
+    } else {
+#pragma unroll
+        for (int j = 0; j < 4; ++j)
+            for (int i = 0; i < mi; ++i)
+                probe_st16<POL>(out, ((m0 + i * 16 + l15) * ld + n0 + j * 16 + g * 4) * 4, u32x4{0x3f800000u + i, 0x40000000u + j, 1u, 2u});
+    }
+}
 __global__ __launch_bounds__(512) void store_pattern_kernel(void* out, int ld, int mode, int rd) {
     const int lane = threadIdx.x & 63, wave = threadIdx.x >> 6, wr = wave >> 2, wc = wave & 3;
     const int l15 = lane & 15, g = lane >> 4;
@@ -372,8 +418,14 @@
         }
     }
 }
-extern "C" int f5x_store_pattern_probe(int32_t M, int32_t N, int32_t mode, int32_t rd, int32_t iters, float* avg_us, f5_stream stream) {
-    if (M % 256 || N % 256 || mode < 0 || mode > 3 || iters <= 0 || !avg_us) return fail(F5_EINVAL, "f5x_store_pattern_probe: bad arguments");
+extern "C" int f5x_store_pattern_probe(int32_t M, int32_t N, int32_t mode, int32_t rd, int32_t policy, int32_t mi, int32_t iters, float* avg_us,
+                                       f5_stream stream) {
+    const bool pol = mi > 0;
+    if (M <= 0 || N <= 0 || N % 256 || iters <= 0 || !avg_us || (size_t)M * N * 4 >= F5_WT_MAX_BYTES ||
+        (!pol && (M % 256 || mode < 0 || mode > 3 || policy != 0)) ||
+        (pol && (mi > 8 || M % (32 * mi) || policy < 0 || policy > 2 || rd || !(mode == 0 || mode == 2 || (mode >= 4 && mode <= 6)) ||
+                 (mode == 6 && N % 512))))
+        return fail(F5_EINVAL, "f5x_store_pattern_probe: bad arguments");
     hipStream_t s = (hipStream_t)stream;
     Scratch<float> buf;
     HIPCHK(buf.alloc((size_t)M * N));
@@ -381,9 +433,16 @@
     hipEvent_t e0, e1;
     HIPCHK(hipEventCreate(&e0));
     HIPCHK(hipEventCreate(&e1));
-    for (int i = 0; i < 2; ++i) hipLaunchKernelGGL(store_pattern_kernel, dim3(N / 256, M / 256), dim3(512), 0, s, buf.p, N, mode, rd);
+    auto launch = [&]() {
+        if (!pol) { hipLaunchKernelGGL(store_pattern_kernel, dim3(N / 256, M / 256), dim3(512), 0, s, buf.p, N, mode, rd); return; }
+        const dim3 grid = mode >= 5 ? dim3((M + 7) / 8) : dim3(N / 256, M / (32 * mi));
+        if (policy == 0) hipLaunchKernelGGL(store_policy_kernel<0>, grid, dim3(512), 0, s, buf.p, N, mode, mi, M);
+        else if (policy == 1) hipLaunchKernelGGL(store_policy_kernel<1>, grid, dim3(512), 0, s, buf.p, N, mode, mi, M);
+        else hipLaunchKernelGGL(store_policy_kernel<2>, grid, dim3(512), 0, s, buf.p, N, mode, mi, M);
+    };
+    for (int i = 0; i < 2; ++i) launch();
     HIPCHK(hipEventRecord(e0, s));
-    for (int i = 0; i < iters; ++i) hipLaunchKernelGGL(store_pattern_kernel, dim3(N / 256, M / 256), dim3(512), 0, s, buf.p, N, mode, rd);
+    for (int i = 0; i < iters; ++i) launch();
     HIPCHK(hipEventRecord(e1, s));
     HIPCHK(hipEventSynchronize(e1));
     KCHK();
```
